# chronista-club/fleetflow

Hardware: AMD Instinct MI355X
Metric: container x node evaluations/sec (FFD what-if plans, work-equivalent) + achieved GB/s % HBM roofline (higher is better)
Workload: dtype u32

## Files before the change

### fleetflow_amd/_lib.py

```python
from __future__ import annotations

import ctypes as ct
import os

_HERE = os.path.dirname(os.path.abspath(__file__))
LIB_PATH = os.environ.get("FLEETPLACE_LIB") or os.path.join(_HERE, "libfleetplace.so")

FP_OK, FP_EINVAL, FP_ENOMEM, FP_EDEVICE, FP_EOVERFLOW, FP_ECORRUPT = 0, -1, -2, -3, -4, -5
FP_NONE = 0xFFFFFFFF
REASON_OK, REASON_NOFIT, REASON_CYCLE, REASON_SKEW, REASON_QUOTA = 0, 1, 2, 3, 4
FP_K_PLACE, FP_K_SORT, FP_K_FEAS, FP_K_LEVEL, FP_K_GEN = 0, 1, 2, 3, 4
STRATEGY_FIRST_FIT, STRATEGY_SPREAD, STRATEGY_PACK, STRATEGY_FILL_LOWEST = 0, 1, 2, 3
POLICY_STRATEGIES = {"spread_across_pool": STRATEGY_SPREAD, "pack_into_dedicated": STRATEGY_PACK,
                     "fill_lowest": STRATEGY_FILL_LOWEST}
FP_POLICY_MAX_NODES = 8192
FP_SPREAD_MAX_DOMAINS = 64
FP_FALLBACK_MAX_HOPS = 4
QUOTA_CPU, QUOTA_MEM, QUOTA_SERVICES, QUOTA_DIMS = 0, 1, 2, 3
QUOTA_NAMES = ("cpu", "memory", "services")
QUOTA_UNLIMITED = 0xFFFFFFFF
WHY_CORDON, WHY_CPU, WHY_MEM, WHY_LABEL, WHY_CONFLICT = 1, 2, 4, 8, 16
EXPLAIN_FAIL, EXPLAIN_ONLY, EXPLAIN_FEASIBLE, EXPLAIN_ALL, EXPLAIN_MISSING, EXPLAIN_NEAR = 0, 5, 10, 11, 12, 13
EXPLAIN_WORDS = 16
EXPLAIN_HIST_MIXED, EXPLAIN_HIST_FITS, EXPLAIN_HIST_SELECTED, EXPLAIN_HIST_WORDS = 5, 6, 7, 8
DRAIN_EVICTED, DRAIN_STRANDED, DRAIN_STRANDED_CPU, DRAIN_STRANDED_MEM = 0, 1, 2, 3
DRAIN_TARGETS, DRAIN_FIRST_STRANDED, DRAIN_NODES, DRAIN_WORDS = 4, 5, 6, 8
DRAIN_FIELDS = ("evicted", "stranded", "stranded_cpu", "stranded_mem", "targets", "first_stranded", "nodes")
DRAIN_STRANDED_SKEW, DRAIN_RELAXED, DRAIN_SKEW_BEFORE, DRAIN_SKEW_AFTER, DRAIN_POLICY_WORDS = 0, 1, 2, 3, 4
DRAIN_POLICY_FIELDS = ("stranded_skew", "relaxed", "skew_before", "skew_after")
SHRINK_RELEASED, SHRINK_TRIED, SHRINK_FAILED, SHRINK_MOVES, SHRINK_MOVED = 0, 1, 2, 3, 4
SHRINK_MOVED_CPU, SHRINK_MOVED_MEM, SHRINK_FIRST_FAILED, SHRINK_WORDS = 5, 6, 7, 8
SHRINK_FIELDS = ("released", "tried", "failed", "moves", "moved", "moved_cpu", "moved_mem", "first_failed")
SHRINK_STATE_NEVER, SHRINK_STATE_RELEASED, SHRINK_STATE_FAILED = 0, 1, 2
SHRINK_FAILED_SKEW, SHRINK_RELAXED, SHRINK_SKEW_BEFORE, SHRINK_SKEW_AFTER, SHRINK_POLICY_WORDS = 0, 1, 2, 3, 4
SHRINK_POLICY_FIELDS = ("failed_skew", "relaxed", "skew_before", "skew_after")
REBAL_MOVES, REBAL_STUCK, REBAL_STUCK_SKEW, REBAL_RELAXED, REBAL_MOVED_CPU = 0, 1, 2, 3, 4
REBAL_MOVED_MEM, REBAL_SKEW_BEFORE, REBAL_SKEW_AFTER, REBAL_WORDS = 5, 6, 7, 8
REBAL_FIELDS = ("moves", "stuck", "stuck_skew", "relaxed", "moved_cpu", "moved_mem", "skew_before", "skew_after")
GROW_PENDING, GROW_PLACED, GROW_OPENED, GROW_UNPLACEABLE, GROW_CAPPED = 0, 1, 2, 3, 4
GROW_LEFT_CPU, GROW_LEFT_MEM, GROW_FIRST_UNPLACED, GROW_WORDS = 5, 6, 7, 8
GROW_FIELDS = ("pending", "placed", "opened", "unplaceable", "capped", "left_cpu", "left_mem", "first_unplaced")
GROW_MAX_NEW = 8192
GROW_ON_LIVE, GROW_RELAXED, GROW_STUCK_SKEW, GROW_STUCK_QUOTA, GROW_SKEW_BEFORE, GROW_SKEW_AFTER = 0, 1, 2, 3, 4, 5
GROW_POLICY_WORDS = 8
GROW_POLICY_FIELDS = ("on_live", "relaxed", "stuck_skew", "stuck_quota", "skew_before", "skew_after")
CHANGE_KEPT, CHANGE_NEW, CHANGE_MOVED, CHANGE_LOST, CHANGE_ABSENT = 0, 1, 2, 3, 4
CHANGE_NAMES = ("kept", "new", "moved", "lost", "absent")
REPLAN_KEPT, REPLAN_NEW, REPLAN_MOVED, REPLAN_LOST, REPLAN_ABSENT = 0, 1, 2, 3, 4
REPLAN_MOVED_CPU, REPLAN_MOVED_MEM, REPLAN_WORDS = 5, 6, 8
FP_OPT_AUTO = -1
OPTIONS = {"pipe_w": 0, "pipe_seg": 1, "pipe_r": 2, "pipe_lag": 3, "link_slots": 4, "link_bounded": 5,
           "pipe_flush": 6, "spin_ticks": 7, "kpack": 8, "scen_sort": 9, "segsort": 10, "systolic": 11,
           "levelize_sync": 12, "systolic_extra": 13, "screen": 14, "payload_lds": 15, "systolic_valu": 16, "link_publish": 17,
           "level_sort": 18, "level_small": 19, "pipe_prio": 20,
           "indeg_bin": 21, "packed": 22, "sort_fused": 23}
GEOM_FIELDS = ("groups", "stages", "segments", "ring", "lag", "link_slots", "bounded", "resident", "systolic")

u8p = ct.POINTER(ct.c_uint8)
u32p = ct.POINTER(ct.c_uint32)
u64p = ct.POINTER(ct.c_uint64)
vp = ct.c_void_p


class FpGraph(ct.Structure):
    _fields_ = [("n_vertices", ct.c_uint32), ("n_edges", ct.c_uint32), ("row_ptr", vp), ("col", vp),
                ("has_deps", vp)]


class FpContainers(ct.Structure):
    _fields_ = [("n", ct.c_uint32), ("cpu_m", vp), ("mem_mib", vp), ("req_labels", vp), ("conflict", vp)]


class FpNodes(ct.Structure):
    _fields_ = [("n", ct.c_uint32), ("cpu_free", vp), ("mem_free", vp), ("labels", vp),
                ("conflict_used", vp), ("schedulable", vp)]


class FpBatch(ct.Structure):
    _fields_ = [("n_scen", ct.c_uint32), ("scen_base", ct.c_uint32), ("n_containers", ct.c_uint32),
                ("n_nodes", ct.c_uint32),
                ("cpu_m", vp), ("mem_mib", vp), ("req_labels", vp), ("conflict", vp), ("level", vp),
                ("cpu_free", vp), ("mem_free", vp), ("labels", vp), ("conflict_used", vp),
                ("schedulable", vp), ("assign", vp), ("reason", vp), ("cost", vp)]


class FleetplaceError(RuntimeError):
    def __init__(self, code, where):
        self.code = code
        msg = _lib_strerror(code) if _LIB is not None else str(code)
        super().__init__(f"{where}: {msg} ({code})")


_LIB = None

SIGNATURES = {
    "fp_ctx_create": (ct.c_int, [ct.POINTER(vp), ct.c_int]),
    "fp_ctx_destroy": (None, [vp]),
    "fp_ctx_set_stream": (ct.c_int, [vp, vp]),
    "fp_ctx_reset_stream": (ct.c_int, [vp]),
    "fp_ctx_sync": (ct.c_int, [vp]),
    "fp_strerror": (ct.c_char_p, [ct.c_int]),
    "fp_abi_version": (ct.c_int, []),
    "fp_ctx_profile": (ct.c_int, [vp, ct.c_int]),
    "fp_ctx_kernel_stats": (ct.c_int, [vp, ct.c_int, ct.POINTER(ct.c_double), ct.POINTER(ct.c_uint64)]),
    "fp_ctx_place_path": (ct.c_int, [vp, u32p]),
    "fp_ctx_set_option": (ct.c_int, [vp, ct.c_int, ct.c_int64]),
    "fp_ctx_get_option": (ct.c_int, [vp, ct.c_int, ct.POINTER(ct.c_int64)]),
    "fp_legacy_order": (ct.c_int, [vp, ct.POINTER(FpGraph), u32p]),
    "fp_levelize": (ct.c_int, [vp, ct.POINTER(FpGraph), u32p, u32p, u32p]),
    "fp_place": (ct.c_int, [vp, ct.POINTER(FpContainers), ct.POINTER(FpNodes), u32p, u32p, u8p]),
    "fp_place_batch": (ct.c_int, [vp, ct.POINTER(FpBatch)]),
    "fp_feasibility": (ct.c_int, [vp, ct.POINTER(FpContainers), ct.POINTER(FpNodes), u32p, u32p, u64p]),
    "fp_plan_stage": (ct.c_int, [vp, ct.POINTER(FpGraph), ct.POINTER(FpContainers), ct.POINTER(FpNodes), vp, vp,
                                 vp, u32p, vp, vp, vp, vp]),
    "fp_dev_legacy_order": (ct.c_int, [vp, ct.POINTER(FpGraph), vp]),
    "fp_dev_levelize": (ct.c_int, [vp, ct.POINTER(FpGraph), vp, vp, vp]),
    "fp_dev_place_batch": (ct.c_int, [vp, ct.POINTER(FpBatch)]),
    "fp_place_ws_bytes": (ct.c_int, [vp, ct.c_uint32, ct.c_uint32, ct.c_uint32, u64p]),
    "fp_place_geometry": (ct.c_int, [vp, ct.c_uint32, ct.c_uint32, ct.c_uint32, u32p]),
    "fp_dev_feasibility": (ct.c_int, [vp, ct.POINTER(FpContainers), ct.POINTER(FpNodes), vp, vp, vp]),
    "fp_dev_feasibility_batch": (ct.c_int, [vp, ct.POINTER(FpBatch), vp, vp]),
    "fp_place_policy": (ct.c_int, [vp, ct.POINTER(FpContainers), ct.POINTER(FpNodes), u32p, ct.c_uint32, ct.c_uint32,
                                   u32p, u32p, u8p]),
    "fp_place_batch_policy": (ct.c_int, [vp, ct.POINTER(FpBatch), u32p, u32p, u32p]),
    "fp_dev_place_batch_policy": (ct.c_int, [vp, ct.POINTER(FpBatch), vp, vp, vp]),
    "fp_place_policy_spread": (ct.c_int, [vp, ct.POINTER(FpContainers), ct.POINTER(FpNodes), u32p, ct.c_uint32,
                                          ct.c_uint32, u32p, u32p, ct.c_uint32, u32p, u8p]),
    "fp_place_batch_policy_spread": (ct.c_int, [vp, ct.POINTER(FpBatch), u32p, u32p, u32p, u32p, u32p]),
    "fp_dev_place_batch_policy_spread": (ct.c_int, [vp, ct.POINTER(FpBatch), vp, vp, vp, vp, vp]),
    "fp_place_policy_fallback": (ct.c_int, [vp, ct.POINTER(FpContainers), ct.POINTER(FpNodes), u32p, ct.c_uint32,
                                            ct.c_uint32, u32p, u32p, ct.c_uint32, u32p, ct.c_uint32, u32p, u8p, u8p]),
    "fp_place_batch_policy_fallback": (ct.c_int, [vp, ct.POINTER(FpBatch), u32p, u32p, u32p, u32p, u32p, u32p, u32p,
                                                  u8p]),
    "fp_dev_place_batch_policy_fallback": (ct.c_int, [vp, ct.POINTER(FpBatch), vp, vp, vp, vp, vp, vp, vp, vp]),
    "fp_place_policy_quota": (ct.c_int, [vp, ct.POINTER(FpContainers), ct.POINTER(FpNodes), u32p, ct.c_uint32,
                                         ct.c_uint32, u32p, u32p, ct.c_uint32, u32p, ct.c_uint32, u32p, u8p, u8p,
                                         u32p, u32p, u8p]),
    "fp_place_batch_policy_quota": (ct.c_int, [vp, ct.POINTER(FpBatch), u32p, u32p, u32p, u32p, u32p, u32p, u32p,
# ... 96 lines not shown
```

### fleetflow_amd/csrc/fp_internal.h

```cpp
#pragma once
#include <cmath>
#include <cstring>
#include <hip/hip_runtime.h>
#include <stdint.h>
#include <type_traits>
#include <vector>
#include "../../include/fleetplace.h"
#include "fp_rows.h"

#define FP_HIP(call)                                   \
    do {                                               \
        hipError_t e_ = (call);                        \
        if (e_ != hipSuccess) return fp_hip_fail(e_);  \
    } while (0)

int fp_hip_fail(hipError_t e);

__device__ __forceinline__ void fp_or_new_bits(uint32_t *w, uint32_t bits) {
    if (bits & ~*(volatile uint32_t *)w) atomicOr(w, bits);
}

struct fp_ctx {
    int device = 0;
    hipStream_t own_stream = nullptr;
// ... 137 lines not shown
                            const uint32_t *group, uint32_t n_cand, uint32_t strategy, uint32_t preferred,
                            const uint32_t *node_count, uint32_t *assign_out, uint8_t *reason_out,
                            uint32_t *summary_out, const fp_drain_policy &pol = fp_drain_policy());

struct fp_shrink_policy {
    const uint32_t *domain = nullptr;
    uint32_t max_skew = 0;
    const uint32_t *relax_mask = nullptr;
    uint32_t n_hops = 0;
    uint8_t *hops_out = nullptr;
    uint8_t *blocker_reason_out = nullptr;
    uint32_t *policy_out = nullptr;
};
constexpr uint32_t FP_SHRINK_MAX_CONTAINERS = 0x7FFF0000u;
int fp_dev_shrink_sweep_impl(fp_ctx *c, const fp_containers *cs, const fp_nodes *ns, const uint32_t *assign,
                             const uint32_t *try_order, uint32_t n_var, uint32_t n_try, uint32_t strategy,
                             uint32_t preferred, const uint32_t *node_count, uint32_t *assign_out, uint8_t *state_out,
                             uint32_t *blocker_out, uint32_t *summary_out, const fp_shrink_policy &pol = fp_shrink_policy());

struct fp_rebalance_opts {
    const uint32_t *node_count = nullptr;
    const uint32_t *domain = nullptr;
    uint32_t max_skew = 0;
    const uint32_t *relax_mask = nullptr;
    uint32_t n_hops = 0;
};
int fp_dev_rebalance_sweep_impl(fp_ctx *c, const fp_containers *cs, const fp_nodes *ns, const uint32_t *assign,
                                const uint32_t *victim_order, uint32_t n_var, uint32_t n_try, const uint32_t *max_moves,
                                uint32_t strategy, uint32_t preferred, const fp_rebalance_opts &o, uint32_t *assign_out,
                                uint8_t *hops_out, uint8_t *reason_out, uint32_t *summary_out);

int fp_dev_grow_sweep_impl(fp_ctx *c, const fp_containers *cs, const uint8_t *reason, uint32_t reason_mask,
                           uint32_t n_cand, const uint32_t *t_cpu, const uint32_t *t_mem, const uint32_t *t_labels,
                           const uint32_t *t_max, uint32_t max_new, uint32_t *summary_out, uint32_t *assign_out);

struct fp_grow_policy {
    const uint32_t *node_count = nullptr;
    uint32_t strategy = 0, preferred = 0;
    const uint32_t *domain = nullptr;
    const uint32_t *t_domain = nullptr;
    uint32_t max_skew = 0;
    const uint32_t *relax_mask = nullptr;
    uint32_t n_hops = 0;
    const uint32_t *quota = nullptr;
    const uint32_t *quota_used = nullptr;
    uint32_t *policy_out = nullptr;
    uint8_t *hops_out = nullptr;
    uint8_t *reason_out = nullptr;
};
int fp_dev_grow_sweep_policy_impl(fp_ctx *c, const fp_containers *cs, const uint8_t *reason, uint32_t reason_mask,
                                  const fp_nodes *ns, uint32_t n_cand, const uint32_t *t_cpu, const uint32_t *t_mem,
                                  const uint32_t *t_labels, const uint32_t *t_max, uint32_t max_new,
                                  uint32_t *summary_out, uint32_t *assign_out, const fp_grow_policy &pol);

int fp_dev_replan_batch_impl(fp_ctx *c, const fp_batch *b, const uint32_t *prev, const fp_policy_opts &o,
                             uint8_t *change_out, uint32_t *summary_out);
int fp_dev_replan_batch_policy_impl(fp_ctx *c, const fp_batch *b, const uint32_t *prev, const fp_policy_opts &o,
                                    uint8_t *change_out, uint32_t *summary_out);

bool fp_pipe_plan(const fp_ctx *c, uint32_t S, uint32_t N, uint32_t *G_out, uint32_t *W_out, uint32_t *B_out,
                  size_t *lds_out);
int fp_place_geometry_impl(fp_ctx *c, uint32_t S, uint32_t C, uint32_t N, uint32_t *out);
size_t fp_pipe_ws_bytes(fp_ctx *c, uint32_t S, uint32_t C, uint32_t N);
int fp_place_ws_bytes_impl(fp_ctx *c, uint32_t S, uint32_t C, uint32_t N, uint64_t *bytes);
constexpr int FP_BUCKETS = 32;
__host__ __device__ inline void fp_thresholds(uint32_t lo, uint32_t hi, uint32_t *T) {
    T[0] = 0;
    if (lo == 0) lo = 1;
    if (hi < lo) hi = lo;
    const double r = pow((double)hi / (double)lo, 1.0 / (double)(FP_BUCKETS - 2));
    double v = (double)lo;
    for (int k = 1; k < FP_BUCKETS; ++k) {
        uint32_t x = k == FP_BUCKETS - 1 ? hi : (uint32_t)ceil(v);
        if (x < T[k - 1]) x = T[k - 1];
        if (x > hi) x = hi;
        T[k] = x;
        v *= r;
    }
}
struct fp_pipe_soa {
    uint32_t *s_cpu, *s_mem, *s_req, *s_conf, *s_idx;
    uint32_t *summ = nullptr;
    bool payload_done = false;
};
int fp_pipe_soa_take(fp_ctx *c, size_t SC, fp_pipe_soa *soa);
uint32_t fp_pipe_kpack(const fp_ctx *c, uint32_t C);
int fp_pipe_node_summary(fp_ctx *c, uint32_t S, uint32_t C, uint32_t N, const fp_batch *b, uint32_t *rng,
                         uint32_t **summ);
uint32_t fp_pipe_payload_lds_max_c(const fp_ctx *c);
int fp_pipe_launch(fp_ctx *c, uint32_t S, uint32_t C, uint32_t N, uint32_t scen_base, const uint32_t *order,
                   const void *skeys, uint32_t key_bytes, uint32_t mbits, uint64_t cmax, uint64_t mmax,
                   const uint32_t *cval, const uint32_t *mval, const fp_batch *b, const uint32_t *thr,
                   const fp_pipe_soa *ready, uint32_t *rng);

namespace fpd {

constexpr uint64_t GAMMA = 0x9E3779B97F4A7C15ull;
constexpr uint64_t TAG_CONT = 0xC0C0C0C0C0C0C0C0ull;
constexpr uint64_t TAG_NODE = 0x5E5E5E5E5E5E5E5Eull;

__host__ __device__ inline uint64_t draw(uint64_t seed, uint64_t idx) {
    uint64_t z = seed + (idx + 1) * GAMMA;
    z = (z ^ (z >> 30)) * 0xBF58476D1CE4E5B9ull;
    z = (z ^ (z >> 27)) * 0x94D049BB133111EBull;
    return z ^ (z >> 31);
}
__host__ __device__ inline uint64_t scenario_seed(uint64_t seed, uint32_t s) {
    return seed ^ ((uint64_t)s * GAMMA);
}

__device__ __forceinline__ bool fits(uint32_t cpu, uint32_t mem, uint32_t req, uint32_t conf,
                                     uint32_t cf, uint32_t mf, uint32_t lab, uint32_t cu) {
    return (cf >= cpu) & (mf >= mem) & ((lab & req) == req) & ((cu & conf) == 0u);
}

__device__ __forceinline__ uint64_t pack_cost(uint32_t rej, uint32_t used, uint32_t id) {
    uint64_t r = rej > 0xFFFFFFu ? 0xFFFFFFu : rej;
    uint64_t u = used > 0xFFFFFFu ? 0xFFFFFFu : used;
    return (r << 40) | (u << 16) | (uint64_t)(id & 0xFFFFu);
}

}
```

### fleetflow_amd/csrc/fp_payload.h

```cpp
#pragma once
#include "fp_internal.h"

#ifndef FPP_PAYLOAD_BY_FIELD
#define FPP_PAYLOAD_BY_FIELD 1
#endif

namespace fpl {

constexpr uint32_t PL_THREADS = 1024, PL_H = 25, PL_MAX_C = PL_THREADS * PL_H * 2;
constexpr uint32_t PL_SKIP = 0x80000000u;
constexpr uint32_t PL_ROWS = 2 * PL_H;
constexpr uint32_t PL_FIELD_CHUNK = 36 * 1024;
constexpr size_t PL_FIELD_LDS_BYTES = (size_t)PL_FIELD_CHUNK * 4;
static_assert(PL_MAX_C < 0xFFFFu, "container indices are kept in 16 bits, 0xFFFF = no position");

enum pl_source {
    PL_ORDER = 0,
    PL_ORDER_SAME_WG,
    PL_LDS_X
};

__device__ __forceinline__ void pl_index(uint32_t w, uint32_t a0, uint32_t &d0, uint32_t &d1) {
    asm volatile("" : "+v"(w));
    d0 = (w & 0xFFFFu) - a0;
    d1 = (w >> 16) - a0;
}
__device__ __forceinline__ void pl_load_chunk(uint32_t *pl_lds, const uint32_t *__restrict__ src, uint32_t n) {
    __syncthreads();
#pragma unroll 8
    for (uint32_t i = threadIdx.x; i < n; i += PL_THREADS) pl_lds[i] = __builtin_nontemporal_load(&src[i]);
    __syncthreads();
}
__device__ __forceinline__ void pl_pick_field(uint32_t *pl_lds, const uint32_t *__restrict__ field, uint32_t C,
                                              const uint32_t (&o)[PL_H], uint32_t (&v)[PL_ROWS]) {
    for (uint32_t a0 = 0; a0 < C; a0 += PL_FIELD_CHUNK) {
        const uint32_t n = C - a0 < PL_FIELD_CHUNK ? C - a0 : PL_FIELD_CHUNK;
        pl_load_chunk(pl_lds, field + a0, n);
#pragma unroll
        for (uint32_t j = 0; j < PL_H; ++j) {
            uint32_t d0, d1;
            pl_index(o[j], a0, d0, d1);
            if (d0 < n) v[2 * j] = pl_lds[d0];
            if (d1 < n) v[2 * j + 1] = pl_lds[d1];
        }
    }
}

template <pl_source SRC>
__device__ __forceinline__ void pl_indices(uint32_t C, const uint32_t *ord, const uint16_t *X,
                                           uint32_t (&o)[PL_H]) {
    const uint32_t t = threadIdx.x;
    uint32_t i[PL_ROWS];
#pragma unroll
    for (uint32_t j = 0; j < PL_ROWS; ++j) {
        const uint32_t p = t + PL_THREADS * j;
        const uint32_t q = p < C ? p : C - 1;
        const uint32_t x = SRC == PL_LDS_X ? (uint32_t)X[q]
                           : SRC == PL_ORDER_SAME_WG
                               ? __hip_atomic_load(&ord[q], __ATOMIC_RELAXED, __HIP_MEMORY_SCOPE_AGENT)
                               : __builtin_nontemporal_load(&ord[q]);
        i[j] = p < C ? x & 0xFFFFu : 0xFFFFu;
    }
#pragma unroll
    for (uint32_t j = 0; j < PL_H; ++j) o[j] = i[2 * j] | i[2 * j + 1] << 16;
}

template <bool SAME_WG>
__device__ __forceinline__ void pl_by_field(uint32_t *pl_lds, uint32_t C, const uint32_t *order, const uint16_t *X,
                                            bool from_x, const uint32_t *req, const uint32_t *conf,
                                            const uint32_t *level, const uint32_t *summ, uint32_t *s_req,
                                            uint32_t *s_conf, uint32_t *s_idx) {
    const uint32_t t = threadIdx.x;
    const size_t cb = (size_t)blockIdx.x * C;
    const uint32_t sm0 = summ ? summ[(size_t)blockIdx.x * 4] : 0xFFFFFFFFu;
    const uint32_t sm1 = summ ? summ[(size_t)blockIdx.x * 4 + 1] : 0u;
    uint32_t o[PL_H];
    if (!SAME_WG) pl_indices<PL_ORDER>(C, order + cb, nullptr, o);
    else if (from_x) pl_indices<PL_LDS_X>(C, nullptr, X, o);
    else pl_indices<PL_ORDER_SAME_WG>(C, order + cb, nullptr, o);
    uint32_t cy0 = 0, cy1 = 0;
    if (level) {
        for (uint32_t a0 = 0; a0 < C; a0 += PL_FIELD_CHUNK) {
            const uint32_t n = C - a0 < PL_FIELD_CHUNK ? C - a0 : PL_FIELD_CHUNK;
            pl_load_chunk(pl_lds, level + cb + a0, n);
#pragma unroll
            for (uint32_t j = 0; j < PL_H; ++j) {
                uint32_t d0, d1;
                pl_index(o[j], a0, d0, d1);
                if (d0 < n) (j < 16 ? cy0 : cy1) |= (uint32_t)(pl_lds[d0] == FP_NONE) << ((2 * j) & 31u);
                if (d1 < n) (j < 16 ? cy0 : cy1) |= (uint32_t)(pl_lds[d1] == FP_NONE) << ((2 * j + 1) & 31u);
            }
        }
    }
    uint32_t v[PL_ROWS];
    uint32_t sc0 = 0, sc1 = 0;
    pl_pick_field(pl_lds, conf + cb, C, o, v);
    uint32_t tc = t, Cc = C;
    asm volatile("" : "+v"(tc), "+s"(Cc));
    uint32_t *const d_conf = s_conf + cb;
#pragma unroll
    for (uint32_t j = 0; j < PL_ROWS; ++j) {
        const uint32_t p = tc + PL_THREADS * j;
        if (p < Cc) {
            __builtin_nontemporal_store(v[j], &d_conf[p]);
            (j < 32 ? sc0 : sc1) |= (uint32_t)((v[j] & sm1) != 0u) << (j & 31u);
        }
    }
    pl_pick_field(pl_lds, req + cb, C, o, v);
    uint32_t tr = t, Cr = C;
    asm volatile("" : "+v"(tr), "+s"(Cr));
    uint32_t *const d_req = s_req + cb, *const d_idx = s_idx + cb;
#pragma unroll
    for (uint32_t j = 0; j < PL_ROWS; ++j) {
        const uint32_t p = tr + PL_THREADS * j;
        if (p < Cr) {
            uint32_t r = v[j];
            const bool c = ((j < 32 ? cy0 : cy1) >> (j & 31u)) & 1u;
            const bool x = (r & ~sm0) != 0u || (((j < 32 ? sc0 : sc1) >> (j & 31u)) & 1u);
            if (c) r = FP_REASON_CYCLE;
            else if (summ && x) r = FP_REASON_NOFIT;
            __builtin_nontemporal_store(r, &d_req[p]);
            if (c || (summ && x)) {
                if (SAME_WG) d_idx[p] = __hip_atomic_load(&d_idx[p], __ATOMIC_RELAXED, __HIP_MEMORY_SCOPE_AGENT) | PL_SKIP;
                else d_idx[p] |= PL_SKIP;
            }
        }
    }
}

}
```

### fleetflow_amd/csrc/fp_pipe.hip

```cpp
#include "fp_internal.h"
#include "fp_payload.h"
#include "fp_pipe_asm.h"
#include "fp_pipe_sys.h"
#include "fp_pipe_pk.h"
#include "fp_pipe_tus.h"
#include <stdlib.h>
#include <string.h>
#include <mutex>
#include <type_traits>
#include <utility>

#ifdef FP_PIPE_STATS
__device__ unsigned long long g_pipe_stats[16 * 16];
#define STAT_ADD(w, i, v) atomicAdd(&g_pipe_stats[(w) * 16 + (i)], (unsigned long long)(v))
#define STAT_CLK() __builtin_amdgcn_s_memtime()
#define STAT_ON 1
#ifdef FP_PIPE_STATS_FINE
#define STAT_GCLK() __builtin_amdgcn_s_memtime()
#define STAT_FINE 1
#else
#define STAT_GCLK() 0ull
#define STAT_FINE 0
#endif
constexpr int TL_B = 2048;
__device__ unsigned long long g_pipe_tl[16 * TL_B * 8];
constexpr int SPAN_MAX = 4096;
__device__ unsigned long long g_stage_span[SPAN_MAX * 8];
#else
#define STAT_ADD(w, i, v) ((void)0)
#define STAT_CLK() 0ull
#define STAT_GCLK() 0ull
#define STAT_ON 0
#define STAT_FINE 0
#endif

#ifndef FP_PRIO_LEVEL
#define FP_PRIO_LEVEL 2
#endif

namespace fpp {

constexpr int K = 32;
static_assert(K == FP_BUCKETS, "fp_place.hip and the pipeline agree on the bucket count");
constexpr uint32_t END = 0x80000000u;
constexpr uint32_t CYC = 0x80000000u;
constexpr uint64_t SPIN_TICKS = 100ull * 1000 * 1000 * 60;
constexpr uint32_t MAX_G = 16;
constexpr int SPIN_MAX = 12;
constexpr int NF = 5;
constexpr uint32_t IDX_POS_MASK = (1u << 21) - 1;

struct PipeArgs {
    uint32_t C, N, scen_base, W, G, R;
    uint32_t B;
    uint32_t S;
    uint32_t lag;
    uint32_t slots;
    uint32_t bounded;
    uint32_t flush;
    uint32_t kpack;
    uint32_t publish;
    uint32_t pub_mask;
    uint32_t sys;
    uint32_t *ticket;
    uint32_t *gabort;
    uint32_t *ghead;
    uint32_t *gdata;
    uint32_t *part;
    const uint32_t *s_cpu, *s_mem, *s_req, *s_conf, *s_idx;
    uint32_t *cf, *mf;
    const uint32_t *lab;
    uint32_t *cu;
    const uint8_t *sched;
    uint32_t *assign;
    uint8_t *reason;
    uint64_t *cost;
    uint32_t *err;
    uint64_t spin_ticks;
    const uint32_t *thr;
    uint32_t prio;
    uint32_t *rng;
    uint32_t pk_mode;
};

__device__ __forceinline__ uint32_t lds_acq(uint32_t *p) {
    return __builtin_amdgcn_readfirstlane(__hip_atomic_load(p, __ATOMIC_ACQUIRE, __HIP_MEMORY_SCOPE_WORKGROUP));
}
__device__ __forceinline__ void lds_rel(uint32_t *p, uint32_t v) {
    __hip_atomic_store(p, v, __ATOMIC_RELEASE, __HIP_MEMORY_SCOPE_WORKGROUP);
}

__device__ __forceinline__ uint32_t g_ld(const uint32_t *p) {
    return __hip_atomic_load(const_cast<uint32_t *>(p), __ATOMIC_RELAXED, __HIP_MEMORY_SCOPE_AGENT);
}
__device__ __forceinline__ uint32_t g_ld_u(const uint32_t *p) {
    return __builtin_amdgcn_readfirstlane(g_ld(p));
}
__device__ __forceinline__ void g_st(uint32_t *p, uint32_t v) {
    __hip_atomic_store(p, v, __ATOMIC_RELAXED, __HIP_MEMORY_SCOPE_AGENT);
}
__device__ __forceinline__ void g_touch(const uint32_t *p) {
    (void)__hip_atomic_load(const_cast<uint32_t *>(p), __ATOMIC_RELAXED, __HIP_MEMORY_SCOPE_WAVEFRONT);
}
__device__ __forceinline__ uint32_t g_ld_w(const uint32_t *p) {
    return __hip_atomic_load(const_cast<uint32_t *>(p), __ATOMIC_RELAXED, __HIP_MEMORY_SCOPE_WAVEFRONT);
}

template <class Pred>
__device__ __forceinline__ bool spin(uint32_t *word, Pred pred, uint32_t *abort_flag, uint32_t *err,
                                     uint64_t ticks, uint32_t &iters) {
    uint32_t n = 0;
    uint64_t t0 = 0;
    while (true) {
        const uint32_t v = lds_acq(word);
        if (pred(v)) { iters += n; return true; }
        if (lds_acq(abort_flag)) return false;
        if ((++n & 1023u) == 0) {
            const uint64_t now = __builtin_amdgcn_s_memrealtime();
            if (!t0) {
                t0 = now;
            } else if (now - t0 > ticks) {
                lds_rel(abort_flag, 1u);
                if ((threadIdx.x & 63) == 0) atomicMax(err, (uint32_t)(-FP_EDEVICE));
                return false;
            }
        }
        if (n < 8) __builtin_amdgcn_s_sleep(1);
        else if (n < 32) __builtin_amdgcn_s_sleep(4);
        else __builtin_amdgcn_s_sleep(SPIN_MAX);
    }
}


__device__ __forceinline__ uint32_t bucket_of(uint32_t v, uint32_t my_t, int base) {
    uint32_t k = 0;
#pragma unroll
    for (uint32_t step = K / 2; step; step >>= 1) {
        const uint32_t t = (uint32_t)__shfl((int)my_t, (int)(base + k + step));
        k += t <= v ? step : 0u;
    }
    return k;
}

__device__ __forceinline__ uint32_t fpp_rank(uint64_t m) {
    return __builtin_amdgcn_mbcnt_hi((uint32_t)(m >> 32), __builtin_amdgcn_mbcnt_lo((uint32_t)m, 0u));
}

__device__ __forceinline__ uint32_t wave_min(uint32_t v) {
    v = min(v, (uint32_t)__builtin_amdgcn_update_dpp(-1, (int)v, 0x111, 0xF, 0xF, false));
    v = min(v, (uint32_t)__builtin_amdgcn_update_dpp(-1, (int)v, 0x112, 0xF, 0xF, false));
    v = min(v, (uint32_t)__builtin_amdgcn_update_dpp(-1, (int)v, 0x114, 0xF, 0xF, false));
    v = min(v, (uint32_t)__builtin_amdgcn_update_dpp(-1, (int)v, 0x118, 0xF, 0xF, false));
    v = min(v, (uint32_t)__builtin_amdgcn_update_dpp(-1, (int)v, 0x142, 0xA, 0xF, false));
    v = min(v, (uint32_t)__builtin_amdgcn_update_dpp(-1, (int)v, 0x143, 0xC, 0xF, false));
    return __builtin_amdgcn_readlane(v, 63);
}


constexpr size_t LCTL = 64;

__device__ __forceinline__ bool gring_wait(uint32_t *tail, uint32_t need, uint32_t slots, uint32_t &seen,
                                           const PipeArgs &a, uint32_t *abort_flag, uint32_t lane,
                                           uint32_t &iters) {
    if (need - seen <= slots) return true;
    uint32_t n = 0;
    uint64_t t0 = 0;
    while (true) {
        seen = g_ld_u(tail);
        if (need - seen <= slots) { iters += n; return true; }
        if (g_ld_u(a.gabort) || lds_acq(abort_flag)) return false;
        if ((++n & 255u) == 0) {
            const uint64_t now = __builtin_amdgcn_s_memrealtime();
            if (!t0) {
                t0 = now;
            } else if (now - t0 > a.spin_ticks) {
                g_st(a.gabort, 1u);
                lds_rel(abort_flag, 1u);
                if (lane == 0) atomicMax(a.err, (uint32_t)(-FP_EDEVICE));
                return false;
            }
        }
        if (n < 8) __builtin_amdgcn_s_sleep(2);
        else __builtin_amdgcn_s_sleep(SPIN_MAX);
    }
}

template <uint32_t G>
using RecT = uint32_t[G];

#ifndef FPP_PF_MAX_WIDE
#define FPP_PF_MAX_WIDE 0
#endif
#ifndef FPP_PF_MAX_NARROW
#define FPP_PF_MAX_NARROW 4
#endif
constexpr uint32_t PF_MAX_NARROW = FPP_PF_MAX_NARROW, PF_MAX_WIDE = FPP_PF_MAX_WIDE;
#ifndef FPP_IB
#define FPP_IB 1
#endif
#ifndef FPP_IB1024
#define FPP_IB1024 1
#endif
#ifndef FPP_LOOKAHEAD
#define FPP_LOOKAHEAD 3
#endif
#ifndef FPP_DIRECT_TICKETS
#define FPP_DIRECT_TICKETS 1
#endif
constexpr uint32_t SYS_MAX_G = 4;
#ifndef FPP_MASK_UPKEEP
#define FPP_MASK_UPKEEP 0
#endif
#ifndef FPP_BIGP_NOMASK
#define FPP_BIGP_NOMASK 1
#endif
#ifndef FPP_BIGP_WAVES
#define FPP_BIGP_WAVES 7
#endif
#ifndef FPP_BIGP_LAZY
#define FPP_BIGP_LAZY 2
#endif
constexpr uint32_t BIGP_WV = 7;
constexpr bool is_bigp(uint32_t G, uint32_t BLK, uint32_t WV, bool PK) {
    return G == 12 && BLK == 64 && WV == BIGP_WV && PK;
}
#ifndef FPP_PK_SYS_MAX_G
#define FPP_PK_SYS_MAX_G 4
#endif
constexpr uint32_t PK_SYS_MAX_G = FPP_PK_SYS_MAX_G;
template <uint32_t G, bool UPD, bool IB, bool PK, uint32_t... gs, class Rec>
__device__ __forceinline__ void fpp_groups(std::integer_sequence<uint32_t, gs...>, uint32_t &nxt, uint64_t &placed,
                                           uint32_t &asg, uint32_t &used, uint32_t &used_hi, Rec &rcf, Rec &rmf,
                                           Rec &rcu, const Rec &rlab, uint32_t cpu, uint32_t mem, uint32_t req,
                                           uint32_t conf, uint32_t cand, uint32_t cand_hi, uint32_t my_t, uint32_t lane,
                                           uint64_t *Mw, uint32_t mlane, uint32_t gb64, uint32_t qc, uint32_t qm, uint32_t &nchk,
                                           uint32_t &nhit, uint32_t sys, unsigned long long (&gst)[4], uint32_t cw,
                                           uint32_t qw, uint32_t sc_c, uint32_t sc_m) {
    constexpr uint32_t pf_max = G <= SYS_MAX_G ? PF_MAX_NARROW : PF_MAX_WIDE;
    (
        [&] {
            uint64_t q = __builtin_amdgcn_ballot_w64(nxt == gs);
            if (pf_max > 0 && q) {
                uint64_t e;
                if constexpr (PK) e = __builtin_amdgcn_ballot_w64(pk_fits(rcf[gs], qw));
                else e = (__builtin_amdgcn_ballot_w64(rcf[gs] >= qc) & __builtin_amdgcn_ballot_w64(rmf[gs] >= qm));
                if (__builtin_popcountll(e) <= pf_max) {
                    bool ok = false;
                    while (e) {
                        const uint32_t l = (uint32_t)__builtin_ctzll(e);
                        e &= e - 1;
                        const uint32_t nlb = __builtin_amdgcn_readlane(rlab[gs], l);
                        const uint32_t ncu = __builtin_amdgcn_readlane(rcu[gs], l);
                        if constexpr (PK) {
                            const uint32_t nw = __builtin_amdgcn_readlane(rcf[gs], l);
                            ok |= ((((nw - cw) & PK_GUARD) | (req & nlb) | (conf & ncu)) == 0u);
                        } else {
                            const uint32_t ncf = __builtin_amdgcn_readlane(rcf[gs], l);
                            const uint32_t nmf = __builtin_amdgcn_readlane(rmf[gs], l);
                            ok |= (ncf >= cpu) & (nmf >= mem) & (((req & nlb) | (conf & ncu)) == 0u);
                        }
                    }
                    const uint64_t fit = q & __builtin_amdgcn_ballot_w64(ok);
                    if (q != fit) {
                        const uint64_t above = (((uint64_t)cand_hi << 32) | cand) & ~((2ull << gs) - 1ull);
                        const uint32_t nx = above ? (uint32_t)__builtin_ctzll(above) : G;
                        nxt = ((q & ~fit) >> lane) & 1ull ? nx : nxt;
                    }
                    q = fit;
                }
            }
            if (q) {
                uint64_t touched = 0;
                const unsigned long long gc0 = STAT_GCLK();
                if constexpr (PK) {
                    if (G <= PK_SYS_MAX_G && sys && (uint32_t)__builtin_popcountll(q) >= (sys & 0xFFFFu))
                        fpp_group_sysp<gs, G>(q, placed, touched, asg, nxt, rcf[gs], rcu[gs], rlab[gs], cw, req, conf,
                                              cand, cand_hi, gb64, nchk, nhit, qw, sys >> 16);
                    else
                        fpp_group_xp<gs, G, IB>(q, placed, touched, asg, nxt, rcf[gs], rcu[gs], rlab[gs], cw, req, conf,
                                                cand, cand_hi, gb64, nchk, nhit, qw);
                } else {
                    if (G <= SYS_MAX_G && sys && (uint32_t)__builtin_popcountll(q) >= (sys & 0xFFFFu))
                        fpp_group_sys<gs, G>(q, placed, touched, asg, nxt, rcf[gs], rmf[gs], rcu[gs], rlab[gs], cpu, mem,
                                             req, conf, cand, cand_hi, gb64, nchk, nhit, qc, qm, sys >> 16);
                    else
                        fpp_group_x<gs, G, IB>(q, placed, touched, asg, nxt, rcf[gs], rmf[gs], rcu[gs], rlab[gs], cpu, mem,
                                               req, conf, cand, cand_hi, gb64, nchk, nhit, qc, qm);
                }
                const unsigned long long gc1 = STAT_GCLK();
                if (STAT_FINE) { gst[0] += gc1 - gc0; gst[2] += 1; gst[3] += (uint32_t)__builtin_popcountll(touched); }
                if (touched) {
                    auto node_cm = [&](uint32_t l, uint32_t &nc, uint32_t &nm) {
                        if constexpr (PK) {
                            const uint32_t nw = __builtin_amdgcn_readlane(rcf[gs], l);
                            nc = pk_cpu(nw, sc_c);
                            nm = pk_mem(nw, sc_m);
                        } else {
                            nc = __builtin_amdgcn_readlane(rcf[gs], l);
                            nm = __builtin_amdgcn_readlane(rmf[gs], l);
                        }
                    };
                    if constexpr (IB) {
                        if (gs < 32) used = fpp_lane_sel<true>(touched, used | (1u << gs), used);
                        else used_hi = fpp_lane_sel<true>(touched, used_hi | (1u << (gs & 31)), used_hi);
// ... 4 lines not shown
                                const uint32_t l = (uint32_t)__builtin_ctzll(tt);
                                tt &= tt - 1;
                                uint32_t nc, nm;
                                node_cm(l, nc, nm);
                                const uint64_t below = (__builtin_amdgcn_ballot_w64(my_t > nc) & 0xFFFFFFFFull) |
                                                       (__builtin_amdgcn_ballot_w64(my_t > nm) & ~0xFFFFFFFFull);
                                if (l < 32) clr_lo = fpp_lane_sel<true>(below, clr_lo | (1u << l), clr_lo);
                                else clr_hi = fpp_lane_sel<true>(below, clr_hi | (1u << (l & 31)), clr_hi);
                            }
                            const uint64_t clr = ((uint64_t)clr_hi << 32) | clr_lo;
                            if (__builtin_amdgcn_ballot_w64(clr != 0))
                                asm volatile("ds_and_b64 %0, %1 offset:%2" ::"v"(mlane), "v"(~clr),
                                             "i"(gs * K * 2 * 8) : "memory");
                        }
                    } else {
                        const bool me = (touched >> lane) & 1ull;
                        if (gs < 32) used |= me ? (1u << gs) : 0u;
                        else used_hi |= me ? (1u << (gs & 31)) : 0u;
                        if (UPD) {
                            uint64_t clr = 0, tt = touched;
                            while (tt) {
                                const uint32_t l = (uint32_t)__builtin_ctzll(tt);
                                tt &= tt - 1;
                                uint32_t nc, nm;
                                node_cm(l, nc, nm);
                                clr |= (my_t > (lane < 32 ? nc : nm)) ? (1ull << l) : 0ull;
                            }
                            if (__builtin_amdgcn_ballot_w64(clr != 0))
                                atomicAnd((unsigned long long *)&Mw[(size_t)gs * K * 2 + (lane & (K - 1)) * 2 + (lane >> 5)],
                                          ~clr);
                        }
                    }
                }
                if (STAT_FINE) gst[1] += STAT_GCLK() - gc1;
            }
        }(),
        ...);
}

template <uint32_t g, bool CLOSE>
__device__ __forceinline__ void fpp_group_lazy_p(uint64_t &remaining, uint32_t &asg, uint32_t &used, uint32_t &rw,
                                                 uint32_t &rcu, uint32_t rlab, uint32_t cw, uint32_t req,
                                                 uint32_t conf, uint32_t gb64, uint32_t &nchk, uint32_t &nhit,
                                                 unsigned long long (&gst)[4], uint32_t &qw) {
    if (!CLOSE && !remaining) return;
    if (!__builtin_amdgcn_ballot_w64(pk_fits(rw, qw))) return;
    uint64_t touched = 0;
    const unsigned long long gc0 = STAT_GCLK();
    fpp_refilter_loop_p(remaining, touched, asg, rw, rcu, rlab, cw, req, conf, gb64 + g * 64u, nchk, qw);
    const uint64_t hit = remaining & __builtin_amdgcn_ballot_w64(asg != 0xFFFFFFFFu);
#ifdef FP_PIPE_STATS
    nhit += (uint32_t)__builtin_popcountll(hit);
#else
    (void)nhit;
#endif
    remaining = fpp_uniform64(remaining & ~hit);
    if (CLOSE) qw = remaining ? qw : PK_GUARD;
    const unsigned long long gc1 = STAT_GCLK();
    if (STAT_FINE) { gst[0] += gc1 - gc0; gst[2] += 1; gst[3] += (uint32_t)__builtin_popcountll(touched); }
    if (touched) used = fpp_lane_sel<true>(touched, used | (1u << g), used);
    if (STAT_FINE) gst[1] += STAT_GCLK() - gc1;
}

template <uint32_t G, uint32_t... gs, class Rec>
__device__ __forceinline__ void fpp_groups_lazy(std::integer_sequence<uint32_t, gs...>, uint64_t &remaining,
                                                uint32_t &asg, uint32_t &used, Rec &rcf, Rec &rcu, const Rec &rlab,
                                                uint32_t req, uint32_t conf, uint32_t gb64, uint32_t &nchk,
                                                uint32_t &nhit, unsigned long long (&gst)[4], uint32_t cw,
                                                uint32_t qw) {
    static_assert(G <= 32, "used bits of the lazy walk: one word");
    (fpp_group_lazy_p<gs, FPP_BIGP_LAZY == 2>(remaining, asg, used, rcf[gs], rcu[gs], rlab[gs], cw, req, conf, gb64,
                                              nchk, nhit, gst, qw),
     ...);
}

constexpr uint32_t WIDE_WAVES = 3, WIDE12_WAVES = 5;
#ifndef FPP_BIG_WAVES
#define FPP_BIG_WAVES 6
#endif
#ifndef FPP_BIG_S
#define FPP_BIG_S 4096
#endif
[[maybe_unused]] constexpr uint32_t WIDE12_BIG_WAVES = FPP_BIG_WAVES, WIDE12_BIG_S = FPP_BIG_S;
template <uint32_t G, uint32_t BLK, uint32_t WV = 0, bool PK = false>
__global__ __launch_bounds__(BLK, BLK == 64 ? (is_bigp(G, BLK, WV, PK) ? FPP_BIGP_WAVES
                                                : WV   ? WV
                                                : G == 12 ? WIDE12_WAVES
                                                          : WIDE_WAVES)
                                               : 1) void
k_ffd_pipe(const PipeArgs a_arg) {
#if defined(__HIP_DEVICE_COMPILE__)
    const PipeArgs &a = *(const PipeArgs *)__builtin_amdgcn_kernarg_segment_ptr();
#else
    const PipeArgs &a = a_arg;
#endif
    extern __shared__ __attribute__((aligned(16))) unsigned char smem[];
#ifndef FPP_W1
#define FPP_W1 1
#endif
    constexpr bool one_wave = BLK == 64 && FPP_W1;
    const uint32_t W = one_wave ? 1u : a.W, R = a.R, B = a.B, prio = a.prio;
    const uint32_t w = one_wave ? 0u : __builtin_amdgcn_readfirstlane(threadIdx.x >> 6);
    const uint32_t lane = threadIdx.x & 63;
    const uint32_t C = a.C, N = a.N;
    const uint32_t pmask = a.kpack ? IDX_POS_MASK : ~CYC;
    using GM = typename std::conditional<(G > 32), uint64_t, uint32_t>::type;

    constexpr bool NM = is_bigp(G, BLK, WV, PK) && FPP_BIGP_NOMASK;
    uint64_t *M = reinterpret_cast<uint64_t *>(smem);
    uint32_t *CTL = reinterpret_cast<uint32_t *>(M + (NM ? 0 : (size_t)W * G * K * 2));
    uint32_t *CNT = CTL + (W - 1) * 8;
    uint32_t *D = CNT + 8;

    uint32_t sc_c = 0, sc_m = 0;
    if (PK || a.pk_mode) {
        const uint32_t orc = __builtin_amdgcn_readfirstlane(a.rng[0]), orm = __builtin_amdgcn_readfirstlane(a.rng[1]);
        sc_c = orc ? (uint32_t)__builtin_ctz(orc) : 0u;
        sc_m = orm ? (uint32_t)__builtin_ctz(orm) : 0u;
        const bool packs = (orc >> sc_c) <= PK_FIELD_MAX && (orm >> sc_m) <= PK_FIELD_MAX;
        if (packs != PK) return;
    }
    if (blockIdx.x == 0 && threadIdx.x == 0 && a.rng) a.rng[2] = PK ? 2u : 1u;
    for (uint32_t i = threadIdx.x; i < (W - 1) * 8 + 8; i += blockDim.x) CTL[i] = 0;
    __syncthreads();
    if (threadIdx.x == 0) {
        const uint32_t total = (a.S + (B - 1) * a.lag) * B;
        uint32_t t;
        if (FPP_DIRECT_TICKETS && a.lag == a.S) {
            const uint32_t v = atomicAdd(a.ticket, 1u);
            t = v < a.S * B ? v * B + v / a.S : 0xFFFFFFFFu;
        } else {
            while (true) {
                t = atomicAdd(a.ticket, 1u);
                if (t >= total) { t = 0xFFFFFFFFu; break; }
                const uint32_t r = t / B, bb = t % B;
                if (r >= bb * a.lag && r - bb * a.lag < a.S) break;
            }
        }
        CNT[4] = t;
    }
    __syncthreads();
    const uint32_t tk = __builtin_amdgcn_readfirstlane(CNT[4]);
    if (tk == 0xFFFFFFFFu) return;
    const uint32_t b = tk % B, s = tk / B - b * a.lag;
    const size_t cb = (size_t)s * C, nb = (size_t)s * N;

    static_assert(K == 32, "mask/threshold lane layout assumes K == 32");
    const uint32_t my_t = NM ? 0u : a.thr[lane];
    const uint32_t gbase = (b * W + w) * G;
    uint64_t *Mw = M + (size_t)w * G * K * 2;
    const uint32_t mlane = (uint32_t)(uintptr_t)(__attribute__((address_space(3))) uint64_t *)(Mw + (lane & (K - 1)) * 2 + (lane >> 5));
    RecT<G> rcf, rmf, rcu, rlab;
    GM schedbits = 0;
    uint32_t usedbits = 0, used_hi = 0;
    {
        const uint32_t n0 = gbase * 64 + lane;
        const uint32_t *cf0 = a.cf + nb + n0, *mf0 = a.mf + nb + n0, *cu0 = a.cu + nb + n0, *lb0 = a.lab + nb + n0;
        const uint8_t *sc0 = a.sched + nb + n0;
#pragma unroll
        for (uint32_t g = 0; g < G; ++g) {
            const bool in = n0 + g * 64 < N;
            const int o = in ? (int)(g * 64) : -(int)n0;
            const bool sc = in && sc0[o] != 0;
            const uint32_t x = cf0[o], y = mf0[o], z = cu0[o], l = lb0[o];
            if constexpr (PK) {
                rcf[g] = sc ? pk_pack(x, y, sc_c, sc_m) : 0u;
            } else {
                rcf[g] = sc ? x : 0u;
                rmf[g] = sc ? y : 0u;
            }
            rcu[g] = sc ? z : 0xFFFFFFFFu;
            rlab[g] = sc ? ~l : 0xFFFFFFFFu;
            schedbits |= sc ? (GM(1) << g) : GM(0);
        }
    }
    uint32_t zs_g = G, zs_l = 0;
#pragma unroll
    for (uint32_t g = 0; g < G; ++g) {
        const uint64_t sm = __builtin_amdgcn_ballot_w64(((schedbits >> g) & 1u) != 0);
        if (zs_g == G && sm) {
            zs_g = g;
            zs_l = (uint32_t)__builtin_ctzll(sm);
        }
    }
#pragma unroll 1
    for (uint32_t k = 0; k < (NM ? 0u : (uint32_t)K); ++k) {
        const uint32_t tc = __builtin_amdgcn_readlane(my_t, k), tm = __builtin_amdgcn_readlane(my_t, K + k);
#pragma unroll
        for (uint32_t g = 0; g < G; ++g) {
            const bool sc = (schedbits >> g) & 1u;
            const uint32_t ncf = PK ? pk_cpu(rcf[g], sc_c) : rcf[g], nmf = PK ? pk_mem(rcf[g], sc_m) : rmf[g];
            const uint64_t bc = __builtin_amdgcn_ballot_w64(sc & (ncf >= tc));
            const uint64_t bm = __builtin_amdgcn_ballot_w64(sc & (nmf >= tm));
            if (lane == k) {
                Mw[((size_t)g * K + k) * 2] = bc;
                Mw[((size_t)g * K + k) * 2 + 1] = bm;
            }
        }
    }
    __syncthreads();

    const bool has_out = w + 1 < W;
    const bool g_in = w == 0 && b > 0;
    const bool g_out = w + 1 == W && b + 1 < B;
    const size_t LSLOT = 2 * 64;
    uint32_t *gin_head = a.ghead + ((size_t)s * (B - 1) + (b - 1)) * LCTL;
    uint32_t *gin_data = a.gdata + ((size_t)s * (B - 1) + (b - 1)) * a.slots * LSLOT;
    uint32_t *gout_head = a.ghead + ((size_t)s * (B - 1) + b) * LCTL;
    uint32_t *gout_data = a.gdata + ((size_t)s * (B - 1) + b) * a.slots * LSLOT;
    constexpr bool unbounded_only = BLK == 64 && WV != 0;
    const uint32_t gslots = a.slots, gbounded = unbounded_only ? 0u : a.bounded;
    const uint32_t gflush = unbounded_only ? (a.flush & 1u) : a.flush;
#define GSLOT(i) (unbounded_only ? (uint32_t)(i) : (uint32_t)(i) % gslots)
    uint32_t otail_seen = 0;
    uint32_t *octl = CTL + w * 8;
    uint32_t *ictl = CTL + (w - 1) * 8;
    uint32_t *odata = D + (size_t)w * R * NF * 64;
    uint32_t *idata = D + (size_t)(w - 1) * R * NF * 64;
    uint32_t *abort_flag = &CNT[2];
    uint32_t ohead = 0, ofill = 0, itail = 0, k0 = 0;
    uint32_t ihead_seen = 0;
    constexpr uint32_t LA = BLK == 64 ? (FPP_LOOKAHEAD >= 3 ? 1 : FPP_LOOKAHEAD) : 0;
    [[maybe_unused]] uint32_t la_n = 0, la_pos = 0;
    [[maybe_unused]] bool la_ok = false;
    constexpr bool DB = BLK == 64 && G == 12 && PK && FPP_LOOKAHEAD >= 3, DB_EARLY = DB && FPP_LOOKAHEAD == 3;
    [[maybe_unused]] uint32_t nf_cpu = 0, nf_mem = 0, nf_req = 0, nf_conf = 0, nf_idx = 0, nf_n = 0;
    [[maybe_unused]] bool nf_ok = false;
    [[maybe_unused]] uint32_t la2_n = 0, la2_pos = 0;
    constexpr int VMCNT0 = 0x0F70;
#define FPP_REQUEST_NEXT()                                                                              \
    do {                                                                                                \
        uint32_t off_;                                                                                  \
        if (g_in) {                                                                                     \
            const uint32_t tn_ = __builtin_amdgcn_readfirstlane(la_n);                                  \
            off_ = (la_ok && !(tn_ & END) && lane < tn_) ? la_pos & pmask : 0u;                         \
            nf_n = tn_;                                                                                 \
            nf_ok = la_ok;                                                                              \
        } else {                                                                                        \
            off_ = min(k0 + lane, C - 1u);                                                              \
            nf_ok = true;                                                                               \
        }                                                                                               \
        const size_t o_ = cb + off_;                                                                    \
        nf_cpu = g_ld_w(a.s_cpu + o_);                                                                  \
        nf_mem = g_ld_w(a.s_mem + o_);                                                                  \
        nf_req = g_ld_w(a.s_req + o_);                                                                  \
        nf_conf = g_ld_w(a.s_conf + o_);                                                                \
        if (!g_in) nf_idx = g_ld_w(a.s_idx + o_);                                                       \
        else if (!DB_EARLY) nf_idx = la_pos;                                                            \
        if (DB_EARLY && g_in) {  \
            la_ok = itail + 1u < ihead_seen;                                                            \
            const uint32_t *sn_ = la_ok ? gin_data + (size_t)GSLOT(itail + 1u) * LSLOT : a.s_idx + cb;  \
            la2_n = g_ld(sn_);                                                                          \
            la2_pos = g_ld(sn_ + (la_ok ? 64u + lane : 0u));                                            \
        }                                                                                               \
    } while (0)
    uint32_t opend = 0;
    uint32_t n_used = 0, n_rej = 0;
    uint32_t st_spin_in = 0, st_spin_out = 0, st_visits = 0, st_checks = 0, st_hits = 0, st_batches = 0;
    unsigned long long ck_in = 0, ck_pre = 0, ck_cand = 0, ck_fwd = 0, ck_wait = 0, ck_gx = 0, ck_gu = 0;
    uint32_t st_queues = 0, st_touched = 0;
    const unsigned long long ck_t0 = STAT_CLK();
    unsigned long long ck_a, ck_b;
#ifdef FP_PIPE_STATS
    const unsigned long long sp_start = __builtin_amdgcn_s_memrealtime();
    unsigned long long sp_first = 0;
#endif
    bool alive = true;
    if constexpr (DB) __builtin_amdgcn_s_waitcnt(VMCNT0);
    while (alive) {
        if (prio == 2u) __builtin_amdgcn_s_setprio(0);
        ck_a = STAT_CLK();
#ifdef FP_PIPE_STATS
        const unsigned long long tl_top = ck_a;
        unsigned long long tl_avail = ck_a;
#endif
        uint32_t cpu = 0, mem = 0, req = 0, conf = 0, idx = 0;
        bool valid = false;
        if (g_in) {
            uint32_t n_sp = 0;
            uint64_t t0 = 0;
            bool got = itail < ihead_seen;
            while (!got) {
                ihead_seen = g_ld_u(gin_head);
                if (ihead_seen > itail) { got = true; break; }
                if (g_ld_u(a.gabort) || lds_acq(abort_flag)) break;
                if ((++n_sp & 255u) == 0) {
                    const uint64_t now = __builtin_amdgcn_s_memrealtime();
                    if (!t0) {
                        t0 = now;
                    } else if (now - t0 > a.spin_ticks) {
                        g_st(a.gabort, 1u);
                        lds_rel(abort_flag, 1u);
                        if (lane == 0) atomicMax(a.err, (uint32_t)(-FP_EDEVICE));
                        break;
                    }
                }
                if (n_sp < 8) __builtin_amdgcn_s_sleep(2);
                else __builtin_amdgcn_s_sleep(SPIN_MAX);
            }
            st_spin_in += n_sp;
            if (!got) break;
#ifdef FP_PIPE_STATS
            tl_avail = STAT_CLK();
#endif
            __builtin_amdgcn_fence(__ATOMIC_ACQUIRE, "wavefront");
            if (((gflush & 2u) || (gbounded && (itail & 3u) == 0)) && lane == 0) g_st(gin_head + LCTL / 2, itail);
            const uint32_t *sd = gin_data + (size_t)GSLOT(itail) * LSLOT;
            uint32_t n, pos;
            if (DB && nf_ok) {
                n = nf_n;
                pos = nf_idx;
            } else if (LA && !DB_EARLY && la_ok) {
                n = __builtin_amdgcn_readfirstlane(la_n);
                pos = la_pos;
            } else {
                n = g_ld_u(sd);
                pos = g_ld(sd + 64 + lane);
                if constexpr (NM) __builtin_amdgcn_s_waitcnt(VMCNT0);
            }
            if (n & END) break;
            valid = lane < n;
            if (DB && nf_ok) {
                idx = valid ? pos : 0u;
                cpu = valid ? nf_cpu : 0u;
                mem = valid ? nf_mem : 0u;
                req = valid ? nf_req : 0u;
                conf = valid ? nf_conf : 0u;
            } else {
                if (valid) {
                    idx = pos;
                    const uint32_t p = pos & pmask;
                    cpu = a.s_cpu[cb + p];
                    mem = a.s_mem[cb + p];
                    req = a.s_req[cb + p];
                    conf = a.s_conf[cb + p];
                }
                if constexpr (DB) __builtin_amdgcn_s_waitcnt(VMCNT0);
            }
            itail++;
        } else if (w == 0) {
            if (k0 >= C) break;
            const uint32_t i = k0 + lane;
            valid = i < C;
            if (DB && nf_ok) {
                cpu = valid ? nf_cpu : 0u;
                mem = valid ? nf_mem : 0u;
                req = valid ? nf_req : 0u;
                conf = valid ? nf_conf : 0u;
                idx = valid ? nf_idx : 0u;
            } else {
                if (valid) {
                    cpu = a.s_cpu[cb + i];
                    mem = a.s_mem[cb + i];
                    req = a.s_req[cb + i];
                    conf = a.s_conf[cb + i];
                    idx = a.s_idx[cb + i];
                }
                if constexpr (DB) __builtin_amdgcn_s_waitcnt(VMCNT0);
            }
            const bool cyc = valid && (idx & CYC);
            if (cyc) {
                const uint32_t j = idx & pmask;
                a.assign[cb + j] = FP_NONE;
                a.reason[cb + j] = (uint8_t)req;
            }
            n_rej += (uint32_t)__popcll(__ballot(cyc));
            valid = valid && !cyc;
            k0 += 64;
            if constexpr (LA >= 2) {
                if (k0 < C) {
                    const size_t ti = cb + min(k0 + (lane == 0 ? 0u : lane == 1 ? 32u : 63u), C - 1);
                    g_touch(a.s_cpu + ti);
                    g_touch(a.s_mem + ti);
                    g_touch(a.s_req + ti);
                    g_touch(a.s_conf + ti);
                    g_touch(a.s_idx + ti);
                }
            }
        } else {
            const uint32_t want = itail;
            if (!spin(&ictl[0], [want](uint32_t h) { return h != want; }, abort_flag, a.err, a.spin_ticks, st_spin_in)) break;
#ifdef FP_PIPE_STATS
            tl_avail = STAT_CLK();
#endif
            const uint32_t slot = itail % R;
            const uint32_t n = __builtin_amdgcn_readfirstlane(ictl[2 + slot]);
            if (n & END) break;
            const uint32_t *sd = idata + (size_t)slot * NF * 64;
            valid = lane < n;
            if (valid) {
                cpu = sd[lane];
                mem = sd[64 + lane];
                req = sd[128 + lane];
                conf = sd[192 + lane];
                idx = sd[256 + lane];
            }
            itail++;
            lds_rel(&ictl[1], itail);
        }
        if constexpr (LA != 0 && !DB_EARLY) {
            la_ok = g_in && itail < ihead_seen;
            if (g_in) {
                const uint32_t *sn = la_ok ? gin_data + (size_t)GSLOT(itail) * LSLOT : a.s_idx + cb;
                la_n = g_ld(sn);
                la_pos = g_ld(sn + (la_ok ? 64u + lane : 0u));
            }
        }
        uint32_t tail_async = 0;
        const bool tail_issued = (gflush & 2u) && g_out && ofill != 0;
        if (tail_issued) tail_async = g_ld(gout_head + LCTL / 2);
        uint32_t kc, km;
        if constexpr (NM) {
            kc = km = 0;
        } else if (a.kpack) {
            kc = (idx >> 21) & (uint32_t)(K - 1);
            km = (idx >> 26) & (uint32_t)(K - 1);
        } else {
            kc = bucket_of(cpu, my_t, 0);
            km = bucket_of(mem, my_t, K);
        }
        if (prio == 2u) __builtin_amdgcn_s_setprio(FP_PRIO_LEVEL);
        ck_b = STAT_CLK(); ck_in += ck_b - ck_a; ck_a = ck_b;
#ifdef FP_PIPE_STATS
        if (!sp_first) sp_first = __builtin_amdgcn_s_memrealtime();
#endif
#ifdef FP_PIPE_STATS
        const unsigned long long ck_t0_batch = ck_b;
#endif

        const uint64_t vm = __builtin_amdgcn_ballot_w64(valid);
        const uint32_t qc = vm ? __builtin_amdgcn_readlane(cpu, 63 - __builtin_clzll(vm)) : 0xFFFFFFFFu;
        const uint32_t qm = wave_min(valid ? mem : 0xFFFFFFFFu);
        const uint32_t cw = PK ? pk_pack(cpu, mem, sc_c, sc_m) : 0u;
        const uint32_t qw = PK ? pk_pack(qc, qm, sc_c, sc_m) : 0u;
        [[maybe_unused]] bool zero_early = false;
        if constexpr (DB_EARLY) {
            zero_early = valid && (cpu | mem | req | conf) == 0u;
            FPP_REQUEST_NEXT();
        }
        const uint32_t oc = kc * 2, om = km * 2 + 1;
        constexpr bool prescan_skip = G > SYS_MAX_G;
        constexpr bool LZ = NM && FPP_BIGP_LAZY;
        GM cand = 0;
#pragma unroll
        for (uint32_t g = 0; g < (LZ ? 0u : G); ++g) {
            const uint64_t e = PK ? __builtin_amdgcn_ballot_w64(pk_fits(rcf[g], qw))
                                  : (__builtin_amdgcn_ballot_w64(rcf[g] >= qc) & __builtin_amdgcn_ballot_w64(rmf[g] >= qm));
            const uint64_t *mg = Mw + (size_t)g * K * 2;
            if constexpr (NM) {
                cand |= e ? GM(1) << g : GM(0);
            } else if (prescan_skip) {
                if (e) cand |= (mg[oc] & mg[om] & e) ? GM(1) << g : GM(0);
            } else {
                cand |= (mg[oc] & mg[om] & e) ? GM(1) << g : GM(0);
            }
        }
        cand = valid ? cand : GM(0);
        if constexpr (LA >= 2) {
            if (g_in && la_ok) {
                const uint32_t tn = __builtin_amdgcn_readfirstlane(la_n);
                if (!(tn & END)) {
                    const uint32_t tp = lane < tn ? la_pos & pmask : 0u;
                    g_touch(a.s_cpu + cb + tp);
                    g_touch(a.s_mem + cb + tp);
                    g_touch(a.s_req + cb + tp);
                    g_touch(a.s_conf + cb + tp);
                }
            }
        }
        const bool zero = DB_EARLY ? zero_early : valid && (cpu | mem | req | conf) == 0u;
        uint64_t todo;
        if constexpr (LZ) todo = __builtin_amdgcn_ballot_w64(valid && !zero);
        else todo = __builtin_amdgcn_ballot_w64(cand != 0 && !zero);
        uint64_t placed = 0;
        uint32_t my_assign = FP_NONE;
        if (STAT_ON) {
            st_batches++;
            st_visits += (uint32_t)__popcll(__ballot(valid));
        }
        ck_b = STAT_CLK(); ck_pre += ck_b - ck_a; ck_a = ck_b;
#ifdef FP_PIPE_STATS
        const unsigned long long tl_pre = ck_b;
        const uint32_t tl_checks0 = st_checks, tl_hits0 = st_hits, tl_todo = (uint32_t)__popcll(todo);
#endif
        if constexpr (LZ) {
            uint32_t nchk = 0, nhit = 0;
            unsigned long long gst[4] = {0, 0, 0, 0};
            if (prio == 1u && todo) __builtin_amdgcn_s_setprio(FP_PRIO_LEVEL);
            if (todo) {
                uint64_t remaining = todo;
                fpp_groups_lazy<G>(std::make_integer_sequence<uint32_t, G>{}, remaining, my_assign, usedbits,
                                   rcf, rcu, rlab, req, conf, __builtin_amdgcn_readfirstlane(gbase * 64u), nchk, nhit,
                                   gst, cw, qw);
                placed = todo & ~remaining;
            }
            if (prio == 1u && todo) __builtin_amdgcn_s_setprio(0);
            if (STAT_ON) { st_checks += nchk; st_hits += nhit; }
            if (STAT_FINE) { ck_gx += gst[0]; ck_gu += gst[1]; st_queues += (uint32_t)gst[2]; st_touched += (uint32_t)gst[3]; }
        } else {
            uint32_t nxt = ((todo >> lane) & 1ull) ? (cand ? (uint32_t)__builtin_ctzll((uint64_t)cand) : G) : G;
            uint32_t nchk = 0, nhit = 0;
            unsigned long long gst[4] = {0, 0, 0, 0};
            if (prio == 1u && todo) __builtin_amdgcn_s_setprio(FP_PRIO_LEVEL);
            if (todo)
                fpp_groups<G, (G > 1) && FPP_MASK_UPKEEP, (BLK == 64 || (FPP_IB1024 && G > SYS_MAX_G)) && FPP_IB, PK>(std::make_integer_sequence<uint32_t, G>{}, nxt, placed, my_assign, usedbits,
                                       used_hi, rcf, rmf, rcu, rlab, cpu, mem, req, conf, (uint32_t)cand,
                                       (uint32_t)((uint64_t)cand >> 32), my_t, lane, Mw, mlane,
                                       __builtin_amdgcn_readfirstlane(gbase * 64u), qc, qm, nchk, nhit, a.sys, gst,
                                       cw, qw, sc_c, sc_m);
            if (prio == 1u && todo) __builtin_amdgcn_s_setprio(0);
            if (STAT_ON) { st_checks += nchk; st_hits += nhit; }
            if (STAT_FINE) { ck_gx += gst[0]; ck_gu += gst[1]; st_queues += (uint32_t)gst[2]; st_touched += (uint32_t)gst[3]; }
        }
        if (zs_g < G) {
            const uint64_t zm = __builtin_amdgcn_ballot_w64(zero);
            if (zm) {
                placed |= zm;
// ... 187 lines not shown
        if (n < N && ((schedbits >> g) & 1u)) {
            a.cf[nb + n] = PK ? pk_cpu(rcf[g], sc_c) : rcf[g];
            a.mf[nb + n] = PK ? pk_mem(rcf[g], sc_m) : rmf[g];
            a.cu[nb + n] = rcu[g];
        }
    }
    __syncthreads();
    if (threadIdx.x == 0) {
        a.part[((size_t)s * B + b) * 2] = CNT[0];
        a.part[((size_t)s * B + b) * 2 + 1] = CNT[1];
    }
}

__global__ void k_cost_reduce(uint32_t S, uint32_t B, uint32_t scen_base, const uint32_t *__restrict__ part,
                              uint64_t *__restrict__ cost) {
    const uint32_t s = blockIdx.x * blockDim.x + threadIdx.x;
    if (s >= S) return;
    uint32_t used = 0, rej = 0;
    for (uint32_t b = 0; b < B; ++b) {
        used += part[((size_t)s * B + b) * 2];
        rej += part[((size_t)s * B + b) * 2 + 1];
    }
    cost[s] = fpd::pack_cost(rej, used, scen_base + s);
}

template <bool SUMM, bool RANGE>
__global__ __launch_bounds__(256) void k_node_summary(uint32_t N, const uint32_t *__restrict__ cf,
                                                      const uint32_t *__restrict__ mf, const uint32_t *__restrict__ lab,
                                                      const uint32_t *__restrict__ cu,
                                                      const uint8_t *__restrict__ sched, uint32_t *__restrict__ summ,
                                                      uint32_t *__restrict__ rng) {
    const size_t nb = (size_t)blockIdx.x * N;
    uint32_t u = 0, a = 0xFFFFFFFFu, oc = 0, om = 0;
    constexpr uint32_t NS_U = 4;
    for (uint32_t n0 = threadIdx.x; n0 < N; n0 += NS_U * blockDim.x) {
        uint32_t l[NS_U], c[NS_U], x[NS_U], y[NS_U];
        uint8_t sc[NS_U];
#pragma unroll
        for (uint32_t k = 0; k < NS_U; ++k) {
            const uint32_t n = n0 + k * blockDim.x;
            sc[k] = n < N ? sched[nb + n] : 0;
            if (SUMM) {
                l[k] = n < N ? lab[nb + n] : 0u;
                c[k] = n < N ? cu[nb + n] : 0xFFFFFFFFu;
            }
            if (RANGE) {
                x[k] = n < N ? cf[nb + n] : 0u;
                y[k] = n < N ? mf[nb + n] : 0u;
            }
        }
#pragma unroll
        for (uint32_t k = 0; k < NS_U; ++k) {
            if (sc[k]) {
                if (SUMM) {
                    u |= l[k];
                    a &= c[k];
                }
                if (RANGE) {
                    oc |= x[k];
                    om |= y[k];
                }
            }
        }
    }
    for (int o = 32; o > 0; o >>= 1) {
        u |= (uint32_t)__shfl_xor((int)u, o);
        a &= (uint32_t)__shfl_xor((int)a, o);
        oc |= (uint32_t)__shfl_xor((int)oc, o);
        om |= (uint32_t)__shfl_xor((int)om, o);
    }
    __shared__ uint32_t red[4][4];
    const uint32_t w = threadIdx.x >> 6;
    if ((threadIdx.x & 63) == 0) { red[0][w] = u; red[1][w] = a; red[2][w] = oc; red[3][w] = om; }
    __syncthreads();
    if (threadIdx.x == 0) {
        for (uint32_t q = 1; q < blockDim.x / 64; ++q) { u |= red[0][q]; a &= red[1][q]; oc |= red[2][q]; om |= red[3][q]; }
        if (SUMM) {
            summ[(size_t)blockIdx.x * 4] = u;
            summ[(size_t)blockIdx.x * 4 + 1] = a;
        }
        if (RANGE) {
            fp_or_new_bits(&rng[0], oc);
            fp_or_new_bits(&rng[1], om);
        }
    }
}

__device__ __forceinline__ bool screened(const uint32_t *sm, uint32_t req, uint32_t conf) {
    return ((req & ~sm[0]) | (conf & sm[1])) != 0u;
}

template <class KeyT>
__global__ void k_gather_sorted(const uint32_t *__restrict__ thr, uint32_t kpack, uint32_t S, uint32_t C,
                                const uint32_t *__restrict__ order,
                                const KeyT *__restrict__ skeys, uint32_t mbits, uint64_t cmax, uint64_t mmax,
                                const uint32_t *__restrict__ cval, const uint32_t *__restrict__ mval,
                                const uint32_t *__restrict__ cpu, const uint32_t *__restrict__ mem,
                                const uint32_t *__restrict__ req, const uint32_t *__restrict__ conf,
                                const uint32_t *__restrict__ level, const uint32_t *__restrict__ summ,
                                uint32_t *__restrict__ s_cpu, uint32_t *__restrict__ s_mem,
                                uint32_t *__restrict__ s_req, uint32_t *__restrict__ s_conf,
                                uint32_t *__restrict__ s_idx) {
    const uint32_t total = S * C;
    const uint32_t lb = (gridDim.x & 7u) ? blockIdx.x : (blockIdx.x & 7u) * (gridDim.x >> 3) + (blockIdx.x >> 3);
    const uint32_t stride = blockDim.x;
    __shared__ uint32_t T[2 * K];
    if (threadIdx.x < 2 * K) T[threadIdx.x] = thr[threadIdx.x];
    __syncthreads();
    auto bucket = [](const uint32_t *t, uint32_t v) {
        uint32_t k = 0;
#pragma unroll
        for (uint32_t step = K / 2; step; step >>= 1) k += t[k + step] <= v ? step : 0u;
        return k;
    };
    {
        const size_t i0 = (size_t)lb * 4 * blockDim.x + threadIdx.x;
        uint32_t j[4], src[4], r[4], f[4], cy[4], cv[4], mv[4], pos[4];
#pragma unroll
        for (int u = 0; u < 4; ++u) {
            const size_t i = i0 + (size_t)u * stride;
            if (i < total) j[u] = __builtin_nontemporal_load(&order[i]);
        }
#pragma unroll
        for (int u = 0; u < 4; ++u) {
            const size_t i = i0 + (size_t)u * stride;
            if (i < total) {
                pos[u] = (uint32_t)i % C;
                src[u] = (uint32_t)i - pos[u] + j[u];
                if (skeys) {
                    const uint64_t k = __builtin_nontemporal_load(&skeys[i]);
                    cv[u] = (uint32_t)(cmax - (mbits >= 64 ? 0ull : ((k >> mbits) & cmax)));
                    mv[u] = (uint32_t)(mmax - (k & mmax));
                }
            }
        }
#pragma unroll
        for (int u = 0; u < 4; ++u) {
            const size_t i = i0 + (size_t)u * stride;
            if (i < total) {
                r[u] = req[src[u]];
                f[u] = conf[src[u]];
                cy[u] = (level && level[src[u]] == FP_NONE) ? CYC : 0u;
                if (cy[u]) {
                    r[u] = FP_REASON_CYCLE;
                } else if (summ && screened(summ + (size_t)((uint32_t)i / C) * 4, r[u], f[u])) {
                    cy[u] = CYC;
                    r[u] = FP_REASON_NOFIT;
                }
                if (skeys) {
                    if (cval) cv[u] = cval[cv[u]];
                    if (mval) mv[u] = mval[mv[u]];
                } else {
                    cv[u] = cpu[src[u]];
                    mv[u] = mem[src[u]];
                }
            }
        }
#pragma unroll
        for (int u = 0; u < 4; ++u) {
            const size_t i = i0 + (size_t)u * stride;
            if (i < total) {
                __builtin_nontemporal_store(cv[u], &s_cpu[i]);
                __builtin_nontemporal_store(mv[u], &s_mem[i]);
                __builtin_nontemporal_store(r[u], &s_req[i]);
                __builtin_nontemporal_store(f[u], &s_conf[i]);
                const uint32_t kb = kpack ? (bucket(T, cv[u]) << 21) | (bucket(T + K, mv[u]) << 26) : 0u;
// ... 51 lines not shown
constexpr size_t PL_LDS_BYTES = fpl::PL_FIELD_LDS_BYTES;

__global__ __launch_bounds__(1024) void k_payload_lds(uint32_t C, const uint32_t *__restrict__ order,
                                                      const uint32_t *__restrict__ req,
                                                      const uint32_t *__restrict__ conf,
                                                      const uint32_t *__restrict__ level,
                                                      const uint32_t *__restrict__ summ,
                                                      uint32_t *__restrict__ s_req, uint32_t *__restrict__ s_conf,
                                                      uint32_t *__restrict__ s_idx) {
    extern __shared__ uint32_t pl_lds[];
    fpl::pl_by_field<false>(pl_lds, C, order, nullptr, false, req, conf, level, summ, s_req, s_conf, s_idx);
}
#else
constexpr uint32_t PL_CHUNK = 18 * 1024;
constexpr size_t PL_LDS_BYTES = (size_t)PL_CHUNK * 8;
__global__ __launch_bounds__(1024) void k_payload_lds(uint32_t C, const uint32_t *__restrict__ order,
                                                      const uint32_t *__restrict__ req,
                                                      const uint32_t *__restrict__ conf,
                                                      const uint32_t *__restrict__ level,
                                                      const uint32_t *__restrict__ summ,
                                                      uint32_t *__restrict__ s_req, uint32_t *__restrict__ s_conf,
                                                      uint32_t *__restrict__ s_idx) {
    extern __shared__ uint2 pl_lds2[];
    uint32_t *pl_lds = reinterpret_cast<uint32_t *>(pl_lds2);
    const uint32_t t = threadIdx.x;
    const size_t cb = (size_t)blockIdx.x * C;
    const uint32_t sm0 = summ ? summ[(size_t)blockIdx.x * 4] : 0xFFFFFFFFu;
    const uint32_t sm1 = summ ? summ[(size_t)blockIdx.x * 4 + 1] : 0u;
    for (uint32_t h = 0; h < 2; ++h) {
        const uint32_t pbase = h * PL_THREADS * PL_H + t;
        if (h * PL_THREADS * PL_H >= C) break;
        uint32_t o[PL_H];
#pragma unroll
        for (uint32_t j = 0; j < PL_H; ++j) {
            const uint32_t p = pbase + PL_THREADS * j;
            o[j] = p < C ? __builtin_nontemporal_load(&order[cb + p]) : 0xFFFFFFFFu;
        }
        uint32_t vr[PL_H], vf[PL_H];
        uint32_t cy = 0;
        if (level) {
            for (uint32_t a0 = 0; a0 < C; a0 += 2 * PL_CHUNK) {
                const uint32_t n = C - a0 < 2 * PL_CHUNK ? C - a0 : 2 * PL_CHUNK;
                __syncthreads();
#pragma unroll 4
                for (uint32_t i = t; i < n; i += PL_THREADS) pl_lds[i] = __builtin_nontemporal_load(&level[cb + a0 + i]);
                __syncthreads();
#pragma unroll
                for (uint32_t j = 0; j < PL_H; ++j) {
                    const uint32_t d = o[j] - a0;
                    if (d < n) cy |= (uint32_t)(pl_lds[d] == FP_NONE) << j;
                }
            }
        }
        for (uint32_t a0 = 0; a0 < C; a0 += PL_CHUNK) {
            const uint32_t n = C - a0 < PL_CHUNK ? C - a0 : PL_CHUNK;
            __syncthreads();
#pragma unroll 4
            for (uint32_t i = t; i < n; i += PL_THREADS)
                pl_lds2[i] = make_uint2(__builtin_nontemporal_load(&req[cb + a0 + i]), __builtin_nontemporal_load(&conf[cb + a0 + i]));
            __syncthreads();
#pragma unroll
            for (uint32_t j = 0; j < PL_H; ++j) {
                const uint32_t d = o[j] - a0;
                if (d < n) { const uint2 x = pl_lds2[d]; vr[j] = x.x; vf[j] = x.y; }
            }
        }
#pragma unroll
        for (uint32_t j = 0; j < PL_H; ++j) {
            const uint32_t p = pbase + PL_THREADS * j;
            if (p < C) {
                uint32_t r = vr[j];
                const bool c = (cy >> j) & 1u, x = ((r & ~sm0) | (vf[j] & sm1)) != 0u;
                if (c) r = FP_REASON_CYCLE;
                else if (summ && x) r = FP_REASON_NOFIT;
                __builtin_nontemporal_store(r, &s_req[cb + p]);
                __builtin_nontemporal_store(vf[j], &s_conf[cb + p]);
                if (c || (summ && x)) s_idx[cb + p] |= CYC;
            }
        }
    }
}
#endif

constexpr uint32_t UNSORT_SPAN16 = 50 * 1024;
constexpr uint32_t UNSORT_SPAN32 = 30 * 1024;
template <bool NARROW>
__global__ __launch_bounds__(1024) void k_unsort(uint32_t C, uint32_t H, uint32_t span,
                                                 const uint32_t *__restrict__ order,
                                                 const uint32_t *__restrict__ asg_s, const uint8_t *__restrict__ rsn_s,
                                                 uint32_t *__restrict__ assign, uint8_t *__restrict__ reason) {
    using A = typename std::conditional<NARROW, uint16_t, uint32_t>::type;
    extern __shared__ __attribute__((aligned(16))) unsigned char ulds[];
    A *la = reinterpret_cast<A *>(ulds);
    uint8_t *lr = ulds + (size_t)span * sizeof(A);
    const uint32_t s = blockIdx.x / H, h = blockIdx.x % H;
    const uint32_t lo = h * span, hi = min(C, lo + span);
    const size_t cb = (size_t)s * C;
    constexpr uint32_t U = 8;
    for (uint32_t p0 = threadIdx.x; p0 < C; p0 += blockDim.x * U) {
        uint32_t j[U], av[U];
        uint8_t rv[U];
#pragma unroll
        for (uint32_t u = 0; u < U; ++u) {
            const uint32_t p = p0 + u * blockDim.x;
            j[u] = p < C ? __builtin_nontemporal_load(&order[cb + p]) : 0xFFFFFFFFu;
            av[u] = p < C ? __builtin_nontemporal_load(&asg_s[cb + p]) : 0u;
            rv[u] = p < C ? __builtin_nontemporal_load(&rsn_s[cb + p]) : 0;
        }
#pragma unroll
        for (uint32_t u = 0; u < U; ++u) {
            if (j[u] >= lo && j[u] < hi) {
                la[j[u] - lo] = (A)av[u];
                lr[j[u] - lo] = av[u] != FP_NONE ? (uint8_t)FP_REASON_OK : rv[u];
            }
        }
    }
    __syncthreads();
    for (uint32_t j = lo + threadIdx.x; j < hi; j += blockDim.x) {
        const A v = la[j - lo];
        __builtin_nontemporal_store(NARROW && v == (A)0xFFFF ? FP_NONE : (uint32_t)v, &assign[cb + j]);
        reason[cb + j] = lr[j - lo];
    }
}

size_t lds_bytes(uint32_t W, uint32_t G, uint32_t R) {
    return (size_t)W * G * K * 16 + ((size_t)(W - 1) * 8 + 8) * 4 + (size_t)(W - 1) * R * NF * 64 * 4;
}
size_t lds_bytes_bigp(uint32_t R) { return FPP_BIGP_NOMASK ? 8 * 4 : lds_bytes(1, 12, R); }

template <uint32_t G, uint32_t BLK = 1024, uint32_t WV = 0, bool PK = false>
static int launch_g(hipStream_t st, unsigned grid, unsigned block, size_t lds, const PipeArgs &a) {
    if (block > BLK) return FP_EINVAL;
    FP_HIP(hipFuncSetAttribute((const void *)k_ffd_pipe<G, BLK, WV, PK>, hipFuncAttributeMaxDynamicSharedMemorySize,
                               (int)lds));
    k_ffd_pipe<G, BLK, WV, PK><<<grid, block, lds, st>>>(a);
    return FP_OK;
}

typedef int (*launch_fn)(hipStream_t, unsigned, unsigned, size_t, const PipeArgs &);
#ifndef FPP_KERNEL_TU
struct TuKernel {
    uint32_t G, BLK, WV, PK;
    launch_fn launch;
    const void *(*kernel)();
};
static_assert(WIDE12_BIG_WAVES == 6 && BIGP_WV == 7,
              "fp_pipe_tus.h names the 4096-scenario kernels: big by six waves per SIMD, bigp by seven");
#ifdef FPP_SPLIT
}
#define FPP_TU_DECL(name, G, BLK, WV, PK)                                                    \
    int fpp_tu_launch_##name(hipStream_t, unsigned, unsigned, size_t, const void *);         \
    const void *fpp_tu_kernel_##name();
FPP_TUS(FPP_TU_DECL)
#undef FPP_TU_DECL
namespace fpp {
#define FPP_TU_ENTRY(name, G, BLK, WV, PK)                                                                     \
    {G, BLK, WV, PK,                                                                                           \
     [](hipStream_t st, unsigned gr, unsigned bl, size_t l, const PipeArgs &a) {                                \
         return ::fpp_tu_launch_##name(st, gr, bl, l, &a);                                                    \
     },                                                                                                        \
     ::fpp_tu_kernel_##name},
#else
#define FPP_TU_ENTRY(name, G, BLK, WV, PK) \
    {G, BLK, WV, PK, launch_g<G, BLK, WV, (bool)PK>, [] { return (const void *)k_ffd_pipe<G, BLK, WV, (bool)PK>; }},
#endif
static const TuKernel kTu[] = {FPP_TUS(FPP_TU_ENTRY)};
#undef FPP_TU_ENTRY
constexpr bool in_tu(uint32_t G, uint32_t BLK, uint32_t WV) {
#define FPP_TU_IS(name, g, blk, wv, pk) || ((g) == G && (blk) == BLK && (wv) == WV && !(pk))
    return false FPP_TUS(FPP_TU_IS);
#undef FPP_TU_IS
}
static const TuKernel *tu_find(uint32_t G, uint32_t BLK, uint32_t WV, bool PK) {
    for (const TuKernel &k : kTu)
        if (k.G == G && k.BLK == BLK && k.WV == WV && (k.PK != 0) == PK) return &k;
    return nullptr;
}
template <uint32_t G, uint32_t BLK = 1024, uint32_t WV = 0>
static constexpr launch_fn main_launch() {
    if constexpr (in_tu(G, BLK, WV)) return nullptr;
    else return launch_g<G, BLK, WV>;
}
template <uint32_t G, uint32_t BLK = 1024, uint32_t WV = 0>
static inline const void *main_kernel() {
    if constexpr (in_tu(G, BLK, WV)) return nullptr;
    else return (const void *)k_ffd_pipe<G, BLK, WV>;
}
static const launch_fn kLaunch[MAX_G + 1] = {
    nullptr,           main_launch<1>(),  main_launch<2>(),  main_launch<3>(),  main_launch<4>(),
    main_launch<5>(),  main_launch<6>(),  main_launch<7>(),  main_launch<8>(),  main_launch<9>(),
    main_launch<10>(), main_launch<11>(), main_launch<12>(), main_launch<13>(), main_launch<14>(),
    main_launch<15>(), main_launch<16>()};
static const void *const kKernel[MAX_G + 1] = {
    nullptr,           main_kernel<1>(),  main_kernel<2>(),  main_kernel<3>(),  main_kernel<4>(),
    main_kernel<5>(),  main_kernel<6>(),  main_kernel<7>(),  main_kernel<8>(),  main_kernel<9>(),
    main_kernel<10>(), main_kernel<11>(), main_kernel<12>(), main_kernel<13>(), main_kernel<14>(),
    main_kernel<15>(), main_kernel<16>()};
constexpr uint32_t MAX_G_WIDE = 40;
static const launch_fn kLaunchWide[MAX_G_WIDE / 4 + 1] = {
    nullptr, nullptr, nullptr, main_launch<12, 64>(), main_launch<16, 64>(), main_launch<20, 64>(),
    main_launch<24, 64>(), main_launch<28, 64>(), main_launch<32, 64>(), main_launch<36, 64>(), main_launch<40, 64>()};
static const void *const kKernelWide[MAX_G_WIDE / 4 + 1] = {
    nullptr, nullptr, nullptr, main_kernel<12, 64>(), main_kernel<16, 64>(), main_kernel<20, 64>(),
    main_kernel<24, 64>(), main_kernel<28, 64>(), main_kernel<32, 64>(), main_kernel<36, 64>(), main_kernel<40, 64>()};
static inline bool wide_g(uint32_t W, uint32_t G) { return W == 1 && G >= 12; }
static inline bool wide12_big(uint32_t S, uint32_t W, uint32_t G) { return W == 1 && G == 12 && S >= WIDE12_BIG_S; }
static void pipe_kernel(uint32_t G, uint32_t W, bool big, bool PK, launch_fn *l, const void **k) {
    const bool wide = wide_g(W, G);
    const uint32_t BLK = wide ? 64u : 1024u, WV = big ? (PK ? BIGP_WV : WIDE12_BIG_WAVES) : 0u;
    *l = nullptr;
    *k = nullptr;
    if (const TuKernel *t = tu_find(G, BLK, WV, PK)) {
        *l = t->launch;
        *k = t->kernel();
        return;
    }
    if (PK || big) return;
    if (wide) {
        if (G % 4 == 0 && G / 4 < sizeof(kLaunchWide) / sizeof(kLaunchWide[0])) {
            *l = kLaunchWide[G / 4];
            *k = kKernelWide[G / 4];
        }
    } else if (G < sizeof(kLaunch) / sizeof(kLaunch[0])) {
        *l = kLaunch[G];
        *k = kKernel[G];
    }
}
#endif

}

#ifdef FPP_KERNEL_TU
#define FPP_TU_CAT2(a, b) a##b
#define FPP_TU_CAT(a, b) FPP_TU_CAT2(a, b)
int FPP_TU_CAT(fpp_tu_launch_, FPP_TU_NAME)(hipStream_t st, unsigned grid, unsigned block, size_t lds, const void *args) {
    return fpp::launch_g<FPP_TU_G, FPP_TU_BLK, FPP_TU_WV, (bool)FPP_TU_PK>(st, grid, block, lds,
                                                                          *static_cast<const fpp::PipeArgs *>(args));
}
const void *FPP_TU_CAT(fpp_tu_kernel_, FPP_TU_NAME)() {
    return (const void *)fpp::k_ffd_pipe<FPP_TU_G, FPP_TU_BLK, FPP_TU_WV, (bool)FPP_TU_PK>;
}
#endif

#ifndef FPP_KERNEL_TU

using namespace fpp;

constexpr uint32_t MAX_SEG_GROUPS = 40;
constexpr size_t LDS_HALF_CU = 80 * 1024;
constexpr uint64_t kNarrowWaves = 4096;

bool fp_pipe_plan(const fp_ctx *c, uint32_t S, uint32_t N, uint32_t *G_out, uint32_t *W_out, uint32_t *B_out,
                  size_t *lds_out) {
    const uint32_t NG = (N + 63) / 64;
    const size_t cap = 160 * 1024;
    if (NG == 0) {
        *G_out = 1; *W_out = 1; *B_out = 1; *lds_out = lds_bytes(1, 1, 2);
        return true;
    }
    const int forced_w = (int)fp_opt(c, FP_OPT_PIPE_W, 0);
    const int forced_seg = (int)fp_opt(c, FP_OPT_PIPE_SEG, 0);
    const bool narrow = (uint64_t)S * NG <= kNarrowWaves;
    const bool mid4 = !narrow && S <= 512, mid2 = !narrow && !mid4 && S <= 1024;
    const uint32_t seg_groups = forced_seg > 0 && forced_seg <= (int)MAX_SEG_GROUPS ? (uint32_t)forced_seg
                                : narrow ? 4u : (forced_w > 1 || mid4) ? MAX_SEG_GROUPS : mid2 ? 16u : 12u;
    const uint32_t B = (NG + seg_groups - 1) / seg_groups;
    const uint32_t per_seg = (NG + B - 1) / B;
    const uint32_t first_w = forced_w > 0 ? (uint32_t)forced_w : narrow ? 4u : mid4 ? 4u : mid2 ? 2u : 1u;
    for (uint32_t W : {first_w, 4u, 8u, 2u, 1u, 12u, 16u}) {
        if (W > per_seg && W > 1) continue;
        uint32_t G = (per_seg + W - 1) / W;
        if (wide_g(W, G)) {
            G = (G + 3) / 4 * 4;
            if (G > MAX_G_WIDE) continue;
        } else if (G > MAX_G) {
            continue;
        }
        const uint32_t Wn = (per_seg + G - 1) / G;
        const size_t lds = lds_bytes(Wn, G, 2);
        if (lds > cap) continue;
        *G_out = G; *W_out = Wn; *B_out = B; *lds_out = lds;
        return true;
    }
    return false;
}

struct PipeGeom {
    uint32_t G, W, B, R;
    size_t lds;
    size_t lds_big_pk;
    uint32_t lag;
    uint32_t slots;
    uint32_t bounded;
    uint32_t resident;
    uint32_t sys;
    uint32_t sys_extra;
    uint32_t prio;
};

struct BoundedGate {
    std::mutex m;
    hipEvent_t ev = nullptr;
};
constexpr int kMaxGateDevices = 64;
static BoundedGate g_bounded_gate[kMaxGateDevices];

constexpr uint32_t LINK_RING_SLOTS = 256;

static bool pipe_geom(fp_ctx *c, uint32_t S, uint32_t C, uint32_t N, PipeGeom *g) {
    if (!fp_pipe_plan(c, S, N, &g->G, &g->W, &g->B, &g->lds)) return false;
    const uint32_t G = g->G, W = g->W, B = g->B;
    uint32_t R = 2;
    for (uint32_t r = 4; r > 2; --r)
        if (lds_bytes(W, G, r) <= LDS_HALF_CU) { R = r; break; }
    {
        const int64_t fr = fp_opt(c, FP_OPT_PIPE_R, 0);
        if (fr >= 2 && fr <= 6 && lds_bytes(W, G, (uint32_t)fr) <= 160 * 1024) R = (uint32_t)fr;
    }
    g->R = R;
    g->lds = lds_bytes(W, G, R);
    g->lds_big_pk = wide12_big(S, W, G) ? lds_bytes_bigp(R) : g->lds;
    auto resident_of = [&](bool big) -> uint64_t {
        int dev_cu = 0;
        (void)hipDeviceGetAttribute(&dev_cu, hipDeviceAttributeMultiprocessorCount, c->device);
        uint64_t res = 0;
        for (const bool pk : {false, true}) {
            launch_fn l;
            const void *fn;
            pipe_kernel(G, W, big, pk, &l, &fn);
            int occ = 0;
            if (!fn) continue;
            if (dev_cu <= 0 || hipOccupancyMaxActiveBlocksPerMultiprocessor(&occ, fn, (int)(W * 64), big && pk ? g->lds_big_pk : g->lds) !=
                                   hipSuccess ||
                occ <= 0)
                return 0;
            const uint64_t r = (uint64_t)occ * (uint64_t)dev_cu;
            res = res && res < r ? res : r;
        }
        return res;
    };
    uint64_t slots_total = resident_of(wide12_big(S, W, G));
    g->resident = (uint32_t)(slots_total < 0xFFFFFFFFull ? slots_total : 0xFFFFFFFFull);
    const bool fits = B > 1 && slots_total && (uint64_t)S * B <= slots_total;
    g->lag = (uint32_t)fp_opt(c, FP_OPT_PIPE_LAG, (B > 1 && S > 1 && slots_total && !fits) ? S : 0u);
    const uint32_t full = (C + 63) / 64 + 2;
    uint32_t ring = LINK_RING_SLOTS;
    {
        const int64_t v = fp_opt(c, FP_OPT_LINK_SLOTS, 0);
        if (v >= 8 && v < (int64_t)full) ring = (uint32_t)v;
    }
    const bool margin = 2ull * B <= slots_total;
    g->bounded = (uint32_t)fp_opt(c, FP_OPT_LINK_BOUNDED, (fits && margin && g->lag == 0 && ring < full) ? 1 : 0);
    if (B <= 1) g->bounded = 0;
    g->slots = g->bounded ? (ring < full ? ring : full) : full;
    if (g->bounded && wide12_big(S, W, G)) {
        const uint64_t r5 = resident_of(false);
        g->resident = (uint32_t)(r5 < 0xFFFFFFFFull ? r5 : 0xFFFFFFFFull);
    }
    g->sys = G <= (SYS_MAX_G > PK_SYS_MAX_G ? SYS_MAX_G : PK_SYS_MAX_G) ? (uint32_t)fp_opt(c, FP_OPT_SYSTOLIC, 32) : 0u;
    if (g->sys > 64) g->sys = 64;
    g->sys_extra = (uint32_t)fp_opt(c, FP_OPT_SYSTOLIC_EXTRA, 16);
    if (g->sys_extra > 128) g->sys_extra = 128;
    {
        const int64_t sv = fp_opt(c, FP_OPT_SYSTOLIC_VALU, 2);
        if (sv == 1) g->sys_extra |= 0x8000u;
        else if (sv == 2) g->sys_extra |= 0x4000u;
    }
    {
        const int64_t pv = fp_opt(c, FP_OPT_PIPE_PRIO, wide12_big(S, W, G) ? 0 : 1);
        g->prio = pv >= 0 && pv <= 2 ? (uint32_t)pv : 0u;
    }
    return true;
}

size_t fp_pipe_ws_bytes(fp_ctx *c, uint32_t S, uint32_t C, uint32_t N) {
    PipeGeom g;
    if (!pipe_geom(c, S, C, N, &g)) return 0;
    const size_t SC = (size_t)S * C, nlinks = (size_t)S * (g.B - 1);
    return 5 * SC * 4 + SC * 5 + 256 + nlinks * LCTL * 4 + (size_t)S * g.B * 8 + 8 + nlinks * g.slots * 2 * 64 * 4 +
           (size_t)S * 16 + 11 * 256;
}

uint32_t fp_pipe_kpack(const fp_ctx *c, uint32_t C) {
    return C <= (IDX_POS_MASK + 1u) && fp_opt(c, FP_OPT_KPACK, 1) != 0;
}

int fp_pipe_soa_take(fp_ctx *c, size_t SC, fp_pipe_soa *soa) {
    soa->s_cpu = (uint32_t *)fp_ws_take(c, SC * 4);
    soa->s_mem = (uint32_t *)fp_ws_take(c, SC * 4);
    soa->s_req = (uint32_t *)fp_ws_take(c, SC * 4);
    soa->s_conf = (uint32_t *)fp_ws_take(c, SC * 4);
    soa->s_idx = (uint32_t *)fp_ws_take(c, SC * 4);
    return (soa->s_cpu && soa->s_mem && soa->s_req && soa->s_conf && soa->s_idx) ? FP_OK : FP_ENOMEM;
}

int fp_pipe_node_summary(fp_ctx *c, uint32_t S, uint32_t C, uint32_t N, const fp_batch *b, uint32_t *rng,
                         uint32_t **summ_out) {
    PipeGeom geo;
    if (!pipe_geom(c, S, C, N, &geo)) return FP_EOVERFLOW;
    hipStream_t st = c->stream;
    uint32_t *summ = nullptr;
    if (N && fp_opt(c, FP_OPT_SCREEN, 1)) {
        summ = (uint32_t *)fp_ws_take(c, (size_t)S * 16);
        if (!summ) return FP_ENOMEM;
    }
    launch_fn pkfn = nullptr;
    if (rng && fp_opt(c, FP_OPT_PACKED, 1) != 0) {
        const void *k_;
        pipe_kernel(geo.G, geo.W, wide12_big(S, geo.W, geo.G) && !geo.bounded, true, &pkfn, &k_);
    }
    if (N && (summ || pkfn)) {
        if (summ && pkfn) k_node_summary<true, true><<<S, 256, 0, st>>>(N, b->cpu_free, b->mem_free, b->labels, b->conflict_used, b->schedulable, summ, rng);
        else if (summ) k_node_summary<true, false><<<S, 256, 0, st>>>(N, b->cpu_free, b->mem_free, b->labels, b->conflict_used, b->schedulable, summ, rng);
        else k_node_summary<false, true><<<S, 256, 0, st>>>(N, b->cpu_free, b->mem_free, b->labels, b->conflict_used, b->schedulable, summ, rng);
        FP_HIP(hipGetLastError());
    }
    *summ_out = summ;
    return FP_OK;
}

uint32_t fp_pipe_payload_lds_max_c(const fp_ctx *c) {
    return FPP_PAYLOAD_BY_FIELD && fp_opt(c, FP_OPT_PAYLOAD_LDS, 1) != 0 ? PL_MAX_C : 0u;
}

int fp_pipe_launch(fp_ctx *c, uint32_t S, uint32_t C, uint32_t N, uint32_t scen_base, const uint32_t *order,
                   const void *skeys, uint32_t key_bytes, uint32_t mbits, uint64_t cmax, uint64_t mmax,
                   const uint32_t *cval, const uint32_t *mval, const fp_batch *b, const uint32_t *thr,
                   const fp_pipe_soa *ready, uint32_t *rng) {
    PipeGeom geo;
    if (!pipe_geom(c, S, C, N, &geo)) return FP_EOVERFLOW;
    const uint32_t G = geo.G, W = geo.W, B = geo.B, R = geo.R, slots = geo.slots;
    const size_t lds = geo.lds;
    if (C >= 0x80000000u) return FP_EOVERFLOW;
    if ((uint64_t)S * B > 0xFFFFFFFFull) return FP_EOVERFLOW;
    hipStream_t st = c->stream;
    const size_t SC = (size_t)S * C;
    const size_t nlinks = (size_t)S * (B - 1);
    fp_pipe_soa soa;
    if (ready) soa = *ready;
    else if (int rc0 = fp_pipe_soa_take(c, SC, &soa)) return rc0;
    uint32_t *s_cpu = soa.s_cpu, *s_mem = soa.s_mem, *s_req = soa.s_req, *s_conf = soa.s_conf, *s_idx = soa.s_idx;
    uint32_t *ctl = (uint32_t *)fp_ws_take(c, 256 + nlinks * LCTL * 4);
    uint32_t *part = (uint32_t *)fp_ws_take(c, (size_t)S * B * 8 + 8);
    uint32_t *gdata = nlinks ? (uint32_t *)fp_ws_take(c, nlinks * slots * 2 * 64 * 4) : nullptr;
    uint32_t *asg_s = (uint32_t *)fp_ws_take(c, SC * 4);
    uint8_t *rsn_s = (uint8_t *)fp_ws_take(c, SC);
    if (!ctl || !part || (nlinks && !gdata) || !asg_s || !rsn_s) return FP_ENOMEM;
    FP_HIP(hipMemsetAsync(ctl, 0, 256 + nlinks * LCTL * 4, st));
    const uint32_t kpack = fp_pipe_kpack(c, C);
    launch_fn u32fn = nullptr, pkfn = nullptr;
    const bool big = wide12_big(S, W, G) && !geo.bounded;
    {
        const void *k_;
        pipe_kernel(G, W, big, false, &u32fn, &k_);
        if (rng && fp_opt(c, FP_OPT_PACKED, 1) != 0) pipe_kernel(G, W, big, true, &pkfn, &k_);
        if (!u32fn) return FP_EOVERFLOW;
    }
    const bool payload_done = ready && ready->payload_done;
    uint32_t *summ = payload_done ? ready->summ : nullptr;
    if (!payload_done)
        if (int rc0 = fp_pipe_node_summary(c, S, C, N, b, rng, &summ)) return rc0;
    const int64_t pl_mode = fp_opt(c, FP_OPT_PAYLOAD_LDS, 1);
    if (payload_done) {
    } else if (ready && C && C <= PL_MAX_C && pl_mode != 0) {
        const size_t pl = PL_LDS_BYTES;
        FP_HIP(hipFuncSetAttribute((const void *)k_payload_lds, hipFuncAttributeMaxDynamicSharedMemorySize, (int)pl));
        k_payload_lds<<<S, PL_THREADS, pl, st>>>(C, order, b->req_labels, b->conflict, b->level, summ, s_req, s_conf,
                                                 s_idx);
        FP_HIP(hipGetLastError());
    } else if (ready) {
        size_t g = (SC + 1023) / 1024;
        if (g >= 64) g = (g + 7) & ~(size_t)7;
        k_gather_payload<<<(unsigned)g, 256, 0, st>>>(S, C, order, b->req_labels, b->conflict, b->level, summ,
                                                      s_req, s_conf, s_idx);
        FP_HIP(hipGetLastError());
    } else {
        size_t g = (SC + 1023) / 1024;
        if (g >= 64) g = (g + 7) & ~(size_t)7;
        if (key_bytes == 4)
            k_gather_sorted<uint32_t><<<(unsigned)g, 256, 0, st>>>(
                thr, kpack, S, C, order, (const uint32_t *)skeys, mbits, cmax, mmax, cval, mval, b->cpu_m, b->mem_mib, b->req_labels,
                b->conflict, b->level, summ, s_cpu, s_mem, s_req, s_conf, s_idx);
        else
            k_gather_sorted<uint64_t><<<(unsigned)g, 256, 0, st>>>(
                thr, kpack, S, C, order, (const uint64_t *)skeys, mbits, cmax, mmax, cval, mval, b->cpu_m, b->mem_mib, b->req_labels,
                b->conflict, b->level, summ, s_cpu, s_mem, s_req, s_conf, s_idx);
        FP_HIP(hipGetLastError());
    }
    PipeArgs a;
    a.C = C; a.N = N; a.scen_base = scen_base; a.W = W; a.G = G; a.R = R;
    a.B = B; a.slots = slots; a.bounded = geo.bounded; a.ticket = ctl; a.gabort = ctl + 32; a.ghead = ctl + 64;
    a.gdata = gdata;
    a.S = S;
    a.lag = geo.lag;
    a.kpack = kpack;
    a.flush = (geo.bounded ? 3u : 1u) & (uint32_t)fp_opt(c, FP_OPT_PIPE_FLUSH, 3);
    a.part = part;
    a.s_cpu = s_cpu; a.s_mem = s_mem; a.s_req = s_req; a.s_conf = s_conf; a.s_idx = s_idx;
    a.cf = b->cpu_free; a.mf = b->mem_free; a.lab = b->labels; a.cu = b->conflict_used; a.sched = b->schedulable;
    a.assign = asg_s; a.reason = rsn_s; a.cost = b->cost; a.err = c->d_err;
    a.spin_ticks = (uint64_t)fp_opt(c, FP_OPT_SPIN_TICKS, (int64_t)SPIN_TICKS);
    a.sys = geo.sys ? (geo.sys | (geo.sys_extra << 16)) : 0u;
    {
        const int64_t pv = fp_opt(c, FP_OPT_LINK_PUBLISH, S >= 4096 ? 32 : 8);
        a.publish = geo.bounded ? 1u : (uint32_t)(pv < 1 ? 1 : pv > 1024 ? 1024 : pv);
        uint32_t p2 = 1;
        while (p2 * 2 <= a.publish) p2 *= 2;
        a.pub_mask = p2 - 1;
    }
    a.thr = thr;
    a.prio = geo.prio;
    const bool wide = wide_g(W, G);
    if (G < 1 || (wide ? (G > MAX_G_WIDE || G % 4) : G > MAX_G)) return FP_EOVERFLOW;
    std::unique_lock<std::mutex> gate_lock;
    BoundedGate *gate = nullptr;
    if (geo.bounded) {
        if (c->device < 0 || c->device >= kMaxGateDevices) return FP_EINVAL;
        gate = &g_bounded_gate[c->device];
        gate_lock = std::unique_lock<std::mutex>(gate->m);
        if (!gate->ev) FP_HIP(hipEventCreateWithFlags(&gate->ev, hipEventDisableTiming));
        else FP_HIP(hipStreamWaitEvent(st, gate->ev, 0));
    }
    hipEvent_t ev;
    fp_prof_begin(c, FP_K_PLACE, &ev);
    int rc;
    a.rng = rng;
    if (pkfn) {
        a.pk_mode = 1;
        rc = u32fn(st, (unsigned)(S * B), W * 64, lds, a);
        if (!rc) {
            FP_HIP(hipGetLastError());
            a.pk_mode = 2;
            rc = pkfn(st, (unsigned)(S * B), W * 64, big ? geo.lds_big_pk : lds, a);
        }
    } else {
        a.pk_mode = 0;
        rc = u32fn(st, (unsigned)(S * B), W * 64, lds, a);
    }
    if (rc) return rc;
    FP_HIP(hipGetLastError());
    fp_prof_end(c, FP_K_PLACE, ev);
    if (gate) {
        FP_HIP(hipEventRecord(gate->ev, st));
        gate_lock.unlock();
    }
    {
        const bool narrow16 = N < 0xFFFFu;
        const uint32_t span = narrow16 ? UNSORT_SPAN16 : UNSORT_SPAN32;
        const uint32_t H = (C + span - 1) / span;
        const size_t ul = (size_t)span * (narrow16 ? 3 : 5);
        const void *fn = narrow16 ? (const void *)k_unsort<true> : (const void *)k_unsort<false>;
        FP_HIP(hipFuncSetAttribute(fn, hipFuncAttributeMaxDynamicSharedMemorySize, (int)ul));
        if (narrow16)
            k_unsort<true><<<(unsigned)(S * H), 1024, ul, st>>>(C, H, span, order, asg_s, rsn_s, b->assign, b->reason);
        else
            k_unsort<false><<<(unsigned)(S * H), 1024, ul, st>>>(C, H, span, order, asg_s, rsn_s, b->assign, b->reason);
        FP_HIP(hipGetLastError());
    }
    if (b->cost) {
        k_cost_reduce<<<(S + 255) / 256, 256, 0, st>>>(S, B, scen_base, part, b->cost);
        FP_HIP(hipGetLastError());
    }
    return FP_OK;
}

int fp_place_geometry_impl(fp_ctx *c, uint32_t S, uint32_t C, uint32_t N, uint32_t *out) {
    PipeGeom g;
    if (!pipe_geom(c, S, C, N, &g)) return FP_EOVERFLOW;
    const uint32_t v[FP_GEOM_COUNT] = {g.G, g.W, g.B, g.R, g.lag, g.slots, g.bounded, g.resident, g.sys};
    memcpy(out, v, sizeof(v));
    return FP_OK;
}
// ... 73 lines not shown
```

### fleetflow_amd/csrc/fp_pipe_tus.h

```cpp
#pragma once

#define FPP_TUS(X)            \
    X(big, 12, 64, 6, 0)      \
    X(bigp, 12, 64, 7, 1)     \
    X(w12, 12, 64, 0, 0)      \
    X(w12p, 12, 64, 0, 1)     \
    X(m8, 8, 1024, 0, 0)      \
    X(m8p, 8, 1024, 0, 1)     \
    X(m10, 10, 1024, 0, 0)    \
    X(m10p, 10, 1024, 0, 1)   \
    X(n1, 1, 1024, 0, 0)      \
    X(n1p, 1, 1024, 0, 1)
```

### fleetflow_amd/csrc/fp_place.hip

```cpp
#include "fp_internal.h"
#include "fp_payload.h"

namespace {

__device__ __forceinline__ void bounds_acc(uint32_t c, uint32_t m, uint32_t &mc, uint32_t &mm, uint32_t &lc,
                                           uint32_t &lm) {
    mc = max(mc, c);
    mm = max(mm, m);
    lc = c ? min(lc, c) : lc;
    lm = m ? min(lm, m) : lm;
}


constexpr uint32_t RANK_MAX_VALUE = 1u << 18;
constexpr uint32_t RANK_WORDS = RANK_MAX_VALUE / 32;

enum { CN_DC = 0, CN_DM = 1, CN_OVER = 6, CN_MAXC = 8, CN_MAXM = 9, CN_MINC = 10, CN_MINM = 11, CN_ORC = 12, CN_ORM = 13,
       CN_WORDS = 16 };
__global__ __launch_bounds__(256) void k_value_bitmap(const uint32_t *__restrict__ cpu,
                                                      const uint32_t *__restrict__ mem, size_t n,
                                                      uint32_t *__restrict__ gbc, uint32_t *__restrict__ gbm,
                                                      uint32_t *__restrict__ cnt) {
    extern __shared__ uint32_t lbm[];
    for (uint32_t i = threadIdx.x; i < 2 * RANK_WORDS; i += blockDim.x) lbm[i] = 0;
// ... 76 lines not shown
    for (uint32_t o = 1; o < blockDim.x; o <<= 1) {
        const uint32_t v = threadIdx.x >= o ? part[threadIdx.x - o] : 0u;
        __syncthreads();
        part[threadIdx.x] += v;
        __syncthreads();
    }
    uint32_t run = part[threadIdx.x] - local;
    for (uint32_t w = w0; w < w0 + per && w < nw; ++w) {
        pre[w] = run;
        uint32_t x = bm[w];
        while (x) {
            const uint32_t b = (uint32_t)__builtin_ctz(x);
            x &= x - 1;
            val[run++] = w * 32 + b;
        }
    }
    __syncthreads();
    if (threadIdx.x == blockDim.x - 1) {
        const uint32_t d = part[threadIdx.x];
        cnt[blockIdx.x] = d;
        cnt[2 + blockIdx.x] = d ? val[d - 1] : 0u;
        cnt[4 + blockIdx.x] = d == 0 ? 0xFFFFFFFFu : val[0] ? val[0] : d > 1 ? val[1] : 0xFFFFFFFFu;
    }
}

__global__ void k_fill_cost(uint32_t S, uint32_t scen_base, uint64_t *__restrict__ cost) {
    const uint32_t s = blockIdx.x * blockDim.x + threadIdx.x;
    if (s < S) cost[s] = fpd::pack_cost(0, 0, scen_base + s);
}

__global__ void k_argmin_cost(const uint64_t *__restrict__ cost, uint32_t n, uint32_t *best) {
    __shared__ uint64_t red[16];
    uint64_t m = ~0ull;
    uint32_t idx = 0xFFFFFFFFu;
    for (uint32_t i = threadIdx.x; i < n; i += blockDim.x) {
        if (cost[i] < m) { m = cost[i]; idx = i; }
    }
    for (int o = 32; o > 0; o >>= 1) {
        uint64_t om = __shfl_xor(m, o);
        uint32_t oi = __shfl_xor(idx, o);
        if (om < m || (om == m && oi < idx)) { m = om; idx = oi; }
    }
    __shared__ uint32_t redi[16];
    if ((threadIdx.x & 63) == 0) { red[threadIdx.x >> 6] = m; redi[threadIdx.x >> 6] = idx; }
    __syncthreads();
    if (threadIdx.x == 0) {
        uint64_t bm = ~0ull;
        uint32_t bi = 0xFFFFFFFFu;
        for (uint32_t w = 0; w < (blockDim.x + 63) / 64; ++w)
            if (red[w] < bm || (red[w] == bm && redi[w] < bi)) { bm = red[w]; bi = redi[w]; }
        *best = bi;
    }
}

constexpr uint32_t SS_DIG = 256;
constexpr uint32_t SS_WAVES = 16;
constexpr uint32_t SS_CHUNKS = 50;
constexpr uint32_t SS_LB = 25;
constexpr uint32_t SS_REG = 16;
constexpr size_t SS_LDS_CAP = 160 * 1024;
constexpr uint32_t SR_W = RANK_WORDS;
constexpr size_t SR_BYTES = (size_t)SR_W * (4 + 2) * 2;
constexpr size_t SS_TAB_BYTES = SS_DIG * (4 + 4 + 1 + 1);
constexpr size_t SS_IMG_BYTES = SR_BYTES + SS_TAB_BYTES;

__host__ __device__ static inline size_t ss_align16(size_t b) { return (b + 15) & ~(size_t)15; }
__host__ __device__ static inline size_t ss_xr_bytes(uint32_t C) {
    return ss_align16((size_t)C * 2 > SR_BYTES ? (size_t)C * 2 : SR_BYTES);
}
static inline size_t ss_lds_bytes(uint32_t C) {
    return ss_xr_bytes(C) + ss_align16(C) + SS_WAVES * SS_DIG * 2 + 2 * SS_DIG * 4 + 2 * SS_DIG * 4 + 2 * SS_DIG + 16;
}

struct ScenSortArgs {
    uint32_t C, kpack;
    const uint32_t *cpu, *mem;
    uint32_t *order, *s_cpu, *s_mem, *s_idx;
    const uint32_t *T;
    const uint32_t *scnt;
    const unsigned char *simg;
    uint32_t *rng;
    const uint32_t *req, *conf, *level, *summ;
    uint32_t *s_req, *s_conf;
};

typedef uint64_t __attribute__((may_alias)) ss_u64a;
typedef uint32_t __attribute__((may_alias)) ss_u32a;
typedef uint32_t ss_u32x4 __attribute__((ext_vector_type(4)));

__device__ __forceinline__ uint64_t ss_match(uint32_t v, bool valid, uint32_t nb) {
    uint64_t m = __builtin_amdgcn_ballot_w64(valid);
    for (uint32_t b = 0; b < nb; ++b) {
        const bool bit = (v >> b) & 1u;
        const uint64_t bb = __builtin_amdgcn_ballot_w64(bit);
        m &= bit ? bb : ~bb;
    }
    return m;
}

__device__ __forceinline__ uint32_t ss_bucket(const uint32_t *t, uint32_t v) {
    uint32_t k = 0;
#pragma unroll
    for (uint32_t step = FP_BUCKETS / 2; step; step >>= 1) k += t[k + step] <= v ? step : 0u;
    return k;
}

__device__ __forceinline__ void ss_inc16(uint16_t *row, uint32_t d) {
    atomicAdd(reinterpret_cast<ss_u32a *>(row) + (d >> 1), 1u << ((d & 1u) * 16u));
}

__device__ __forceinline__ void ss_row_scan(uint16_t *row, uint32_t lane, uint32_t base) {
    const uint64_t q = reinterpret_cast<ss_u64a *>(row)[lane];
    const uint32_t c0 = (uint32_t)(q & 0xFFFF), c1 = (uint32_t)((q >> 16) & 0xFFFF), c2 = (uint32_t)((q >> 32) & 0xFFFF);
    const uint32_t sum = c0 + c1 + c2 + (uint32_t)(q >> 48);
    uint32_t inc = sum;
#pragma unroll
    for (int o = 1; o < 64; o <<= 1) {
        const uint32_t y = (uint32_t)__shfl_up((int)inc, o);
        inc += lane >= (uint32_t)o ? y : 0u;
    }
    const uint64_t e0 = base + inc - sum;
    reinterpret_cast<ss_u64a *>(row)[lane] = e0 | ((e0 + c0) << 16) | ((e0 + c0 + c1) << 32) | ((e0 + c0 + c1 + c2) << 48);
}

__device__ __forceinline__ void ss_offsets(uint16_t *WH, uint32_t *HS, uint32_t *HB, uint32_t t, uint32_t lane,
                                           uint32_t w) {
    if (t < SS_DIG) {
        uint32_t s = 0;
#pragma unroll
        for (uint32_t ww = 0; ww < SS_WAVES; ++ww) s += WH[ww * SS_DIG + t];
        HB[t] = s;
    }
    __syncthreads();
    if (w == 0) {
        const uint32_t c0 = HB[4 * lane], c1 = HB[4 * lane + 1], c2 = HB[4 * lane + 2], c3 = HB[4 * lane + 3];
        const uint32_t sum = c0 + c1 + c2 + c3;
        uint32_t inc = sum;
#pragma unroll
        for (int o = 1; o < 64; o <<= 1) {
            const uint32_t y = (uint32_t)__shfl_up((int)inc, o);
            inc += lane >= (uint32_t)o ? y : 0u;
        }
        const uint32_t ex = inc - sum;
        HS[4 * lane] = ex;
        HS[4 * lane + 1] = ex + c0;
        HS[4 * lane + 2] = ex + c0 + c1;
        HS[4 * lane + 3] = ex + c0 + c1 + c2;
    }
    __syncthreads();
    if (t < SS_DIG) {
        uint32_t run = HS[t];
#pragma unroll
        for (uint32_t ww = 0; ww < SS_WAVES; ++ww) {
            const uint32_t c = WH[ww * SS_DIG + t];
            WH[ww * SS_DIG + t] = (uint16_t)run;
            run += c;
        }
        HB[t] = run;
    }
    __syncthreads();
}

__device__ void ss_generic(const ScenSortArgs &a, uint16_t *X, uint16_t *WH, uint32_t *HS, uint32_t *HB,
                           size_t cb, uint32_t C) {
    const uint32_t t = threadIdx.x, lane = t & 63, w = t >> 6;
    const uint64_t lt = (1ull << lane) - 1ull;
    const uint32_t L = (C + SS_WAVES - 1) / SS_WAVES;
    const uint32_t s0 = min(C, w * L), s1 = min(C, s0 + L);
    uint16_t *myrow = WH + w * SS_DIG;
    uint32_t *ord = a.order + cb;
    const uint32_t *cpu = a.cpu + cb, *mem = a.mem + cb;
    for (uint32_t k = 0; k < 8; ++k) {
        const uint32_t *key = k < 4 ? mem : cpu;
        const uint32_t sh = 8u * (k & 3u);
        auto src = [&](uint32_t p) -> uint32_t {
            return k == 0 ? p
                   : (k & 1u) ? (uint32_t)X[p]
                              : __hip_atomic_load(&ord[p], __ATOMIC_RELAXED, __HIP_MEMORY_SCOPE_AGENT);
        };
        for (uint32_t i = t; i < SS_WAVES * SS_DIG / 2; i += blockDim.x) reinterpret_cast<ss_u32a *>(WH)[i] = 0u;
        __syncthreads();
        for (uint32_t p = s0 + lane; p < s1; p += 64) ss_inc16(myrow, ((~key[src(p)]) >> sh) & 0xFFu);
        __syncthreads();
        ss_offsets(WH, HS, HB, t, lane, w);
        for (uint32_t p0 = s0; p0 < s1; p0 += 64) {
            const uint32_t p = p0 + lane;
            const bool valid = p < s1;
            const uint32_t j = valid ? src(p) : 0u;
            const uint32_t d = valid ? ((~key[j]) >> sh) & 0xFFu : 0u;
            const uint64_t m = ss_match(d, valid, 8);
            const uint32_t off = myrow[d];
            __builtin_amdgcn_fence(__ATOMIC_SEQ_CST, "wavefront");
            if (valid) {
                if ((m & lt) == 0) myrow[d] = (uint16_t)(off + __popcll(m));
                const uint32_t q = off + (uint32_t)__popcll(m & lt);
                if (k & 1u) ord[q] = j;
                else X[q] = (uint16_t)j;
            }
            __builtin_amdgcn_fence(__ATOMIC_SEQ_CST, "wavefront");
        }
        __syncthreads();
    }
    uint32_t oc = 0, om = 0;
    for (uint32_t P = t; P < C; P += blockDim.x) {
        const uint32_t j = __hip_atomic_load(&ord[P], __ATOMIC_RELAXED, __HIP_MEMORY_SCOPE_AGENT);
        const uint32_t cv = cpu[j], mv = mem[j];
        a.s_cpu[cb + P] = cv;
        a.s_mem[cb + P] = mv;
        a.s_idx[cb + P] = P | (a.kpack ? (ss_bucket(a.T, cv) << 21) | (ss_bucket(a.T + FP_BUCKETS, mv) << 26) : 0u);
        oc |= cv;
        om |= mv;
    }
    for (int o = 32; o > 0; o >>= 1) {
        oc |= (uint32_t)__shfl_xor((int)oc, o);
        om |= (uint32_t)__shfl_xor((int)om, o);
    }
    __syncthreads();
    if (t < 2) HS[t] = 0u;
    __syncthreads();
    if (lane == 0) {
        atomicOr(&HS[0], oc);
        atomicOr(&HS[1], om);
    }
    __syncthreads();
    if (t == 0) {
        fp_or_new_bits(&a.rng[0], HS[0]);
        fp_or_new_bits(&a.rng[1], HS[1]);
    }
}

#ifdef FP_PIPE_STATS
constexpr int SORT_STATS = 9;
__device__ unsigned long long g_sort_stats[SORT_STATS];
#define SS_CLK() __builtin_amdgcn_s_memtime()
#else
#define SS_CLK() 0ull
#endif

__device__ __forceinline__ uint32_t ss_block_excl(uint32_t v, uint32_t *part, uint32_t lane, uint32_t w,
                                                  uint32_t &total) {
    uint32_t inc = v;
#pragma unroll
    for (int o = 1; o < 64; o <<= 1) {
        const uint32_t y = (uint32_t)__shfl_up((int)inc, o);
        inc += lane >= (uint32_t)o ? y : 0u;
    }
    if (lane == 63) part[w] = inc;
    __syncthreads();
    uint32_t before = 0;
    total = 0;
#pragma unroll
    for (uint32_t ww = 0; ww < SS_WAVES; ++ww) {
        const uint32_t x = part[ww];
        before += ww < w ? x : 0u;
        total += x;
    }
    return before + inc - v;
}

template <bool FUSED>
__global__ __launch_bounds__(1024) void k_scen_sort(const ScenSortArgs a) {
    extern __shared__ __attribute__((aligned(16))) unsigned char ssm[];
    const uint32_t C = a.C;
    uint16_t *X = reinterpret_cast<uint16_t *>(ssm);
    uint8_t *LD = ssm + ss_xr_bytes(C);
    uint16_t *WH = reinterpret_cast<uint16_t *>(LD + ss_align16(C));
    uint32_t *HS = reinterpret_cast<uint32_t *>(WH + SS_WAVES * SS_DIG);
    uint32_t *HB = HS + SS_DIG;
    uint32_t *MV = HB + SS_DIG;
    uint32_t *CV = MV + SS_DIG;
    uint8_t *MB = reinterpret_cast<uint8_t *>(CV + SS_DIG);
    uint8_t *CB = MB + SS_DIG;
    uint32_t *NEXT = reinterpret_cast<uint32_t *>(CB + SS_DIG);
    uint32_t *BMC = reinterpret_cast<uint32_t *>(ssm), *BMM = BMC + SR_W;
    uint16_t *PRC = reinterpret_cast<uint16_t *>(BMM + SR_W), *PRM = PRC + SR_W;
    const uint32_t t = threadIdx.x, lane = t & 63, w = t >> 6;
    const uint64_t lt = (1ull << lane) - 1ull;
    const size_t cb = (size_t)blockIdx.x * C;
    const uint32_t *cpu = a.cpu + cb, *mem = a.mem + cb;
    const unsigned long long ck0 = SS_CLK();

    const uint32_t scd = a.scnt[CN_DC], scm = a.scnt[CN_DM];
    const bool samp = a.scnt[CN_OVER] == 0u && scd - 1u < SS_DIG && scm - 1u < SS_DIG;
    const uint32_t L = (C + SS_WAVES - 1) / SS_WAVES;
    const uint32_t s0 = min(C, w * L), s1 = min(C, s0 + L);
    uint16_t *myrow = WH + w * SS_DIG;
    uint32_t dc = 0, dm = 0, hbits = 0, lbits = 0;
    uint32_t dvp[SS_CHUNKS / 2];
    unsigned long long ck1 = 0;
    const __amdgpu_buffer_rsrc_t rc_cpu = __builtin_amdgcn_make_buffer_rsrc((void *)cpu, (short)0, (int)(4 * C), 0x00020000);
    const __amdgpu_buffer_rsrc_t rc_mem = __builtin_amdgcn_make_buffer_rsrc((void *)mem, (short)0, (int)(4 * C), 0x00020000);
    const uint32_t smc = a.scnt[2], smm = a.scnt[3];
    const uint32_t iwc = (smc >> 5) + 1u, iwm = (smm >> 5) + 1u;
    const uint32_t ib1 = (4u * iwc + 15u) / 16u, ib2 = ib1 + (4u * iwm + 15u) / 16u;
    const uint32_t ib3 = ib2 + (2u * iwc + 15u) / 16u, ib4 = ib3 + (2u * iwm + 15u) / 16u;
    const uint32_t img_units = ib4 + (uint32_t)(SS_TAB_BYTES / 16);
    const uint32_t tab_dst = (uint32_t)(reinterpret_cast<unsigned char *>(MV) - ssm);
    auto img_unit = [&](uint32_t u, uint32_t &dst) -> uint32_t {
        const uint32_t src = u < ib1   ? 16u * u
                             : u < ib2 ? 4u * SR_W + 16u * (u - ib1)
                             : u < ib3 ? 8u * SR_W + 16u * (u - ib2)
                             : u < ib4 ? 10u * SR_W + 16u * (u - ib3)
                                       : (uint32_t)SR_BYTES + 16u * (u - ib4);
        dst = u < ib4 ? src : tab_dst + 16u * (u - ib4);
        return src;
    };
    auto rank_pass = [&](const uint32_t pass) -> uint32_t {
        ss_u32x4 imv;
        uint32_t isrc = 0, idst = 0;
        uint32_t pcv[SS_LB], pmv[SS_LB];
        if (pass == 0) {
            isrc = img_unit(min(t, img_units - 1u), idst);
            imv = *reinterpret_cast<const ss_u32x4 *>(a.simg + isrc);
            __builtin_amdgcn_sched_barrier(0);
#pragma unroll
            for (uint32_t k = 0; k < SS_LB; ++k) {
                pcv[k] = __builtin_amdgcn_raw_buffer_load_b32(rc_cpu, (int)(4 * (s0 + lane)), (int)(256 * k), 0);
                pmv[k] = __builtin_amdgcn_raw_buffer_load_b32(rc_mem, (int)(4 * (s0 + lane)), (int)(256 * k), 0);
            }
        }
        for (uint32_t i = t; i < SS_WAVES * SS_DIG / 2; i += blockDim.x) reinterpret_cast<ss_u32a *>(WH)[i] = 0u;
        if (t < 4) NEXT[t] = 0u;
        if (pass == 0) {
            if (t < img_units) *reinterpret_cast<ss_u32x4 *>(ssm + idst) = imv;
            for (uint32_t u = t + 1024; u < img_units; u += 1024) {
                const uint32_t so = img_unit(u, idst);
                *reinterpret_cast<ss_u32x4 *>(ssm + idst) = *reinterpret_cast<const ss_u32x4 *>(a.simg + so);
            }
            dc = scd;
            dm = scm;
            __syncthreads();
        } else {
            for (uint32_t i = t; i < 2 * SR_W; i += blockDim.x) BMC[i] = 0u;
            __syncthreads();
            bool big = false;
            for (uint32_t k0 = 0; k0 < SS_CHUNKS; k0 += SS_LB) {
                uint32_t cv[SS_LB], mv[SS_LB];
#pragma unroll
                for (uint32_t k = 0; k < SS_LB; ++k) {
                    const uint32_t i = t + blockDim.x * (k0 + k);
                    cv[k] = i < C ? __builtin_nontemporal_load(&cpu[i]) : 0u;
                    mv[k] = i < C ? __builtin_nontemporal_load(&mem[i]) : 0u;
                }
#pragma unroll
                for (uint32_t k = 0; k < SS_LB; ++k) {
                    if (t + blockDim.x * (k0 + k) < C) {
                        const uint32_t c = cv[k], m = mv[k];
                        if ((c | m) >= RANK_MAX_VALUE) {
                            big = true;
                        } else {
                            const uint32_t bc = 1u << (c & 31), bm = 1u << (m & 31);
                            if (!(BMC[c >> 5] & bc)) atomicOr(&BMC[c >> 5], bc);
                            if (!(BMM[m >> 5] & bm)) atomicOr(&BMM[m >> 5], bm);
                        }
                    }
                }
            }
            if (__ballot(big) && lane == 0) atomicOr(&NEXT[1], 1u);
            __syncthreads();
            static_assert(SR_W == 8 * 1024, "rank words per thread");
            uint32_t bw[8], bx[8], sc = 0, sm = 0;
#pragma unroll
            for (uint32_t j = 0; j < 8; ++j) {
                bw[j] = BMC[8 * t + j];
                bx[j] = BMM[8 * t + j];
                sc += (uint32_t)__popc(bw[j]);
                sm += (uint32_t)__popc(bx[j]);
            }
            uint32_t pc = ss_block_excl(sc, HS, lane, w, dc);
            __syncthreads();
            uint32_t pm = ss_block_excl(sm, HB, lane, w, dm);
            const bool elig = NEXT[1] == 0u && dc >= 1u && dm >= 1u && dc <= SS_DIG && dm <= SS_DIG;
#pragma unroll
            for (uint32_t j = 0; j < 8; ++j) {
                PRC[8 * t + j] = (uint16_t)pc;
                PRM[8 * t + j] = (uint16_t)pm;
                if (elig) {
                    for (uint32_t x = bw[j]; x; x &= x - 1) CV[dc - 1u - pc++] = (8 * t + j) * 32 + (uint32_t)__builtin_ctz(x);
                    for (uint32_t x = bx[j]; x; x &= x - 1) MV[dm - 1u - pm++] = (8 * t + j) * 32 + (uint32_t)__builtin_ctz(x);
                } else {
                    pc += (uint32_t)__popc(bw[j]);
                    pm += (uint32_t)__popc(bx[j]);
                }
            }
            __syncthreads();
            if (!elig) {
                ss_generic(a, X, WH, HS, HB, cb, C);
                return 2u;
            }
            if (t < SS_DIG) {
                MB[t] = a.kpack && t < dm ? (uint8_t)ss_bucket(a.T + FP_BUCKETS, MV[t]) : 0;
                CB[t] = a.kpack && t < dc ? (uint8_t)ss_bucket(a.T, CV[t]) : 0;
            }
        }
        ck1 = SS_CLK();
        hbits = dc > 1 ? 32u - (uint32_t)__builtin_clz(dc - 1u) : 0u;
        lbits = dm > 1 ? 32u - (uint32_t)__builtin_clz(dm - 1u) : 0u;

        bool miss = false;
#pragma unroll
        for (uint32_t k = 0; k < SS_CHUNKS / 2; ++k) dvp[k] = 0u;
#pragma unroll
        for (uint32_t k0 = 0; k0 < SS_CHUNKS; k0 += SS_LB) {
            uint32_t cv[SS_LB], mv[SS_LB];
#pragma unroll
            for (uint32_t k = 0; k < SS_LB; ++k) {
                const uint32_t p = s0 + 64 * (k0 + k) + lane;
                if (pass == 0 && k0 == 0) {
                    cv[k] = pcv[k];
                    mv[k] = pmv[k];
                } else {
                    cv[k] = p < s1 ? __builtin_nontemporal_load(&cpu[p]) : 0u;
                    mv[k] = p < s1 ? __builtin_nontemporal_load(&mem[p]) : 0u;
                }
            }
#pragma unroll
            for (uint32_t k = 0; k < SS_LB; ++k) {
                const uint32_t p = s0 + 64 * (k0 + k) + lane;
                const uint32_t c = cv[k], m = mv[k];
                if (p < s1 && (pass == 0 ? c > smc || m > smm : (c | m) >= RANK_MAX_VALUE)) miss = true;
                else if (p < s1) {
                    const uint32_t wc = BMC[c >> 5], wm = BMM[m >> 5];
                    if ((((wc >> (c & 31)) & (wm >> (m & 31))) & 1u) == 0u) {
                        miss = true;
                    } else {
                        const uint32_t rc = PRC[c >> 5] + (uint32_t)__popc(wc & ((1u << (c & 31)) - 1u));
                        const uint32_t rm = PRM[m >> 5] + (uint32_t)__popc(wm & ((1u << (m & 31)) - 1u));
                        const uint32_t hd = dc - 1u - rc, ld = dm - 1u - rm;
                        LD[p] = (uint8_t)ld;
                        ss_inc16(myrow, hd);
                        dvp[(k0 + k) >> 1] |= hd << (16u * ((k0 + k) & 1u));
                    }
                }
            }
        }
        if (__ballot(miss) && lane == 0) atomicOr(&NEXT[2], 1u);
        __syncthreads();
        if (NEXT[2] == 0u) return 0u;
        __syncthreads();
        return 1u;
    };
    uint32_t rr = samp ? rank_pass(0u) : 1u;
    if (rr == 1u) rr = rank_pass(1u);
    if (!FUSED && rr == 2u) return;
    if (rr != 2u) {
        ss_offsets(WH, HS, HB, t, lane, w);
        const unsigned long long ck2 = SS_CLK();

#pragma unroll
        for (uint32_t k = 0; k < SS_CHUNKS; ++k) {
            const uint32_t p0 = s0 + 64 * k;
            if (p0 >= s1) break;
            const uint32_t p = p0 + lane;
            const bool valid = p < s1;
            const uint32_t d = (dvp[k >> 1] >> (16u * (k & 1u))) & 0xFFFFu;
            const uint64_t m = ss_match(d, valid, hbits);
            const uint32_t off = myrow[d];
            if (valid) {
                if ((m & lt) == 0) myrow[d] = (uint16_t)(off + __popcll(m));
                X[off + (uint32_t)__popcll(m & lt)] = (uint16_t)p;
            }
        }
        __syncthreads();
        const unsigned long long ck3 = SS_CLK();
        uint32_t big = 0;

        while (true) {
            uint32_t d = 0;
            if (lane == 0) d = atomicAdd(NEXT, 1u);
            d = (uint32_t)__shfl((int)d, 0);
            if (d >= dc) break;
            const uint32_t lo = HS[d], hi = HB[d];
            if (lo == hi) continue;
            big = max(big, hi - lo);
            reinterpret_cast<ss_u64a *>(myrow)[lane] = 0ull;
            __builtin_amdgcn_fence(__ATOMIC_SEQ_CST, "workgroup");
            const uint32_t cv = CV[d];
            const uint32_t kbc = a.kpack ? (uint32_t)CB[d] << 21 : 0u;
            if (hi - lo <= 64 * SS_REG) {
                uint32_t jv[SS_REG], lv[SS_REG];
#pragma unroll
                for (uint32_t k = 0; k < SS_REG; ++k) {
                    const uint32_t p = lo + 64 * k + lane;
                    jv[k] = p < hi ? X[p] : 0u;
                    lv[k] = p < hi ? LD[jv[k]] : 0u;
                    if (p < hi) ss_inc16(myrow, lv[k]);
                }
                __builtin_amdgcn_fence(__ATOMIC_SEQ_CST, "workgroup");
                ss_row_scan(myrow, lane, lo);
                __builtin_amdgcn_fence(__ATOMIC_SEQ_CST, "workgroup");
#pragma unroll
                for (uint32_t k = 0; k < SS_REG; ++k) {
                    if (lo + 64 * k >= hi) break;
                    const bool valid = lo + 64 * k + lane < hi;
                    const uint64_t m = ss_match(lv[k], valid, lbits);
                    const uint32_t off = myrow[lv[k]];
                    if (valid) {
                        if ((m & lt) == 0) myrow[lv[k]] = (uint16_t)(off + __popcll(m));
                        X[off + (uint32_t)__popcll(m & lt)] = (uint16_t)jv[k];
                    }
                }
                __builtin_amdgcn_fence(__ATOMIC_SEQ_CST, "workgroup");
                for (uint32_t P = lo + lane; P < hi; P += 64) {
                    const uint32_t j = X[P], l = LD[j];
                    a.order[cb + P] = j;
                    a.s_cpu[cb + P] = cv;
                    a.s_mem[cb + P] = MV[l];
                    a.s_idx[cb + P] = P | kbc | (a.kpack ? (uint32_t)MB[l] << 26 : 0u);
                }
            } else {
                if (FUSED && lane == 0) NEXT[3] = 1u;
#pragma unroll 4
                for (uint32_t p = lo + lane; p < hi; p += 64) ss_inc16(myrow, LD[X[p]]);
                __builtin_amdgcn_fence(__ATOMIC_SEQ_CST, "workgroup");
                ss_row_scan(myrow, lane, lo);
                __builtin_amdgcn_fence(__ATOMIC_SEQ_CST, "workgroup");
                for (uint32_t p0 = lo; p0 < hi; p0 += 64) {
                    const uint32_t p = p0 + lane;
                    const bool valid = p < hi;
                    const uint32_t j = valid ? X[p] : 0u;
                    const uint32_t l = valid ? LD[j] : 0u;
                    const uint64_t m = ss_match(l, valid, lbits);
                    const uint32_t off = myrow[l];
                    if (valid) {
                        if ((m & lt) == 0) myrow[l] = (uint16_t)(off + __popcll(m));
                        const uint32_t P = off + (uint32_t)__popcll(m & lt);
                        a.order[cb + P] = j;
                        a.s_cpu[cb + P] = cv;
                        a.s_mem[cb + P] = MV[l];
                        a.s_idx[cb + P] = P | kbc | (a.kpack ? (uint32_t)MB[l] << 26 : 0u);
                    }
                }
            }
            __builtin_amdgcn_fence(__ATOMIC_SEQ_CST, "workgroup");
        }
#ifdef FP_PIPE_STATS
        const unsigned long long ck4 = SS_CLK();
        if (lane == 0) {
            atomicAdd(&g_sort_stats[4], ck4 - ck3);
            atomicMax(&g_sort_stats[6], (unsigned long long)big);
        }
        __syncthreads();
        if (t == 0) {
            const unsigned long long ck5 = SS_CLK();
            atomicAdd(&g_sort_stats[0], ck1 - ck0);
            atomicAdd(&g_sort_stats[1], ck2 - ck1);
            atomicAdd(&g_sort_stats[2], ck3 - ck2);
            atomicAdd(&g_sort_stats[3], ck5 - ck3);
            atomicAdd(&g_sort_stats[5], 1ull);
            atomicAdd(&g_sort_stats[7], ck5 - ck0);
        }
#else
        (void)ck0; (void)ck1; (void)ck2; (void)ck3; (void)big;
#endif
        if (w == 0) {
            uint32_t oc = 0, om = 0;
            for (uint32_t i = lane; i < dc; i += 64) oc |= CV[i];
            for (uint32_t i = lane; i < dm; i += 64) om |= MV[i];
            for (int o = 32; o > 0; o >>= 1) {
                oc |= (uint32_t)__shfl_xor((int)oc, o);
                om |= (uint32_t)__shfl_xor((int)om, o);
            }
            if (lane == 0) {
                fp_or_new_bits(&a.rng[0], oc);
                fp_or_new_bits(&a.rng[1], om);
            }
        }
    }
    if constexpr (FUSED) {
        asm volatile("s_waitcnt vmcnt(0)" ::: "memory");
        __syncthreads();
        const unsigned long long ckp = SS_CLK();
        const bool from_x = rr != 2u && __builtin_amdgcn_readfirstlane((int)NEXT[3]) == 0;
        fpl::pl_by_field<true>(reinterpret_cast<uint32_t *>(ssm), C, a.order, X, from_x, a.req, a.conf, a.level, a.summ,
                               a.s_req, a.s_conf, a.s_idx);
#ifdef FP_PIPE_STATS
        __syncthreads();
        if (t == 0) atomicAdd(&g_sort_stats[8], SS_CLK() - ckp);
#else
        (void)ckp;
#endif
    }
}

__device__ void value_thresholds(const uint32_t *v, uint32_t d, uint32_t *T) {
    while (d && v[0] == 0) { ++v; --d; }
    T[0] = 0;
    for (int k = 1; k < FP_BUCKETS; ++k) {
        if (d == 0) { T[k] = 1; continue; }
        const uint64_t i = d <= (uint32_t)(FP_BUCKETS - 1) ? (uint64_t)(k - 1 < (int)d ? k - 1 : d - 1)
                                                             : (uint64_t)(k - 1) * (d - 1) / (FP_BUCKETS - 2);
        T[k] = v[i];
    }
}

__global__ void k_thresholds(uint32_t *__restrict__ cnt, const uint32_t *__restrict__ cval,
                             const uint32_t *__restrict__ mval, uint32_t *__restrict__ thr) {
    const uint32_t d = threadIdx.x;
    if (d > 1) return;
    const bool ranks = cnt[CN_OVER] == 0;
    uint32_t T[FP_BUCKETS];
    if (ranks) {
        value_thresholds(d ? mval : cval, cnt[d ? CN_DM : CN_DC], T);
    } else {
        const uint32_t lo = cnt[d ? CN_MINM : CN_MINC], hi = cnt[d ? CN_MAXM : CN_MAXC];
        fp_thresholds(lo == 0xFFFFFFFFu ? 1u : lo, hi, T);
    }
    for (int k = 0; k < FP_BUCKETS; ++k) thr[d * FP_BUCKETS + k] = T[k];
}

__global__ __launch_bounds__(1024) void k_sort_image(const uint32_t *__restrict__ bm, const uint32_t *__restrict__ pre,
                                                     const uint32_t *__restrict__ val, const uint32_t *__restrict__ cnt,
                                                     const uint32_t *__restrict__ T, uint32_t kpack,
                                                     unsigned char *__restrict__ img) {
    const uint32_t dc = cnt[CN_DC], dm = cnt[CN_DM], t = threadIdx.x;
    if (cnt[CN_OVER] != 0u || dc - 1u >= SS_DIG || dm - 1u >= SS_DIG) return;
    uint32_t *ibm = reinterpret_cast<uint32_t *>(img);
    uint16_t *ipr = reinterpret_cast<uint16_t *>(ibm + 2 * SR_W);
    for (uint32_t i = t; i < 2 * SR_W; i += blockDim.x) {
        ibm[i] = bm[i];
        ipr[i] = (uint16_t)pre[i];
    }
    uint32_t *mv = reinterpret_cast<uint32_t *>(img + SR_BYTES), *cv = mv + SS_DIG;
    uint8_t *mb = reinterpret_cast<uint8_t *>(cv + SS_DIG), *cbk = mb + SS_DIG;
    if (t < SS_DIG) {
        const uint32_t c = t < dc ? val[dc - 1u - t] : 0u, m = t < dm ? val[RANK_MAX_VALUE + dm - 1u - t] : 0u;
        cv[t] = c;
        mv[t] = m;
        cbk[t] = kpack && t < dc ? (uint8_t)ss_bucket(T, c) : 0;
        mb[t] = kpack && t < dm ? (uint8_t)ss_bucket(T + FP_BUCKETS, m) : 0;
    }
}

}

#ifdef FP_PIPE_STATS
extern "C" int fp_debug_sort_stats(unsigned long long *out, int reset) {
    if (hipMemcpyFromSymbol(out, HIP_SYMBOL(g_sort_stats), sizeof(unsigned long long) * SORT_STATS) != hipSuccess)
        return FP_EDEVICE;
    if (reset) {
        static const unsigned long long zero[SORT_STATS] = {0};
        if (hipMemcpyToSymbol(HIP_SYMBOL(g_sort_stats), zero, sizeof(zero)) != hipSuccess) return FP_EDEVICE;
    }
    return FP_OK;
}
#endif

constexpr uint32_t THR_SAMPLE = 8;

static int place_ws_need(fp_ctx *c, uint32_t S, uint32_t C, uint32_t N, size_t *need, fp_ffd_order *fo) {
    if (int rc = fp_ffd_order_size(c, S, C, 0, fo)) return rc;
    const size_t pipe_ws = fp_pipe_ws_bytes(c, S, C, N);
    if (pipe_ws == 0) return FP_EOVERFLOW;
    const size_t rank_ws = 2 * (2 * RANK_WORDS * 4 + RANK_MAX_VALUE * 4) + CN_WORDS * 4 + 2 * FP_BUCKETS * 4 + 3 * 256
                           + SS_IMG_BYTES + 256;
    *need = rank_ws + fo->bytes + pipe_ws + 2 * 256;
    return FP_OK;
}

int fp_place_ws_bytes_impl(fp_ctx *c, uint32_t S, uint32_t C, uint32_t N, uint64_t *bytes) {
    if (S == 0 || C == 0) { *bytes = 0; return FP_OK; }
    if ((size_t)S * C > 0xFFFFFFFFull) return FP_EOVERFLOW;
    size_t need = 0;
    fp_ffd_order fo;
    if (int rc = place_ws_need(c, S, C, N, &need, &fo)) return rc;
    *bytes = need;
    return FP_OK;
}

int fp_dev_place_batch_impl(fp_ctx *c, const fp_batch *b) {
    const uint32_t S = b->n_scen, C = b->n_containers, N = b->n_nodes;
    c->last_rng = nullptr;
    if (S == 0) return FP_OK;
    if ((uint64_t)b->scen_base + S > 65536ull) return FP_EOVERFLOW;
    hipStream_t st = c->stream;
    if (C == 0) {
        if (b->cost) {
            k_fill_cost<<<(S + 255) / 256, 256, 0, st>>>(S, b->scen_base, b->cost);
            FP_HIP(hipGetLastError());
        }
        return FP_OK;
    }
    const size_t SC = (size_t)S * C;
    if (SC > 0xFFFFFFFFull) return FP_EOVERFLOW;
    if (!b->cpu_m || !b->mem_mib || !b->req_labels || !b->conflict || !b->assign || !b->reason)
        return FP_EINVAL;
    if (N && (!b->cpu_free || !b->mem_free || !b->labels || !b->conflict_used || !b->schedulable))
        return FP_EINVAL;

    size_t need = 0;
    fp_ffd_order fo;
    if (int rc0 = place_ws_need(c, S, C, N, &need, &fo)) return rc0;
    int rc = fp_ws_reserve(c, need);
    if (rc) return rc;
    fp_ws_reset(c);
    uint32_t *rbm = (uint32_t *)fp_ws_take(c, 2 * RANK_WORDS * 4);
    uint32_t *rpre = (uint32_t *)fp_ws_take(c, 2 * RANK_WORDS * 4);
    uint32_t *rval = (uint32_t *)fp_ws_take(c, 2 * RANK_MAX_VALUE * 4);
    uint32_t *rcnt = (uint32_t *)fp_ws_take(c, CN_WORDS * 4);
    uint32_t *thr = (uint32_t *)fp_ws_take(c, 2 * FP_BUCKETS * 4);
    unsigned char *simg = (unsigned char *)fp_ws_take(c, SS_IMG_BYTES);
    if (!rbm || !rpre || !rval || !rcnt || !thr || !simg) return FP_ENOMEM;
    c->last_rng = rcnt + CN_ORC;

    hipEvent_t ev;
    fp_prof_begin(c, FP_K_SORT, &ev);
    FP_HIP(hipMemsetAsync(rbm, 0, 2 * RANK_WORDS * 4, st));
    FP_HIP(hipMemsetAsync(rcnt, 0, CN_WORDS * 4, st));
    FP_HIP(hipMemsetAsync(rcnt + CN_MINC, 0xFF, 8, st));
    {
        const size_t n = (size_t)(S < THR_SAMPLE ? S : THR_SAMPLE) * C;
        unsigned gb = grid_for((n + 3) / 4, 256);
        if (gb > 1024) gb = 1024;
        FP_HIP(hipFuncSetAttribute((const void *)k_value_bitmap, hipFuncAttributeMaxDynamicSharedMemorySize,
                                   (int)(2 * RANK_WORDS * 4)));
        k_value_bitmap<<<gb, 256, 2 * RANK_WORDS * 4, st>>>(b->cpu_m, b->mem_mib, n, rbm, rbm + RANK_WORDS, rcnt);
        FP_HIP(hipGetLastError());
        k_rank_tables<<<2, 1024, 0, st>>>(rbm, rbm + RANK_WORDS, RANK_WORDS, RANK_WORDS, rpre, rpre + RANK_WORDS, rval,
                                          rval + RANK_MAX_VALUE, rcnt);
        FP_HIP(hipGetLastError());
        k_thresholds<<<1, 64, 0, st>>>(rcnt, rval, rval + RANK_MAX_VALUE, thr);
        FP_HIP(hipGetLastError());
    }
    if (ss_lds_bytes(C) <= SS_LDS_CAP && C <= SS_WAVES * SS_CHUNKS * 64 && fp_opt(c, FP_OPT_SCEN_SORT, 1) != 0) {
        ScenSortArgs sa;
        sa.C = C; sa.kpack = fp_pipe_kpack(c, C);
        sa.cpu = b->cpu_m; sa.mem = b->mem_mib;
        fp_pipe_soa soa;
        if (int rs = fp_pipe_soa_take(c, SC, &soa)) return rs;
        uint32_t *order = (uint32_t *)fp_ws_take(c, SC * 4);
        if (!order) return FP_ENOMEM;
        sa.order = order; sa.s_cpu = soa.s_cpu; sa.s_mem = soa.s_mem; sa.s_idx = soa.s_idx;
        sa.T = thr;
        sa.scnt = rcnt;
        sa.rng = rcnt + CN_ORC;
        sa.simg = simg;
        k_sort_image<<<1, 1024, 0, st>>>(rbm, rpre, rval, rcnt, thr, sa.kpack, simg);
        FP_HIP(hipGetLastError());
        const bool fused = FPP_PAYLOAD_BY_FIELD && fp_opt(c, FP_OPT_SORT_FUSED, 1) != 0 && C <= fp_pipe_payload_lds_max_c(c);
        size_t lds = ss_lds_bytes(C);
        if (fused) {
            if (int rs = fp_pipe_node_summary(c, S, C, N, b, sa.rng, &soa.summ)) return rs;
            soa.payload_done = true;
            sa.req = b->req_labels; sa.conf = b->conflict; sa.level = b->level; sa.summ = soa.summ;
            sa.s_req = soa.s_req; sa.s_conf = soa.s_conf;
            if (lds < fpl::PL_FIELD_LDS_BYTES) lds = fpl::PL_FIELD_LDS_BYTES;
            static_assert(fpl::PL_FIELD_LDS_BYTES <= SS_LDS_CAP, "the chunk buffer fits the sort's LDS");
            FP_HIP(hipFuncSetAttribute((const void *)k_scen_sort<true>, hipFuncAttributeMaxDynamicSharedMemorySize, (int)lds));
            k_scen_sort<true><<<S, 1024, lds, st>>>(sa);
        } else {
            sa.req = sa.conf = sa.level = sa.summ = nullptr;
            sa.s_req = sa.s_conf = nullptr;
            FP_HIP(hipFuncSetAttribute((const void *)k_scen_sort<false>, hipFuncAttributeMaxDynamicSharedMemorySize, (int)lds));
            k_scen_sort<false><<<S, 1024, lds, st>>>(sa);
        }
        FP_HIP(hipGetLastError());
        fp_prof_end(c, FP_K_SORT, ev);
        return fp_pipe_launch(c, S, C, N, b->scen_base, order, nullptr, 4, 0, 0, 0, rval, rval + RANK_MAX_VALUE, b,
                              thr, &soa, rcnt + CN_ORC);
    }
    const uint64_t full = 0xFFFFFFFFull;
    if (int rs = fp_ffd_order_run(c, S, C, b->cpu_m, b->mem_mib, rcnt + CN_ORC, &fo)) return rs;
    fp_prof_end(c, FP_K_SORT, ev);
    return fp_pipe_launch(c, S, C, N, b->scen_base, fo.order, fo.keys_out, 8, 32, full, full, nullptr, nullptr, b, thr,
                          nullptr, rcnt + CN_ORC);
}

extern "C" int fp_ctx_place_path(fp_ctx *c, uint32_t *out3) {
    if (!c || !out3) return FP_EINVAL;
    out3[0] = out3[1] = out3[2] = 0u;
    if (!c->last_rng) return FP_OK;
    FP_HIP(hipSetDevice(c->device));
    FP_HIP(hipStreamSynchronize(c->stream));
    FP_HIP(hipMemcpy(out3, c->last_rng, 12, hipMemcpyDeviceToHost));
    return FP_OK;
}

extern "C" int fp_dev_argmin_cost(fp_ctx *c, const uint64_t *cost, uint32_t n, uint32_t *best) {
    if (!c || !cost || !best || n == 0) return FP_EINVAL;
    FP_HIP(hipSetDevice(c->device));
    k_argmin_cost<<<1, 1024, 0, c->stream>>>(cost, n, best);
    return fp_dev_done(c, hipGetLastError() == hipSuccess ? FP_OK : FP_EDEVICE);
}
```

### fleetflow_amd/planner.py

```python
from __future__ import annotations

import ctypes as ct
from dataclasses import dataclass
from types import SimpleNamespace

import numpy as np

from . import _lib
from ._lib import FpBatch, FpContainers, FpGraph, FpNodes, check

NONE = _lib.FP_NONE


def _u32(a):
    return np.ascontiguousarray(a, dtype=np.uint32)


def _u8(a):
    return np.ascontiguousarray(a, dtype=np.uint8)


def _ptr(a):
    return None if a is None else a.ctypes.data

# ... 185 lines not shown
    return int(strategy)


class Planner:
    def __init__(self, device: int = 0):
        self._L = _lib.load()
        h = ct.c_void_p()
        check(self._L.fp_ctx_create(ct.byref(h), device), "fp_ctx_create")
        self._ctx = h
        self.device = device
        self._tstream = None

    def close(self):
        if getattr(self, "_ctx", None):
            if getattr(self, "_tstream", None) is not None:
                self._L.fp_ctx_reset_stream(self._ctx)
                self._tstream = None
            self._L.fp_ctx_destroy(self._ctx)
            self._ctx = None
            self._fs = None

    def __del__(self):
        try:
            self.close()
        except Exception:
            pass

    def __enter__(self):
        return self

    def __exit__(self, *exc):
        self.close()

    def set_stream(self, hip_stream_handle: int):
        check(self._L.fp_ctx_set_stream(self._ctx, ct.c_void_p(int(hip_stream_handle))), "fp_ctx_set_stream")
        import torch
        self._tstream = torch.cuda.ExternalStream(int(hip_stream_handle), device=torch.device("cuda", self.device))

    def reset_stream(self):
        check(self._L.fp_ctx_reset_stream(self._ctx), "fp_ctx_reset_stream")
        self._tstream = None

    def _dev(self, fn, *args):
        import torch
        cur = torch.cuda.current_stream(self.device)
        if self._tstream is None:
            st = torch.cuda.Stream(device=torch.device("cuda", self.device))
            check(self._L.fp_ctx_set_stream(self._ctx, ct.c_void_p(st.cuda_stream)), "fp_ctx_set_stream")
            self._tstream = st
        if self._tstream.cuda_stream == cur.cuda_stream:
            return fn(*args)
        self._tstream.wait_stream(cur)
        try:
            return fn(*args)
        finally:
            cur.wait_stream(self._tstream)

    def sync(self):
        check(self._L.fp_ctx_sync(self._ctx), "fp_ctx_sync")

    def profile(self, enable=True):
        check(self._L.fp_ctx_profile(self._ctx, int(enable)), "fp_ctx_profile")

    def set_option(self, name: str, value: int = _lib.FP_OPT_AUTO):
        check(self._L.fp_ctx_set_option(self._ctx, _lib.OPTIONS[name], int(value)), f"fp_ctx_set_option({name})")

    def get_option(self, name: str) -> int:
        v = ct.c_int64()
        check(self._L.fp_ctx_get_option(self._ctx, _lib.OPTIONS[name], ct.byref(v)), f"fp_ctx_get_option({name})")
        return int(v.value)

    def reset_options(self):
        for name in _lib.OPTIONS:
            self.set_option(name, _lib.FP_OPT_AUTO)

    def geometry(self, S: int, C: int, N: int) -> dict:
        out = (ct.c_uint32 * len(_lib.GEOM_FIELDS))()
        check(self._L.fp_place_geometry(self._ctx, S, C, N, out), "fp_place_geometry")
        return dict(zip(_lib.GEOM_FIELDS, (int(x) for x in out)))

    def place_path(self) -> dict:
        out = (ct.c_uint32 * 3)()
        check(self._L.fp_ctx_place_path(self._ctx, out), "fp_ctx_place_path")
        return {"or_cpu": int(out[0]), "or_mem": int(out[1]), "packed": int(out[2]) == 2, "ran": int(out[2]) != 0}

    def kernel_stats(self, kernel_id: int):
        ms = ct.c_double()
        n = ct.c_uint64()
        check(self._L.fp_ctx_kernel_stats(self._ctx, kernel_id, ct.byref(ms), ct.byref(n)), "kernel_stats")
        return ms.value, n.value

    _need = staticmethod(_need)
    _relax_row = staticmethod(_relax_row)
    _quota_rows = staticmethod(_quota_rows)

    def legacy_order(self, has_deps):
        hd = _u8(has_deps)
        out = np.empty(hd.size, np.uint32)
        g = FpGraph(hd.size, 0, None, None, _ptr(hd))
        check(self._L.fp_legacy_order(self._ctx, ct.byref(g), out.ctypes.data_as(_lib.u32p)), "fp_legacy_order")
        return out

    def levelize(self, row_ptr, col, has_deps):
        rp, cl, hd = _u32(row_ptr), _u32(col), _u8(has_deps)
        V = hd.size
        self._need(V == 0 or rp.size == V + 1, "row_ptr must hold V + 1 entries")
        level = np.empty(V, np.uint32)
        order = np.empty(V, np.uint32)
        ncyc = ct.c_uint32()
        g = FpGraph(V, cl.size, _ptr(rp), _ptr(cl) if cl.size else None, _ptr(hd))
        check(self._L.fp_levelize(self._ctx, ct.byref(g), level.ctypes.data_as(_lib.u32p),
                                  order.ctypes.data_as(_lib.u32p), ct.byref(ncyc)), "fp_levelize")
        return level, order, ncyc.value

    def plan_stage_lists(self, row_ptr, col, has_deps):
        V, E = len(has_deps), len(col)
        self._need(V == 0 or len(row_ptr) == V + 1, "row_ptr must hold V + 1 entries")
        fs = getattr(self, "_fs", None)
        if fs is None or V > fs["V"] or E > fs["E"] or fs["args"][0] is not self._ctx:
            cv, ce = max(64, V), max(256, E)
            rp, cl, hd = (ct.c_uint32 * (cv + 1))(), (ct.c_uint32 * ce)(), (ct.c_uint8 * cv)()
            out, ncyc = (ct.c_uint32 * (3 * cv))(), ct.c_uint32()
            g = FpGraph(0, 0, ct.addressof(rp), ct.addressof(cl), ct.addressof(hd))
            a = ct.addressof(out)
            args = (self._ctx, ct.byref(g), None, None, ct.c_void_p(a), ct.c_void_p(a + 4 * cv),
                    ct.c_void_p(a + 8 * cv), ct.byref(ncyc), None, None, None, None)
            fs = self._fs = {"V": cv, "E": ce, "rp": rp, "col": cl, "hd": hd, "out": out, "ncyc": ncyc, "g": g,
                             "args": args, "fn": _lib.raw_function("fp_plan_stage")}
        if V == 0:
            return [], [], [], 0
        fs["rp"][:V + 1] = row_ptr
        if E:
            fs["col"][:E] = col
        fs["hd"][:V] = has_deps
        g = fs["g"]
        g.n_vertices = V
        g.n_edges = E
        check(fs["fn"](*fs["args"]), "fp_plan_stage")
        out, cv = fs["out"], fs["V"]
        return out[:V], out[cv:cv + V], out[2 * cv:2 * cv + V], fs["ncyc"].value

    def plan_stage(self, row_ptr, col, has_deps, cont=None, nodes=None):
        rp, cl, hd = _u32(row_ptr), _u32(col), _u8(has_deps)
        V = hd.size
        self._need(V == 0 or rp.size == V + 1, "row_ptr must hold V + 1 entries")
        out = np.empty(3 * V, np.uint32)
        perm, level, order = out[:V], out[V:2 * V], out[2 * V:]
        o = out.ctypes.data
        ncyc = ct.c_uint32()
        g = FpGraph(V, cl.size, rp.ctypes.data, cl.ctypes.data if cl.size else None, hd.ctypes.data)
        if nodes is None:
            check(self._L.fp_plan_stage(self._ctx, ct.byref(g), None, None, o, o + 4 * V, o + 8 * V, ct.byref(ncyc),
                                        None, None, None, None), "fp_plan_stage")
            return perm, level, order, ncyc.value, None
        cont, nodes = _tables(cont, nodes, V, None, True, ("V", "N"))
        first = np.empty(V, np.uint32)
        count = np.empty(V, np.uint32)
        assign = np.empty(V, np.uint32)
        reason = np.empty(V, np.uint8)
        cs, ns = _pair(cont, nodes)
        check(self._L.fp_plan_stage(self._ctx, ct.byref(g), ct.byref(cs), ct.byref(ns), o, o + 4 * V, o + 8 * V,
                                    ct.byref(ncyc), first.ctypes.data, count.ctypes.data, assign.ctypes.data,
                                    reason.ctypes.data), "fp_plan_stage")
        return perm, level, order, ncyc.value, (first, count, assign, reason, nodes)

    def place(self, cont, nodes, level=None):
        cont, nodes = _tables(cont, nodes, None, None, True)
# ... 655 lines not shown
```

### include/fleetplace.h

```cpp
#ifndef FLEETPLACE_H
#define FLEETPLACE_H
#include <stdint.h>
#include <stddef.h>

#ifdef __cplusplus
extern "C" {
#endif

#define FP_ABI_VERSION 1

#define FP_OK 0
#define FP_EINVAL (-1)
#define FP_ENOMEM (-2)
#define FP_EDEVICE (-3)
#define FP_EOVERFLOW (-4)
#define FP_ECORRUPT (-5)

#define FP_NONE 0xFFFFFFFFu

enum fp_reason { FP_REASON_OK = 0, FP_REASON_NOFIT = 1, FP_REASON_CYCLE = 2, FP_REASON_SKEW = 3, FP_REASON_QUOTA = 4 };

typedef struct fp_ctx fp_ctx;

typedef struct {
    uint32_t n_vertices, n_edges;
    const uint32_t *row_ptr;
    const uint32_t *col;
    const uint8_t *has_deps;
} fp_graph;

typedef struct {
    uint32_t n;
    const uint32_t *cpu_m, *mem_mib, *req_labels, *conflict;
} fp_containers;

typedef struct {
    uint32_t n;
    uint32_t *cpu_free, *mem_free;
    const uint32_t *labels;
    uint32_t *conflict_used;
    const uint8_t *schedulable;
} fp_nodes;

typedef struct {
    uint32_t n_scen, scen_base;
    uint32_t n_containers, n_nodes;
    const uint32_t *cpu_m, *mem_mib, *req_labels, *conflict;
    const uint32_t *level;
    uint32_t *cpu_free, *mem_free;
    const uint32_t *labels;
    uint32_t *conflict_used;
    const uint8_t *schedulable;
    uint32_t *assign;
    uint8_t *reason;
    uint64_t *cost;
} fp_batch;

int fp_ctx_create(fp_ctx **out, int device);
void fp_ctx_destroy(fp_ctx *ctx);
int fp_ctx_set_stream(fp_ctx *ctx, void *hip_stream);
int fp_ctx_reset_stream(fp_ctx *ctx);
int fp_ctx_sync(fp_ctx *ctx);
const char *fp_strerror(int code);
int fp_abi_version(void);
enum { FP_K_PLACE = 0, FP_K_SORT = 1, FP_K_FEAS = 2, FP_K_LEVEL = 3, FP_K_GEN = 4, FP_K_COUNT = 5 };
int fp_ctx_profile(fp_ctx *ctx, int enable);
int fp_ctx_kernel_stats(fp_ctx *ctx, int kernel_id, double *total_ms, uint64_t *launches);
int fp_ctx_place_path(fp_ctx *ctx, uint32_t *out3);

#define FP_OPT_AUTO (-1)
enum fp_option {
    FP_OPT_PIPE_W = 0,
    FP_OPT_PIPE_SEG = 1,
    FP_OPT_PIPE_R = 2,
    FP_OPT_PIPE_LAG = 3,
    FP_OPT_LINK_SLOTS = 4,
    FP_OPT_LINK_BOUNDED = 5,
    FP_OPT_PIPE_FLUSH = 6,
    FP_OPT_SPIN_TICKS = 7,
    FP_OPT_KPACK = 8,
    FP_OPT_SCEN_SORT = 9,
    FP_OPT_SEGSORT = 10,
    FP_OPT_SYSTOLIC = 11,
    FP_OPT_LEVELIZE_SYNC = 12,
    FP_OPT_SYSTOLIC_EXTRA = 13,
    FP_OPT_SCREEN = 14,
    FP_OPT_PAYLOAD_LDS = 15,
    FP_OPT_SYSTOLIC_VALU = 16,
    FP_OPT_LINK_PUBLISH = 17,
    FP_OPT_LEVEL_SORT = 18,
    FP_OPT_LEVEL_SMALL = 19,
    FP_OPT_PIPE_PRIO = 20,
    FP_OPT_INDEG_BIN = 21,
    FP_OPT_PACKED = 22,
    FP_OPT_SORT_FUSED = 23,
    FP_OPT_COUNT = 24
};
int fp_ctx_set_option(fp_ctx *ctx, int option, int64_t value);
int fp_ctx_get_option(fp_ctx *ctx, int option, int64_t *value);

int fp_legacy_order(fp_ctx *ctx, const fp_graph *g, uint32_t *perm_out);
int fp_levelize(fp_ctx *ctx, const fp_graph *g, uint32_t *level_out, uint32_t *order_out,
                uint32_t *n_cycle_out);
int fp_place(fp_ctx *ctx, const fp_containers *c, fp_nodes *nodes, const uint32_t *level,
             uint32_t *assign_out, uint8_t *reason_out);
int fp_place_batch(fp_ctx *ctx, const fp_batch *b);
enum fp_strategy { FP_STRATEGY_FIRST_FIT = 0, FP_STRATEGY_SPREAD = 1, FP_STRATEGY_PACK = 2, FP_STRATEGY_FILL_LOWEST = 3 };
#define FP_POLICY_MAX_NODES 8192
int fp_place_policy(fp_ctx *ctx, const fp_containers *c, fp_nodes *nodes, const uint32_t *level,
                    uint32_t strategy, uint32_t preferred_labels, uint32_t *node_count,
                    uint32_t *assign_out, uint8_t *reason_out);
int fp_place_batch_policy(fp_ctx *ctx, const fp_batch *b, const uint32_t *strategy,
                          const uint32_t *preferred_labels, uint32_t *node_count);
#define FP_SPREAD_MAX_DOMAINS 64
int fp_place_policy_spread(fp_ctx *ctx, const fp_containers *c, fp_nodes *nodes, const uint32_t *level,
                           uint32_t strategy, uint32_t preferred_labels, uint32_t *node_count,
                           const uint32_t *domain, uint32_t max_skew, uint32_t *assign_out, uint8_t *reason_out);
int fp_place_batch_policy_spread(fp_ctx *ctx, const fp_batch *b, const uint32_t *strategy,
                                 const uint32_t *preferred_labels, uint32_t *node_count, const uint32_t *domain,
                                 const uint32_t *max_skew);
#define FP_FALLBACK_MAX_HOPS 4
int fp_place_policy_fallback(fp_ctx *ctx, const fp_containers *c, fp_nodes *nodes, const uint32_t *level,
                             uint32_t strategy, uint32_t preferred_labels, uint32_t *node_count,
                             const uint32_t *domain, uint32_t max_skew, const uint32_t *relax_mask, uint32_t n_hops,
                             uint32_t *assign_out, uint8_t *reason_out, uint8_t *hops_out);
int fp_place_batch_policy_fallback(fp_ctx *ctx, const fp_batch *b, const uint32_t *strategy,
                                   const uint32_t *preferred_labels, uint32_t *node_count, const uint32_t *domain,
                                   const uint32_t *max_skew, const uint32_t *relax_mask, const uint32_t *n_hops,
                                   uint8_t *hops_out);
enum fp_quota_dim { FP_QUOTA_CPU = 0, FP_QUOTA_MEM = 1, FP_QUOTA_SERVICES = 2, FP_QUOTA_DIMS = 3 };
#define FP_QUOTA_UNLIMITED 0xFFFFFFFFu
int fp_place_policy_quota(fp_ctx *ctx, const fp_containers *c, fp_nodes *nodes, const uint32_t *level,
                          uint32_t strategy, uint32_t preferred_labels, uint32_t *node_count,
                          const uint32_t *domain, uint32_t max_skew, const uint32_t *relax_mask, uint32_t n_hops,
                          uint32_t *assign_out, uint8_t *reason_out, uint8_t *hops_out, const uint32_t *quota,
                          uint32_t *quota_used, uint8_t *quota_why_out);
int fp_place_batch_policy_quota(fp_ctx *ctx, const fp_batch *b, const uint32_t *strategy,
                                const uint32_t *preferred_labels, uint32_t *node_count, const uint32_t *domain,
                                const uint32_t *max_skew, const uint32_t *relax_mask, const uint32_t *n_hops,
                                uint8_t *hops_out, const uint32_t *quota, uint32_t *quota_used,
                                uint8_t *quota_why_out);
int fp_feasibility(fp_ctx *ctx, const fp_containers *c, const fp_nodes *nodes,
                   uint32_t *first_out, uint32_t *count_out, uint64_t *bitmap_out);
enum fp_why { FP_WHY_CORDON = 1, FP_WHY_CPU = 2, FP_WHY_MEM = 4, FP_WHY_LABEL = 8, FP_WHY_CONFLICT = 16 };
enum { FP_EXPLAIN_FAIL = 0, FP_EXPLAIN_ONLY = 5, FP_EXPLAIN_FEASIBLE = 10, FP_EXPLAIN_ALL = 11,
       FP_EXPLAIN_MISSING = 12, FP_EXPLAIN_NEAR = 13, FP_EXPLAIN_WORDS = 16 };
enum { FP_EXPLAIN_HIST_MIXED = 5, FP_EXPLAIN_HIST_FITS = 6, FP_EXPLAIN_HIST_SELECTED = 7, FP_EXPLAIN_HIST_WORDS = 8 };
int fp_explain(fp_ctx *ctx, const fp_containers *c, const fp_nodes *nodes, const uint32_t *sel, uint32_t n_sel,
               uint32_t ignore_labels, uint32_t *rows_out);
int fp_explain_batch(fp_ctx *ctx, const fp_batch *b, uint32_t reason_mask, const uint32_t *ignore_labels,
                     uint32_t *hist_out);
enum { FP_DRAIN_EVICTED = 0, FP_DRAIN_STRANDED = 1, FP_DRAIN_STRANDED_CPU = 2, FP_DRAIN_STRANDED_MEM = 3,
       FP_DRAIN_TARGETS = 4, FP_DRAIN_FIRST_STRANDED = 5, FP_DRAIN_NODES = 6, FP_DRAIN_WORDS = 8 };
int fp_drain_sweep(fp_ctx *ctx, const fp_containers *c, const fp_nodes *nodes, const uint32_t *assign,
                   const uint32_t *group, uint32_t n_cand, uint32_t strategy, uint32_t preferred_labels,
                   const uint32_t *node_count, uint32_t *assign_out, uint8_t *reason_out, uint32_t *summary_out);
enum { FP_DRAIN_STRANDED_SKEW, FP_DRAIN_RELAXED, FP_DRAIN_SKEW_BEFORE, FP_DRAIN_SKEW_AFTER,
       FP_DRAIN_POLICY_WORDS  };
int fp_drain_sweep_policy(fp_ctx *ctx, const fp_containers *c, const fp_nodes *nodes, const uint32_t *assign,
                          const uint32_t *group, uint32_t n_cand, uint32_t strategy, uint32_t preferred_labels,
                          const uint32_t *node_count, const uint32_t *domain, uint32_t max_skew,
                          const uint32_t *relax_mask, uint32_t n_hops, uint32_t *assign_out, uint8_t *reason_out,
                          uint8_t *hops_out, uint32_t *summary_out, uint32_t *policy_out);
enum { FP_SHRINK_RELEASED = 0, FP_SHRINK_TRIED = 1, FP_SHRINK_FAILED = 2, FP_SHRINK_MOVES = 3, FP_SHRINK_MOVED = 4,
       FP_SHRINK_MOVED_CPU = 5, FP_SHRINK_MOVED_MEM = 6, FP_SHRINK_FIRST_FAILED = 7, FP_SHRINK_WORDS = 8 };
enum { FP_SHRINK_STATE_NEVER = 0, FP_SHRINK_STATE_RELEASED = 1, FP_SHRINK_STATE_FAILED = 2 };
int fp_shrink_sweep(fp_ctx *ctx, const fp_containers *c, const fp_nodes *nodes, const uint32_t *assign,
                    const uint32_t *try_order, uint32_t n_var, uint32_t n_try, uint32_t strategy,
                    uint32_t preferred_labels, const uint32_t *node_count, uint32_t *assign_out, uint8_t *state_out,
                    uint32_t *blocker_out, uint32_t *summary_out);
enum { FP_SHRINK_FAILED_SKEW, FP_SHRINK_RELAXED, FP_SHRINK_SKEW_BEFORE, FP_SHRINK_SKEW_AFTER,
       FP_SHRINK_POLICY_WORDS  };
int fp_shrink_sweep_policy(fp_ctx *ctx, const fp_containers *c, const fp_nodes *nodes, const uint32_t *assign,
                           const uint32_t *try_order, uint32_t n_var, uint32_t n_try, uint32_t strategy,
                           uint32_t preferred_labels, const uint32_t *node_count, const uint32_t *domain,
                           uint32_t max_skew, const uint32_t *relax_mask, uint32_t n_hops, uint32_t *assign_out,
                           uint8_t *state_out, uint32_t *blocker_out, uint32_t *summary_out, uint8_t *hops_out,
                           uint8_t *blocker_reason_out, uint32_t *policy_out);
enum { FP_REBAL_MOVES = 0, FP_REBAL_STUCK = 1, FP_REBAL_STUCK_SKEW = 2, FP_REBAL_RELAXED = 3, FP_REBAL_MOVED_CPU = 4,
// ... 128 lines not shown
```

### integration/fleetflow-placement/src/ffi.rs

```rust
#![allow(non_camel_case_types)]
use std::os::raw::{c_char, c_int, c_void};

pub const FP_ABI_VERSION: c_int = 1;
pub const FP_OK: c_int = 0;
pub const FP_EINVAL: c_int = -1;
pub const FP_ENOMEM: c_int = -2;
pub const FP_EDEVICE: c_int = -3;
pub const FP_EOVERFLOW: c_int = -4;
pub const FP_ECORRUPT: c_int = -5;
pub const FP_NONE: u32 = 0xFFFF_FFFF;
pub const FP_REASON_OK: u8 = 0;
pub const FP_REASON_NOFIT: u8 = 1;
pub const FP_REASON_CYCLE: u8 = 2;
pub const FP_REASON_SKEW: u8 = 3;
pub const FP_REASON_QUOTA: u8 = 4;
pub const FP_STRATEGY_FIRST_FIT: u32 = 0;
pub const FP_STRATEGY_SPREAD: u32 = 1;
pub const FP_STRATEGY_PACK: u32 = 2;
pub const FP_STRATEGY_FILL_LOWEST: u32 = 3;
pub const FP_POLICY_MAX_NODES: u32 = 8192;
pub const FP_SPREAD_MAX_DOMAINS: u32 = 64;
pub const FP_FALLBACK_MAX_HOPS: u32 = 4;
pub const FP_QUOTA_CPU: usize = 0;
pub const FP_QUOTA_MEM: usize = 1;
// ... 35 lines not shown
pub const FP_SHRINK_WORDS: usize = 8;
pub const FP_REBAL_MOVES: usize = 0;
pub const FP_REBAL_STUCK: usize = 1;
pub const FP_REBAL_STUCK_SKEW: usize = 2;
pub const FP_REBAL_RELAXED: usize = 3;
pub const FP_REBAL_MOVED_CPU: usize = 4;
pub const FP_REBAL_MOVED_MEM: usize = 5;
pub const FP_REBAL_SKEW_BEFORE: usize = 6;
pub const FP_REBAL_SKEW_AFTER: usize = 7;
pub const FP_REBAL_WORDS: usize = 8;
pub const FP_SHRINK_STATE_NEVER: u8 = 0;
pub const FP_SHRINK_STATE_RELEASED: u8 = 1;
pub const FP_SHRINK_STATE_FAILED: u8 = 2;
pub const FP_DRAIN_STRANDED_SKEW: usize = 0;
pub const FP_DRAIN_RELAXED: usize = 1;
pub const FP_DRAIN_SKEW_BEFORE: usize = 2;
pub const FP_DRAIN_SKEW_AFTER: usize = 3;
pub const FP_DRAIN_POLICY_WORDS: usize = 4;
pub const FP_SHRINK_FAILED_SKEW: usize = 0;
pub const FP_SHRINK_RELAXED: usize = 1;
pub const FP_SHRINK_SKEW_BEFORE: usize = 2;
pub const FP_SHRINK_SKEW_AFTER: usize = 3;
pub const FP_SHRINK_POLICY_WORDS: usize = 4;
pub const FP_GROW_PENDING: usize = 0;
pub const FP_GROW_PLACED: usize = 1;
pub const FP_GROW_OPENED: usize = 2;
pub const FP_GROW_UNPLACEABLE: usize = 3;
pub const FP_GROW_CAPPED: usize = 4;
pub const FP_GROW_LEFT_CPU: usize = 5;
pub const FP_GROW_LEFT_MEM: usize = 6;
pub const FP_GROW_FIRST_UNPLACED: usize = 7;
pub const FP_GROW_WORDS: usize = 8;
pub const FP_GROW_MAX_NEW: u32 = 8192;
pub const FP_GROW_ON_LIVE: usize = 0;
pub const FP_GROW_RELAXED: usize = 1;
pub const FP_GROW_STUCK_SKEW: usize = 2;
pub const FP_GROW_STUCK_QUOTA: usize = 3;
pub const FP_GROW_SKEW_BEFORE: usize = 4;
pub const FP_GROW_SKEW_AFTER: usize = 5;
pub const FP_GROW_POLICY_WORDS: usize = 8;
pub const FP_CHANGE_KEPT: u8 = 0;
pub const FP_CHANGE_NEW: u8 = 1;
pub const FP_CHANGE_MOVED: u8 = 2;
pub const FP_CHANGE_LOST: u8 = 3;
pub const FP_CHANGE_ABSENT: u8 = 4;
pub const FP_REPLAN_KEPT: usize = 0;
pub const FP_REPLAN_NEW: usize = 1;
pub const FP_REPLAN_MOVED: usize = 2;
pub const FP_REPLAN_LOST: usize = 3;
pub const FP_REPLAN_ABSENT: usize = 4;
pub const FP_REPLAN_MOVED_CPU: usize = 5;
pub const FP_REPLAN_MOVED_MEM: usize = 6;
pub const FP_REPLAN_WORDS: usize = 8;
pub const FP_K_PLACE: c_int = 0;
pub const FP_K_SORT: c_int = 1;
pub const FP_K_FEAS: c_int = 2;
pub const FP_K_LEVEL: c_int = 3;
pub const FP_K_GEN: c_int = 4;
pub const FP_OPT_AUTO: i64 = -1;
pub const FP_OPT_PIPE_W: c_int = 0;
pub const FP_OPT_PIPE_SEG: c_int = 1;
pub const FP_OPT_PIPE_R: c_int = 2;
pub const FP_OPT_PIPE_LAG: c_int = 3;
pub const FP_OPT_LINK_SLOTS: c_int = 4;
pub const FP_OPT_LINK_BOUNDED: c_int = 5;
pub const FP_OPT_PIPE_FLUSH: c_int = 6;
pub const FP_OPT_SPIN_TICKS: c_int = 7;
pub const FP_OPT_KPACK: c_int = 8;
pub const FP_OPT_SCEN_SORT: c_int = 9;
pub const FP_OPT_SEGSORT: c_int = 10;
pub const FP_OPT_SYSTOLIC: c_int = 11;
pub const FP_OPT_LEVELIZE_SYNC: c_int = 12;
pub const FP_OPT_SYSTOLIC_EXTRA: c_int = 13;
pub const FP_OPT_SCREEN: c_int = 14;
pub const FP_OPT_PAYLOAD_LDS: c_int = 15;
pub const FP_OPT_SYSTOLIC_VALU: c_int = 16;
pub const FP_OPT_LINK_PUBLISH: c_int = 17;
pub const FP_OPT_LEVEL_SORT: c_int = 18;
pub const FP_OPT_LEVEL_SMALL: c_int = 19;
pub const FP_OPT_PIPE_PRIO: c_int = 20;
pub const FP_OPT_INDEG_BIN: c_int = 21;
pub const FP_OPT_PACKED: c_int = 22;
pub const FP_OPT_SORT_FUSED: c_int = 23;
pub const FP_GEOM_GROUPS: usize = 0;
pub const FP_GEOM_STAGES: usize = 1;
pub const FP_GEOM_SEGMENTS: usize = 2;
pub const FP_GEOM_RING: usize = 3;
pub const FP_GEOM_LAG: usize = 4;
pub const FP_GEOM_LINK_SLOTS: usize = 5;
pub const FP_GEOM_BOUNDED: usize = 6;
pub const FP_GEOM_RESIDENT: usize = 7;
pub const FP_GEOM_SYSTOLIC: usize = 8;
pub const FP_GEOM_COUNT: usize = 9;

#[repr(C)]
pub struct fp_ctx {
    _private: [u8; 0],
}

#[repr(C)]
pub struct fp_graph {
    pub n_vertices: u32,
    pub n_edges: u32,
    pub row_ptr: *const u32,
    pub col: *const u32,
    pub has_deps: *const u8,
}

#[repr(C)]
pub struct fp_containers {
    pub n: u32,
    pub cpu_m: *const u32,
    pub mem_mib: *const u32,
    pub req_labels: *const u32,
    pub conflict: *const u32,
}

#[repr(C)]
pub struct fp_nodes {
    pub n: u32,
    pub cpu_free: *mut u32,
    pub mem_free: *mut u32,
    pub labels: *const u32,
    pub conflict_used: *mut u32,
    pub schedulable: *const u8,
}

#[repr(C)]
pub struct fp_batch {
    pub n_scen: u32,
    pub scen_base: u32,
    pub n_containers: u32,
    pub n_nodes: u32,
    pub cpu_m: *const u32,
    pub mem_mib: *const u32,
    pub req_labels: *const u32,
    pub conflict: *const u32,
    pub level: *const u32,
    pub cpu_free: *mut u32,
    pub mem_free: *mut u32,
    pub labels: *const u32,
    pub conflict_used: *mut u32,
    pub schedulable: *const u8,
    pub assign: *mut u32,
    pub reason: *mut u8,
    pub cost: *mut u64,
}

#[link(name = "fleetplace")]
unsafe extern "C" {
    pub fn fp_ctx_create(out: *mut *mut fp_ctx, device: c_int) -> c_int;
    pub fn fp_ctx_destroy(ctx: *mut fp_ctx);
    pub fn fp_ctx_set_stream(ctx: *mut fp_ctx, hip_stream: *mut c_void) -> c_int;
    pub fn fp_ctx_reset_stream(ctx: *mut fp_ctx) -> c_int;
    pub fn fp_ctx_sync(ctx: *mut fp_ctx) -> c_int;
    pub fn fp_strerror(code: c_int) -> *const c_char;
    pub fn fp_abi_version() -> c_int;
    pub fn fp_ctx_profile(ctx: *mut fp_ctx, enable: c_int) -> c_int;
    pub fn fp_ctx_kernel_stats(ctx: *mut fp_ctx, kernel_id: c_int, total_ms: *mut f64, launches: *mut u64) -> c_int;
    pub fn fp_ctx_place_path(ctx: *mut fp_ctx, out3: *mut u32) -> c_int;
    pub fn fp_ctx_set_option(ctx: *mut fp_ctx, option: c_int, value: i64) -> c_int;
    pub fn fp_ctx_get_option(ctx: *mut fp_ctx, option: c_int, value: *mut i64) -> c_int;

    pub fn fp_legacy_order(ctx: *mut fp_ctx, g: *const fp_graph, perm_out: *mut u32) -> c_int;
    pub fn fp_levelize(ctx: *mut fp_ctx, g: *const fp_graph, level_out: *mut u32, order_out: *mut u32,
                       n_cycle_out: *mut u32) -> c_int;
// ... 174 lines not shown
```

Measured before the change: 81720 billion.

## Prepack cpu/mem into one word in the fused sort for the bigp FFD pipe

The fused scenario sort now writes cpu and mem as a single shifted 16:16 word into s_cpu when the per-scenario OR ranges fit, storing shift headers per scenario. It skips the s_mem and s_idx writes, and the skip bit moves into the same word. A new bigp kernel variant (PW) reads only that packed word per container, which cuts the sort's write traffic and the pipe's read traffic. A repair kernel unpacks rows when the global range check disagrees. The cost is extra template instantiations, header and summary bookkeeping, and a fallback path.

```diff
diff --git a/fleetflow_amd/_lib.py b/fleetflow_amd/_lib.py
--- a/fleetflow_amd/_lib.py
+++ b/fleetflow_amd/_lib.py
@@ -53,7 +53,7 @@
            "pipe_flush": 6, "spin_ticks": 7, "kpack": 8, "scen_sort": 9, "segsort": 10, "systolic": 11,
            "levelize_sync": 12, "systolic_extra": 13, "screen": 14, "payload_lds": 15, "systolic_valu": 16, "link_publish": 17,
            "level_sort": 18, "level_small": 19, "pipe_prio": 20,
-           "indeg_bin": 21, "packed": 22, "sort_fused": 23}
+           "indeg_bin": 21, "packed": 22, "sort_fused": 23, "prepack": 24}
 GEOM_FIELDS = ("groups", "stages", "segments", "ring", "lag", "link_slots", "bounded", "resident", "systolic")
 
 u8p = ct.POINTER(ct.c_uint8)
diff --git a/fleetflow_amd/csrc/fp_internal.h b/fleetflow_amd/csrc/fp_internal.h
--- a/fleetflow_amd/csrc/fp_internal.h
+++ b/fleetflow_amd/csrc/fp_internal.h
@@ -243,8 +243,15 @@
     uint32_t *s_cpu, *s_mem, *s_req, *s_conf, *s_idx;
     uint32_t *summ = nullptr;
     bool payload_done = false;
+    uint32_t *pkhdr = nullptr;
 };
 int fp_pipe_soa_take(fp_ctx *c, size_t SC, fp_pipe_soa *soa);
+bool fp_pipe_prepack(fp_ctx *c, uint32_t S, uint32_t C, uint32_t N);
+__host__ __device__ static inline bool fp_pk_shifts(uint32_t orc, uint32_t orm, uint32_t *sc_c, uint32_t *sc_m) {
+    *sc_c = orc ? (uint32_t)__builtin_ctz(orc) : 0u;
+    *sc_m = orm ? (uint32_t)__builtin_ctz(orm) : 0u;
+    return (orc >> *sc_c) <= 0x7FFFu && (orm >> *sc_m) <= 0x7FFFu;
+}
 uint32_t fp_pipe_kpack(const fp_ctx *c, uint32_t C);
 int fp_pipe_node_summary(fp_ctx *c, uint32_t S, uint32_t C, uint32_t N, const fp_batch *b, uint32_t *rng,
                          uint32_t **summ);
diff --git a/fleetflow_amd/csrc/fp_payload.h b/fleetflow_amd/csrc/fp_payload.h
--- a/fleetflow_amd/csrc/fp_payload.h
+++ b/fleetflow_amd/csrc/fp_payload.h
@@ -69,7 +69,7 @@
 __device__ __forceinline__ void pl_by_field(uint32_t *pl_lds, uint32_t C, const uint32_t *order, const uint16_t *X,
                                             bool from_x, const uint32_t *req, const uint32_t *conf,
                                             const uint32_t *level, const uint32_t *summ, uint32_t *s_req,
-                                            uint32_t *s_conf, uint32_t *s_idx) {
+                                            uint32_t *s_conf, uint32_t *s_skip) {
     const uint32_t t = threadIdx.x;
     const size_t cb = (size_t)blockIdx.x * C;
     const uint32_t sm0 = summ ? summ[(size_t)blockIdx.x * 4] : 0xFFFFFFFFu;
@@ -109,7 +109,7 @@
     pl_pick_field(pl_lds, req + cb, C, o, v);
     uint32_t tr = t, Cr = C;
     asm volatile("" : "+v"(tr), "+s"(Cr));
-    uint32_t *const d_req = s_req + cb, *const d_idx = s_idx + cb;
+    uint32_t *const d_req = s_req + cb, *const d_idx = s_skip + cb;
 #pragma unroll
     for (uint32_t j = 0; j < PL_ROWS; ++j) {
         const uint32_t p = tr + PL_THREADS * j;
diff --git a/fleetflow_amd/csrc/fp_pipe.hip b/fleetflow_amd/csrc/fp_pipe.hip
--- a/fleetflow_amd/csrc/fp_pipe.hip
+++ b/fleetflow_amd/csrc/fp_pipe.hip
@@ -81,6 +81,7 @@
     uint32_t prio;
     uint32_t *rng;
     uint32_t pk_mode;
+    const uint32_t *pkhdr;
 };
 
 __device__ __forceinline__ uint32_t lds_acq(uint32_t *p) {
@@ -220,6 +221,13 @@
 #ifndef FPP_BIGP_LAZY
 #define FPP_BIGP_LAZY 2
 #endif
+#ifndef FPP_PREPACK
+#define FPP_PREPACK 1
+#endif
+#ifndef FPP_PREPACK_FFD
+#define FPP_PREPACK_FFD 1
+#endif
+constexpr bool PREPACK_OK = FPP_PREPACK && FPP_BIGP_NOMASK && FPP_BIGP_LAZY != 0 && FPP_LOOKAHEAD == 3;
 constexpr uint32_t BIGP_WV = 7;
 constexpr bool is_bigp(uint32_t G, uint32_t BLK, uint32_t WV, bool PK) {
     return G == 12 && BLK == 64 && WV == BIGP_WV && PK;
@@ -390,13 +398,14 @@
 #define FPP_BIG_S 4096
 #endif
 [[maybe_unused]] constexpr uint32_t WIDE12_BIG_WAVES = FPP_BIG_WAVES, WIDE12_BIG_S = FPP_BIG_S;
-template <uint32_t G, uint32_t BLK, uint32_t WV = 0, bool PK = false>
+template <uint32_t G, uint32_t BLK, uint32_t WV = 0, bool PK = false, bool PW = false>
 __global__ __launch_bounds__(BLK, BLK == 64 ? (is_bigp(G, BLK, WV, PK) ? FPP_BIGP_WAVES
                                                 : WV   ? WV
                                                 : G == 12 ? WIDE12_WAVES
                                                           : WIDE_WAVES)
                                                : 1) void
 k_ffd_pipe(const PipeArgs a_arg) {
+    static_assert(!PW || is_bigp(G, BLK, WV, PK), "prepacked input: bigp alone (launched only when PREPACK_OK)");
 #if defined(__HIP_DEVICE_COMPILE__)
     const PipeArgs &a = *(const PipeArgs *)__builtin_amdgcn_kernarg_segment_ptr();
 #else
@@ -428,7 +437,7 @@
         const bool packs = (orc >> sc_c) <= PK_FIELD_MAX && (orm >> sc_m) <= PK_FIELD_MAX;
         if (packs != PK) return;
     }
-    if (blockIdx.x == 0 && threadIdx.x == 0 && a.rng) a.rng[2] = PK ? 2u : 1u;
+    if (blockIdx.x == 0 && threadIdx.x == 0 && a.rng) a.rng[2] = PK ? (PW ? 3u : 2u) : 1u;
     for (uint32_t i = threadIdx.x; i < (W - 1) * 8 + 8; i += blockDim.x) CTL[i] = 0;
     __syncthreads();
     if (threadIdx.x == 0) {
@@ -452,6 +461,10 @@
     if (tk == 0xFFFFFFFFu) return;
     const uint32_t b = tk % B, s = tk / B - b * a.lag;
     const size_t cb = (size_t)s * C, nb = (size_t)s * N;
+    if constexpr (PW) {
+        sc_c = __builtin_amdgcn_readfirstlane(a.pkhdr[(size_t)s * 4]);
+        sc_m = __builtin_amdgcn_readfirstlane(a.pkhdr[(size_t)s * 4 + 1]);
+    }
 
     static_assert(K == 32, "mask/threshold lane layout assumes K == 32");
     const uint32_t my_t = NM ? 0u : a.thr[lane];
@@ -532,6 +545,7 @@
     [[maybe_unused]] uint32_t la_n = 0, la_pos = 0;
     [[maybe_unused]] bool la_ok = false;
     constexpr bool DB = BLK == 64 && G == 12 && PK && FPP_LOOKAHEAD >= 3, DB_EARLY = DB && FPP_LOOKAHEAD == 3;
+    static_assert(!PW || !PREPACK_OK || DB_EARLY, "prepacked input needs the early double buffer");
     [[maybe_unused]] uint32_t nf_cpu = 0, nf_mem = 0, nf_req = 0, nf_conf = 0, nf_idx = 0, nf_n = 0;
     [[maybe_unused]] bool nf_ok = false;
     [[maybe_unused]] uint32_t la2_n = 0, la2_pos = 0;
@@ -549,15 +563,18 @@
             nf_ok = true;                                                                               \
         }                                                                                               \
         const size_t o_ = cb + off_;                                                                    \
-        nf_cpu = g_ld_w(a.s_cpu + o_);                                                                  \
-        nf_mem = g_ld_w(a.s_mem + o_);                                                                  \
+        nf_cpu = g_ld_w(a.s_cpu + o_);         \
+        if constexpr (!PW) nf_mem = g_ld_w(a.s_mem + o_);                                               \
         nf_req = g_ld_w(a.s_req + o_);                                                                  \
         nf_conf = g_ld_w(a.s_conf + o_);                                                                \
-        if (!g_in) nf_idx = g_ld_w(a.s_idx + o_);                                                       \
-        else if (!DB_EARLY) nf_idx = la_pos;                                                            \
+        if constexpr (!PW) {         \
+            if (!g_in) nf_idx = g_ld_w(a.s_idx + o_);                                                   \
+            else if (!DB_EARLY) nf_idx = la_pos;                                                        \
+        }                                                                                               \
         if (DB_EARLY && g_in) {  \
             la_ok = itail + 1u < ihead_seen;                                                            \
-            const uint32_t *sn_ = la_ok ? gin_data + (size_t)GSLOT(itail + 1u) * LSLOT : a.s_idx + cb;  \
+            const uint32_t *sn_ = la_ok ? gin_data + (size_t)GSLOT(itail + 1u) * LSLOT                  \
+                                        : (PW ? a.s_cpu : a.s_idx) + cb;                                \
             la2_n = g_ld(sn_);                                                                          \
             la2_pos = g_ld(sn_ + (la_ok ? 64u + lane : 0u));                                            \
         }                                                                                               \
@@ -631,7 +648,7 @@
             if (DB && nf_ok) {
                 idx = valid ? pos : 0u;
                 cpu = valid ? nf_cpu : 0u;
-                mem = valid ? nf_mem : 0u;
+                if constexpr (!PW) mem = valid ? nf_mem : 0u;
                 req = valid ? nf_req : 0u;
                 conf = valid ? nf_conf : 0u;
             } else {
@@ -639,7 +656,7 @@
                     idx = pos;
                     const uint32_t p = pos & pmask;
                     cpu = a.s_cpu[cb + p];
-                    mem = a.s_mem[cb + p];
+                    if constexpr (!PW) mem = a.s_mem[cb + p];
                     req = a.s_req[cb + p];
                     conf = a.s_conf[cb + p];
                 }
@@ -652,21 +669,22 @@
             valid = i < C;
             if (DB && nf_ok) {
                 cpu = valid ? nf_cpu : 0u;
-                mem = valid ? nf_mem : 0u;
+                if constexpr (!PW) mem = valid ? nf_mem : 0u;
                 req = valid ? nf_req : 0u;
                 conf = valid ? nf_conf : 0u;
-                idx = valid ? nf_idx : 0u;
+                if constexpr (!PW) idx = valid ? nf_idx : 0u;
             } else {
                 if (valid) {
                     cpu = a.s_cpu[cb + i];
-                    mem = a.s_mem[cb + i];
+                    if constexpr (!PW) mem = a.s_mem[cb + i];
                     req = a.s_req[cb + i];
                     conf = a.s_conf[cb + i];
-                    idx = a.s_idx[cb + i];
+                    if constexpr (!PW) idx = a.s_idx[cb + i];
                 }
                 if constexpr (DB) __builtin_amdgcn_s_waitcnt(VMCNT0);
             }
-            const bool cyc = valid && (idx & CYC);
+            if constexpr (PW) idx = valid ? i : 0u;
+            const bool cyc = valid && ((PW ? cpu : idx) & CYC);
             if (cyc) {
                 const uint32_t j = idx & pmask;
                 a.assign[cb + j] = FP_NONE;
@@ -737,10 +755,18 @@
 #endif
 
         const uint64_t vm = __builtin_amdgcn_ballot_w64(valid);
-        const uint32_t qc = vm ? __builtin_amdgcn_readlane(cpu, 63 - __builtin_clzll(vm)) : 0xFFFFFFFFu;
-        const uint32_t qm = wave_min(valid ? mem : 0xFFFFFFFFu);
-        const uint32_t cw = PK ? pk_pack(cpu, mem, sc_c, sc_m) : 0u;
-        const uint32_t qw = PK ? pk_pack(qc, qm, sc_c, sc_m) : 0u;
+        uint32_t qc, qm, cw, qw;
+        if constexpr (PW) {
+            cw = valid ? cpu : 0u;
+            qc = qm = 0u;
+            const uint32_t ql = wave_min(valid ? cw & 0xFFFFu : 0xFFFFFFFFu);
+            qw = vm ? (__builtin_amdgcn_readlane(cw, 63 - __builtin_clzll(vm)) & 0xFFFF0000u) | ql : PK_GUARD;
+        } else {
+            qc = vm ? __builtin_amdgcn_readlane(cpu, 63 - __builtin_clzll(vm)) : 0xFFFFFFFFu;
+            qm = wave_min(valid ? mem : 0xFFFFFFFFu);
+            cw = PK ? pk_pack(cpu, mem, sc_c, sc_m) : 0u;
+            qw = PK ? pk_pack(qc, qm, sc_c, sc_m) : 0u;
+        }
         [[maybe_unused]] bool zero_early = false;
         if constexpr (DB_EARLY) {
             zero_early = valid && (cpu | mem | req | conf) == 0u;
@@ -1094,6 +1120,10 @@
         if (RANGE) {
             fp_or_new_bits(&rng[0], oc);
             fp_or_new_bits(&rng[1], om);
+            if (SUMM) {
+                summ[(size_t)blockIdx.x * 4 + 2] = oc;
+                summ[(size_t)blockIdx.x * 4 + 3] = om;
+            }
         }
     }
 }
@@ -1311,6 +1341,36 @@
 }
 #endif
 
+__global__ __launch_bounds__(1024) void k_unpack_rows(uint32_t C, uint32_t kpack, uint32_t all,
+                                                      const uint32_t *__restrict__ hdr, uint32_t *rng,
+                                                      const uint32_t *__restrict__ thr, uint32_t *__restrict__ s_cpu,
+                                                      uint32_t *__restrict__ s_mem, uint32_t *__restrict__ s_idx) {
+    const uint32_t s = blockIdx.x;
+    if (hdr[(size_t)s * 4 + 2] == 0u) return;
+    uint32_t bc, bm;
+    if (!all && fp_pk_shifts(rng[0], rng[1], &bc, &bm)) return;
+    const uint32_t sc_c = hdr[(size_t)s * 4], sc_m = hdr[(size_t)s * 4 + 1];
+    if (threadIdx.x == 0) atomicAdd(&rng[3], 1u);
+    __shared__ uint32_t T[2 * K];
+    if (threadIdx.x < 2 * K) T[threadIdx.x] = kpack ? thr[threadIdx.x] : 0u;
+    __syncthreads();
+    auto bucket = [](const uint32_t *t, uint32_t v) {
+        uint32_t k = 0;
+#pragma unroll
+        for (uint32_t step = K / 2; step; step >>= 1) k += t[k + step] <= v ? step : 0u;
+        return k;
+    };
+    const size_t cb = (size_t)s * C;
+    for (uint32_t P = threadIdx.x; P < C; P += blockDim.x) {
+        const uint32_t w = s_cpu[cb + P];
+        const uint32_t cv = pk_cpu(w & ~CYC, sc_c), mv = pk_mem(w, sc_m);
+        const uint32_t kb = kpack ? (bucket(T, cv) << 21) | (bucket(T + K, mv) << 26) : 0u;
+        s_cpu[cb + P] = cv;
+        s_mem[cb + P] = mv;
+        s_idx[cb + P] = P | kb | (w & CYC);
+    }
+}
+
 constexpr uint32_t UNSORT_SPAN16 = 50 * 1024;
 constexpr uint32_t UNSORT_SPAN32 = 30 * 1024;
 template <bool NARROW>
@@ -1357,12 +1417,13 @@
 }
 size_t lds_bytes_bigp(uint32_t R) { return FPP_BIGP_NOMASK ? 8 * 4 : lds_bytes(1, 12, R); }
 
-template <uint32_t G, uint32_t BLK = 1024, uint32_t WV = 0, bool PK = false>
+template <uint32_t G, uint32_t BLK = 1024, uint32_t WV = 0, bool PK = false, bool PW = false>
 static int launch_g(hipStream_t st, unsigned grid, unsigned block, size_t lds, const PipeArgs &a) {
     if (block > BLK) return FP_EINVAL;
-    FP_HIP(hipFuncSetAttribute((const void *)k_ffd_pipe<G, BLK, WV, PK>, hipFuncAttributeMaxDynamicSharedMemorySize,
+    if (PW && !a.pkhdr) return FP_EINVAL;
+    FP_HIP(hipFuncSetAttribute((const void *)k_ffd_pipe<G, BLK, WV, PK, PW>, hipFuncAttributeMaxDynamicSharedMemorySize,
                                (int)lds));
-    k_ffd_pipe<G, BLK, WV, PK><<<grid, block, lds, st>>>(a);
+    k_ffd_pipe<G, BLK, WV, PK, PW><<<grid, block, lds, st>>>(a);
     return FP_OK;
 }
 
@@ -1391,7 +1452,8 @@
      ::fpp_tu_kernel_##name},
 #else
 #define FPP_TU_ENTRY(name, G, BLK, WV, PK) \
-    {G, BLK, WV, PK, launch_g<G, BLK, WV, (bool)PK>, [] { return (const void *)k_ffd_pipe<G, BLK, WV, (bool)PK>; }},
+    {G, BLK, WV, PK, launch_g<G, BLK, WV, (PK) != 0, (PK) == 2>,                          \
+     [] { return (const void *)k_ffd_pipe<G, BLK, WV, (PK) != 0, (PK) == 2>; }},
 #endif
 static const TuKernel kTu[] = {FPP_TUS(FPP_TU_ENTRY)};
 #undef FPP_TU_ENTRY
@@ -1400,9 +1462,9 @@
     return false FPP_TUS(FPP_TU_IS);
 #undef FPP_TU_IS
 }
-static const TuKernel *tu_find(uint32_t G, uint32_t BLK, uint32_t WV, bool PK) {
+static const TuKernel *tu_find(uint32_t G, uint32_t BLK, uint32_t WV, bool PK, bool PW = false) {
     for (const TuKernel &k : kTu)
-        if (k.G == G && k.BLK == BLK && k.WV == WV && (k.PK != 0) == PK) return &k;
+        if (k.G == G && k.BLK == BLK && k.WV == WV && k.PK == (PK ? (PW ? 2u : 1u) : 0u)) return &k;
     return nullptr;
 }
 template <uint32_t G, uint32_t BLK = 1024, uint32_t WV = 0>
@@ -1434,12 +1496,12 @@
     main_kernel<24, 64>(), main_kernel<28, 64>(), main_kernel<32, 64>(), main_kernel<36, 64>(), main_kernel<40, 64>()};
 static inline bool wide_g(uint32_t W, uint32_t G) { return W == 1 && G >= 12; }
 static inline bool wide12_big(uint32_t S, uint32_t W, uint32_t G) { return W == 1 && G == 12 && S >= WIDE12_BIG_S; }
-static void pipe_kernel(uint32_t G, uint32_t W, bool big, bool PK, launch_fn *l, const void **k) {
+static void pipe_kernel(uint32_t G, uint32_t W, bool big, bool PK, launch_fn *l, const void **k, bool PW = false) {
     const bool wide = wide_g(W, G);
     const uint32_t BLK = wide ? 64u : 1024u, WV = big ? (PK ? BIGP_WV : WIDE12_BIG_WAVES) : 0u;
     *l = nullptr;
     *k = nullptr;
-    if (const TuKernel *t = tu_find(G, BLK, WV, PK)) {
+    if (const TuKernel *t = tu_find(G, BLK, WV, PK, PW)) {
         *l = t->launch;
         *k = t->kernel();
         return;
@@ -1463,11 +1525,11 @@
 #define FPP_TU_CAT2(a, b) a##b
 #define FPP_TU_CAT(a, b) FPP_TU_CAT2(a, b)
 int FPP_TU_CAT(fpp_tu_launch_, FPP_TU_NAME)(hipStream_t st, unsigned grid, unsigned block, size_t lds, const void *args) {
-    return fpp::launch_g<FPP_TU_G, FPP_TU_BLK, FPP_TU_WV, (bool)FPP_TU_PK>(st, grid, block, lds,
-                                                                          *static_cast<const fpp::PipeArgs *>(args));
+    return fpp::launch_g<FPP_TU_G, FPP_TU_BLK, FPP_TU_WV, FPP_TU_PK != 0, FPP_TU_PK == 2>(
+        st, grid, block, lds, *static_cast<const fpp::PipeArgs *>(args));
 }
 const void *FPP_TU_CAT(fpp_tu_kernel_, FPP_TU_NAME)() {
-    return (const void *)fpp::k_ffd_pipe<FPP_TU_G, FPP_TU_BLK, FPP_TU_WV, (bool)FPP_TU_PK>;
+    return (const void *)fpp::k_ffd_pipe<FPP_TU_G, FPP_TU_BLK, FPP_TU_WV, FPP_TU_PK != 0, FPP_TU_PK == 2>;
 }
 #endif
 
@@ -1607,7 +1669,18 @@
     if (!pipe_geom(c, S, C, N, &g)) return 0;
     const size_t SC = (size_t)S * C, nlinks = (size_t)S * (g.B - 1);
     return 5 * SC * 4 + SC * 5 + 256 + nlinks * LCTL * 4 + (size_t)S * g.B * 8 + 8 + nlinks * g.slots * 2 * 64 * 4 +
-           (size_t)S * 16 + 11 * 256;
+           2 * (size_t)S * 16 + 12 * 256;
+}
+
+bool fp_pipe_prepack(fp_ctx *c, uint32_t S, uint32_t C, uint32_t N) {
+    if (!PREPACK_OK || fp_opt(c, FP_OPT_PREPACK, 1) == 0 || fp_opt(c, FP_OPT_PACKED, 1) == 0) return false;
+    PipeGeom g;
+    if (!pipe_geom(c, S, C, N, &g)) return false;
+    if (!wide12_big(S, g.W, g.G) || g.bounded) return false;
+    launch_fn l;
+    const void *k;
+    pipe_kernel(g.G, g.W, true, true, &l, &k, FPP_PREPACK_FFD != 0);
+    return l != nullptr;
 }
 
 uint32_t fp_pipe_kpack(const fp_ctx *c, uint32_t C) {
@@ -1679,11 +1752,13 @@
     const uint32_t kpack = fp_pipe_kpack(c, C);
     launch_fn u32fn = nullptr, pkfn = nullptr;
     const bool big = wide12_big(S, W, G) && !geo.bounded;
+    const uint32_t *pkhdr = ready ? ready->pkhdr : nullptr;
+    if (pkhdr && !(big && rng && ready->payload_done)) return FP_EINVAL;
     {
         const void *k_;
         pipe_kernel(G, W, big, false, &u32fn, &k_);
-        if (rng && fp_opt(c, FP_OPT_PACKED, 1) != 0) pipe_kernel(G, W, big, true, &pkfn, &k_);
-        if (!u32fn) return FP_EOVERFLOW;
+        if (rng && fp_opt(c, FP_OPT_PACKED, 1) != 0) pipe_kernel(G, W, big, true, &pkfn, &k_, pkhdr && FPP_PREPACK_FFD);
+        if (!u32fn || (pkhdr && !pkfn)) return FP_EOVERFLOW;
     }
     const bool payload_done = ready && ready->payload_done;
     uint32_t *summ = payload_done ? ready->summ : nullptr;
@@ -1716,7 +1791,12 @@
                 b->conflict, b->level, summ, s_cpu, s_mem, s_req, s_conf, s_idx);
         FP_HIP(hipGetLastError());
     }
+    if (pkhdr) {
+        k_unpack_rows<<<S, 1024, 0, st>>>(C, kpack, FPP_PREPACK_FFD ? 0u : 1u, pkhdr, rng, thr, s_cpu, s_mem, s_idx);
+        FP_HIP(hipGetLastError());
+    }
     PipeArgs a;
+    a.pkhdr = pkhdr;
     a.C = C; a.N = N; a.scen_base = scen_base; a.W = W; a.G = G; a.R = R;
     a.B = B; a.slots = slots; a.bounded = geo.bounded; a.ticket = ctl; a.gabort = ctl + 32; a.ghead = ctl + 64;
     a.gdata = gdata;
diff --git a/fleetflow_amd/csrc/fp_pipe_tus.h b/fleetflow_amd/csrc/fp_pipe_tus.h
--- a/fleetflow_amd/csrc/fp_pipe_tus.h
+++ b/fleetflow_amd/csrc/fp_pipe_tus.h
@@ -3,6 +3,7 @@
 #define FPP_TUS(X)            \
     X(big, 12, 64, 6, 0)      \
     X(bigp, 12, 64, 7, 1)     \
+    X(bigpw, 12, 64, 7, 2)    \
     X(w12, 12, 64, 0, 0)      \
     X(w12p, 12, 64, 0, 1)     \
     X(m8, 8, 1024, 0, 0)      \
diff --git a/fleetflow_amd/csrc/fp_place.hip b/fleetflow_amd/csrc/fp_place.hip
--- a/fleetflow_amd/csrc/fp_place.hip
+++ b/fleetflow_amd/csrc/fp_place.hip
@@ -182,7 +182,20 @@
     uint32_t *rng;
     const uint32_t *req, *conf, *level, *summ;
     uint32_t *s_req, *s_conf;
+    uint32_t *pkhdr;
 };
+
+__device__ __forceinline__ bool ss_prepack(const ScenSortArgs &a, uint32_t oc, uint32_t om, uint32_t &sc_c,
+                                           uint32_t &sc_m) {
+    oc = __builtin_amdgcn_readfirstlane(oc | a.summ[(size_t)blockIdx.x * 4 + 2]);
+    om = __builtin_amdgcn_readfirstlane(om | a.summ[(size_t)blockIdx.x * 4 + 3]);
+    const bool packs = fp_pk_shifts(oc, om, &sc_c, &sc_m);
+    if (threadIdx.x == 0) {
+        uint32_t *h = a.pkhdr + (size_t)blockIdx.x * 4;
+        h[0] = sc_c; h[1] = sc_m; h[2] = packs ? 1u : 0u; h[3] = 0u;
+    }
+    return packs;
+}
 
 typedef uint64_t __attribute__((may_alias)) ss_u64a;
 typedef uint32_t __attribute__((may_alias)) ss_u32a;
@@ -270,6 +283,7 @@
     uint16_t *myrow = WH + w * SS_DIG;
     uint32_t *ord = a.order + cb;
     const uint32_t *cpu = a.cpu + cb, *mem = a.mem + cb;
+    uint32_t oc = 0, om = 0;
     for (uint32_t k = 0; k < 8; ++k) {
         const uint32_t *key = k < 4 ? mem : cpu;
         const uint32_t sh = 8u * (k & 3u);
@@ -280,7 +294,12 @@
         };
         for (uint32_t i = t; i < SS_WAVES * SS_DIG / 2; i += blockDim.x) reinterpret_cast<ss_u32a *>(WH)[i] = 0u;
         __syncthreads();
-        for (uint32_t p = s0 + lane; p < s1; p += 64) ss_inc16(myrow, ((~key[src(p)]) >> sh) & 0xFFu);
+        for (uint32_t p = s0 + lane; p < s1; p += 64) {
+            const uint32_t v = key[src(p)];
+            om |= k == 0 ? v : 0u;
+            oc |= k == 4 ? v : 0u;
+            ss_inc16(myrow, ((~v) >> sh) & 0xFFu);
+        }
         __syncthreads();
         ss_offsets(WH, HS, HB, t, lane, w);
         for (uint32_t p0 = s0; p0 < s1; p0 += 64) {
@@ -301,31 +320,37 @@
         }
         __syncthreads();
     }
-    uint32_t oc = 0, om = 0;
+    for (int o = 32; o > 0; o >>= 1) {
+        oc |= (uint32_t)__shfl_xor((int)oc, o);
+        om |= (uint32_t)__shfl_xor((int)om, o);
+    }
+    if (t < 2) HS[t] = 0u;
+    __syncthreads();
+    if (lane == 0) {
+        atomicOr(&HS[0], oc);
+        atomicOr(&HS[1], om);
+    }
+    __syncthreads();
+    if (t == 0) {
+        fp_or_new_bits(&a.rng[0], HS[0]);
+        fp_or_new_bits(&a.rng[1], HS[1]);
+    }
+}
+
+__device__ __forceinline__ void ss_generic_fields(const ScenSortArgs &a, size_t cb, uint32_t C, bool pw,
+                                                  uint32_t sc_c, uint32_t sc_m) {
+    const uint32_t t = threadIdx.x;
+    const uint32_t *ord = a.order + cb, *cpu = a.cpu + cb, *mem = a.mem + cb;
     for (uint32_t P = t; P < C; P += blockDim.x) {
         const uint32_t j = __hip_atomic_load(&ord[P], __ATOMIC_RELAXED, __HIP_MEMORY_SCOPE_AGENT);
         const uint32_t cv = cpu[j], mv = mem[j];
-        a.s_cpu[cb + P] = cv;
-        a.s_mem[cb + P] = mv;
-        a.s_idx[cb + P] = P | (a.kpack ? (ss_bucket(a.T, cv) << 21) | (ss_bucket(a.T + FP_BUCKETS, mv) << 26) : 0u);
-        oc |= cv;
-        om |= mv;
-    }
-    for (int o = 32; o > 0; o >>= 1) {
-        oc |= (uint32_t)__shfl_xor((int)oc, o);
-        om |= (uint32_t)__shfl_xor((int)om, o);
-    }
-    __syncthreads();
-    if (t < 2) HS[t] = 0u;
-    __syncthreads();
-    if (lane == 0) {
-        atomicOr(&HS[0], oc);
-        atomicOr(&HS[1], om);
-    }
-    __syncthreads();
-    if (t == 0) {
-        fp_or_new_bits(&a.rng[0], HS[0]);
-        fp_or_new_bits(&a.rng[1], HS[1]);
+        if (pw) {
+            a.s_cpu[cb + P] = ((cv >> sc_c) << 16) | (mv >> sc_m);
+        } else {
+            a.s_cpu[cb + P] = cv;
+            a.s_mem[cb + P] = mv;
+            a.s_idx[cb + P] = P | (a.kpack ? (ss_bucket(a.T, cv) << 21) | (ss_bucket(a.T + FP_BUCKETS, mv) << 26) : 0u);
+        }
     }
 }
 
@@ -387,6 +412,7 @@
     uint16_t *myrow = WH + w * SS_DIG;
     uint32_t dc = 0, dm = 0, hbits = 0, lbits = 0;
     uint32_t dvp[SS_CHUNKS / 2];
+    bool pw = false;
     unsigned long long ck1 = 0;
     const __amdgpu_buffer_rsrc_t rc_cpu = __builtin_amdgcn_make_buffer_rsrc((void *)cpu, (short)0, (int)(4 * C), 0x00020000);
     const __amdgpu_buffer_rsrc_t rc_mem = __builtin_amdgcn_make_buffer_rsrc((void *)mem, (short)0, (int)(4 * C), 0x00020000);
@@ -486,6 +512,9 @@
             __syncthreads();
             if (!elig) {
                 ss_generic(a, X, WH, HS, HB, cb, C);
+                uint32_t gsc_c = 0, gsc_m = 0;
+                if (FUSED && a.pkhdr) pw = ss_prepack(a, HS[0], HS[1], gsc_c, gsc_m);
+                ss_generic_fields(a, cb, C, pw, gsc_c, gsc_m);
                 return 2u;
             }
             if (t < SS_DIG) {
@@ -564,6 +593,17 @@
         __syncthreads();
         const unsigned long long ck3 = SS_CLK();
         uint32_t big = 0;
+        uint32_t psc_c = 0, psc_m = 0;
+        if (FUSED && a.pkhdr) {
+            uint32_t oc = 0, om = 0;
+            for (uint32_t i = lane; i < dc; i += 64) oc |= CV[i];
+            for (uint32_t i = lane; i < dm; i += 64) om |= MV[i];
+            for (int o = 32; o > 0; o >>= 1) {
+                oc |= (uint32_t)__shfl_xor((int)oc, o);
+                om |= (uint32_t)__shfl_xor((int)om, o);
+            }
+            pw = ss_prepack(a, oc, om, psc_c, psc_m);
+        }
 
         while (true) {
             uint32_t d = 0;
@@ -577,6 +617,7 @@
             __builtin_amdgcn_fence(__ATOMIC_SEQ_CST, "workgroup");
             const uint32_t cv = CV[d];
             const uint32_t kbc = a.kpack ? (uint32_t)CB[d] << 21 : 0u;
+            const uint32_t cvw = (cv >> psc_c) << 16;
             if (hi - lo <= 64 * SS_REG) {
                 uint32_t jv[SS_REG], lv[SS_REG];
 #pragma unroll
@@ -601,12 +642,20 @@
                     }
                 }
                 __builtin_amdgcn_fence(__ATOMIC_SEQ_CST, "workgroup");
-                for (uint32_t P = lo + lane; P < hi; P += 64) {
-                    const uint32_t j = X[P], l = LD[j];
-                    a.order[cb + P] = j;
-                    a.s_cpu[cb + P] = cv;
-                    a.s_mem[cb + P] = MV[l];
-                    a.s_idx[cb + P] = P | kbc | (a.kpack ? (uint32_t)MB[l] << 26 : 0u);
+                if (pw) {
+                    for (uint32_t P = lo + lane; P < hi; P += 64) {
+                        const uint32_t j = X[P], l = LD[j];
+                        a.order[cb + P] = j;
+                        a.s_cpu[cb + P] = cvw | (MV[l] >> psc_m);
+                    }
+                } else {
+                    for (uint32_t P = lo + lane; P < hi; P += 64) {
+                        const uint32_t j = X[P], l = LD[j];
+                        a.order[cb + P] = j;
+                        a.s_cpu[cb + P] = cv;
+                        a.s_mem[cb + P] = MV[l];
+                        a.s_idx[cb + P] = P | kbc | (a.kpack ? (uint32_t)MB[l] << 26 : 0u);
+                    }
                 }
             } else {
                 if (FUSED && lane == 0) NEXT[3] = 1u;
@@ -626,9 +675,13 @@
                         if ((m & lt) == 0) myrow[l] = (uint16_t)(off + __popcll(m));
                         const uint32_t P = off + (uint32_t)__popcll(m & lt);
                         a.order[cb + P] = j;
-                        a.s_cpu[cb + P] = cv;
-                        a.s_mem[cb + P] = MV[l];
-                        a.s_idx[cb + P] = P | kbc | (a.kpack ? (uint32_t)MB[l] << 26 : 0u);
+                        if (pw) {
+                            a.s_cpu[cb + P] = cvw | (MV[l] >> psc_m);
+                        } else {
+                            a.s_cpu[cb + P] = cv;
+                            a.s_mem[cb + P] = MV[l];
+                            a.s_idx[cb + P] = P | kbc | (a.kpack ? (uint32_t)MB[l] << 26 : 0u);
+                        }
                     }
                 }
             }
@@ -672,8 +725,9 @@
         __syncthreads();
         const unsigned long long ckp = SS_CLK();
         const bool from_x = rr != 2u && __builtin_amdgcn_readfirstlane((int)NEXT[3]) == 0;
+        static_assert(fpl::PL_SKIP == 1u << 31, "the skip bit of s_w");
         fpl::pl_by_field<true>(reinterpret_cast<uint32_t *>(ssm), C, a.order, X, from_x, a.req, a.conf, a.level, a.summ,
-                               a.s_req, a.s_conf, a.s_idx);
+                               a.s_req, a.s_conf, pw ? a.s_cpu : a.s_idx);
 #ifdef FP_PIPE_STATS
         __syncthreads();
         if (t == 0) atomicAdd(&g_sort_stats[8], SS_CLK() - ckp);
@@ -835,6 +889,7 @@
         sa.scnt = rcnt;
         sa.rng = rcnt + CN_ORC;
         sa.simg = simg;
+        sa.pkhdr = nullptr;
         k_sort_image<<<1, 1024, 0, st>>>(rbm, rpre, rval, rcnt, thr, sa.kpack, simg);
         FP_HIP(hipGetLastError());
         const bool fused = FPP_PAYLOAD_BY_FIELD && fp_opt(c, FP_OPT_SORT_FUSED, 1) != 0 && C <= fp_pipe_payload_lds_max_c(c);
@@ -844,6 +899,11 @@
             soa.payload_done = true;
             sa.req = b->req_labels; sa.conf = b->conflict; sa.level = b->level; sa.summ = soa.summ;
             sa.s_req = soa.s_req; sa.s_conf = soa.s_conf;
+            if (soa.summ && fp_pipe_prepack(c, S, C, N)) {
+                soa.pkhdr = (uint32_t *)fp_ws_take(c, (size_t)S * 16);
+                if (!soa.pkhdr) return FP_ENOMEM;
+                sa.pkhdr = soa.pkhdr;
+            }
             if (lds < fpl::PL_FIELD_LDS_BYTES) lds = fpl::PL_FIELD_LDS_BYTES;
             static_assert(fpl::PL_FIELD_LDS_BYTES <= SS_LDS_CAP, "the chunk buffer fits the sort's LDS");
             FP_HIP(hipFuncSetAttribute((const void *)k_scen_sort<true>, hipFuncAttributeMaxDynamicSharedMemorySize, (int)lds));
@@ -872,7 +932,12 @@
     if (!c->last_rng) return FP_OK;
     FP_HIP(hipSetDevice(c->device));
     FP_HIP(hipStreamSynchronize(c->stream));
-    FP_HIP(hipMemcpy(out3, c->last_rng, 12, hipMemcpyDeviceToHost));
+    uint32_t w[4];
+    static_assert(CN_ORC + 4 == CN_WORDS, "last_rng holds four words");
+    FP_HIP(hipMemcpy(w, c->last_rng, 16, hipMemcpyDeviceToHost));
+    out3[0] = w[0];
+    out3[1] = w[1];
+    out3[2] = (w[2] == 1u && w[3] != 0u) ? 4u : w[2];
     return FP_OK;
 }
 
diff --git a/fleetflow_amd/planner.py b/fleetflow_amd/planner.py
--- a/fleetflow_amd/planner.py
+++ b/fleetflow_amd/planner.py
@@ -291,7 +291,9 @@
     def place_path(self) -> dict:
         out = (ct.c_uint32 * 3)()
         check(self._L.fp_ctx_place_path(self._ctx, out), "fp_ctx_place_path")
-        return {"or_cpu": int(out[0]), "or_mem": int(out[1]), "packed": int(out[2]) == 2, "ran": int(out[2]) != 0}
+        k = int(out[2])
+        return {"or_cpu": int(out[0]), "or_mem": int(out[1]), "packed": k in (2, 3), "ran": k != 0,
+                "prepacked": k == 3, "repaired": k == 4}
 
     def kernel_stats(self, kernel_id: int):
         ms = ct.c_double()
diff --git a/include/fleetplace.h b/include/fleetplace.h
--- a/include/fleetplace.h
+++ b/include/fleetplace.h
@@ -94,7 +94,8 @@
     FP_OPT_INDEG_BIN = 21,
     FP_OPT_PACKED = 22,
     FP_OPT_SORT_FUSED = 23,
-    FP_OPT_COUNT = 24
+    FP_OPT_PREPACK = 24,
+    FP_OPT_COUNT = 25
 };
 int fp_ctx_set_option(fp_ctx *ctx, int option, int64_t value);
 int fp_ctx_get_option(fp_ctx *ctx, int option, int64_t *value);
diff --git a/integration/fleetflow-placement/src/ffi.rs b/integration/fleetflow-placement/src/ffi.rs
--- a/integration/fleetflow-placement/src/ffi.rs
+++ b/integration/fleetflow-placement/src/ffi.rs
@@ -141,6 +141,7 @@
 pub const FP_OPT_INDEG_BIN: c_int = 21;
 pub const FP_OPT_PACKED: c_int = 22;
 pub const FP_OPT_SORT_FUSED: c_int = 23;
+pub const FP_OPT_PREPACK: c_int = 24;
 pub const FP_GEOM_GROUPS: usize = 0;
 pub const FP_GEOM_STAGES: usize = 1;
 pub const FP_GEOM_SEGMENTS: usize = 2;
```

Result: faster. 83570 billion (median of 6 runs) (+2.3%).
